# zqs01/ASR_chinese_e2e

Hardware: AMD Instinct MI355X
Metric: training throughput (utterances/s; frames/s = x T), AISHELL-1-shaped 80-mel T=500 (higher is better)
Workload: dtype bf16; 1 GPU; configs[2]: joint CTC/attention (lambda=0.3) encoder-decoder, bf16, per-GPU batch 32, T=500, F=80, V=4232, 6 layers, d_model 512, 8x64 heads, ff 1024, dropout 0.0, fwd+loss+CER+bwd+clip+Noam/Adam per step, eager launches; global_batch=32, seq_len=500, parallelism=dp1

## Files before the change

asr_chinese_e2e_amd/Models/transformer_official.py:

```python
import math

import torch

from .. import engine as E
from .. import kernels as K
from ..Bases import BaseConfig, BaseModel
from ..Utils import Pack

SOS_ID, EOS_ID, PAD_ID = 2, 3, 0
PE_MAXLEN = 5000
CLIP_NORM = 5.0


def _set_nested(root, dotted, value, is_buffer=False):
    parts = dotted.split(".")
    mod = root
    for p in parts[:-1]:
        if not hasattr(mod, p):
            mod.add_module(p, torch.nn.Module())
        mod = getattr(mod, p)
    if is_buffer:
        mod.register_buffer(parts[-1], value)
    else:
        mod.register_parameter(parts[-1], value)


class _SpeechTransformer(BaseModel):
    USE_DECODER = True

    def __init__(self, config, vocab):
        super().__init__()
        self.config = config
        self.vocab = vocab
        c = config
        self.use_decoder = self.USE_DECODER
        lam = float(getattr(c, "ctc_weight", 0.0))
        self.ctc_weight = lam if self.use_decoder else 1.0
        self.use_ctc = (lam > 0.0) or not self.use_decoder
        self.cross_mask = getattr(c, "cross_mask", "ref_compat")
        self.lowp = str(getattr(c, "dtype", "bf16")).lower() in ("bf16", "bfloat16")
        self.attn_window = int(getattr(c, "attn_window", -1))
        self.label_smoothing = float(getattr(c, "label_smoothing", 0.0))
        self.cer_in_iterate = bool(getattr(c, "cer_in_iterate", True))
        self._step_seed = int(getattr(c, "seed", 0))
        d, H, dk, ff = c.d_model, c.num_head, c.hidden_size, c.ff_size
        d_in = c.n_mels * c.lfr_m
        V = vocab.vocab_size
        self.V = V

        blocks = [[("encoder.linear_in.weight", (d, d_in))], [("encoder.linear_in.bias", (d,))],
                  [("encoder.layer_norm_in.weight", (d,))], [("encoder.layer_norm_in.bias", (d,))]]
        for i in range(c.layer_num):
            blocks += E.mha_param_block(f"encoder.layer_stack.{i}.slf_attn.", H, dk, d)
            blocks += E.ffn_param_block(f"encoder.layer_stack.{i}.pos_ffn.", d, ff)
        if self.use_ctc:
            blocks += [[("ctc_lo.weight", (V, d))], [("ctc_lo.bias", (V,))]]
        if self.use_decoder:
            blocks += [[("decoder.tgt_word_emb.weight", (V, d))]]
            blocks += E.cross_kv_param_blocks([f"decoder.layer_stack.{i}.enc_attn." for i in range(c.layer_num)], H, dk, d)
            for i in range(c.layer_num):
                blocks += E.mha_param_block(f"decoder.layer_stack.{i}.slf_attn.", H, dk, d)
                blocks += E.cross_q_param_block(f"decoder.layer_stack.{i}.enc_attn.", H, dk, d)
                blocks += E.ffn_param_block(f"decoder.layer_stack.{i}.pos_ffn.", d, ff)
        self._flat = E.FlatParams(blocks)
        self._engine = None
        self._views_checked = False
        self._grads_checked = False
        self._flat_device = None

        order = self._state_order(c.layer_num)
        for name in order:
            if name.endswith("positional_encoding.pe"):
                _set_nested(self, name, E.positional_encoding(PE_MAXLEN, d), is_buffer=True)
            elif name == "decoder.tgt_word_prj.weight":
                _set_nested(self, name, self.decoder.tgt_word_emb.weight)
            else:
                wname = name[:-5] + ".weight" if name.endswith(".bias") else name
                wshape = self._flat.index[wname][1]
                _set_nested(self, name, torch.nn.Parameter(self._init_tensor(name, self._flat.index[name][1], wshape, d, dk)))

    def _state_order(self, L):
        def mha(pre):
            return [pre + n for n in ("w_qs.weight", "w_qs.bias", "w_ks.weight", "w_ks.bias", "w_vs.weight", "w_vs.bias",
                                      "layer_norm.weight", "layer_norm.bias", "fc.weight", "fc.bias")]

        def ffn(pre):
            return [pre + n for n in ("w_1.weight", "w_1.bias", "w_2.weight", "w_2.bias", "layer_norm.weight", "layer_norm.bias")]

        names = ["encoder.linear_in.weight", "encoder.linear_in.bias", "encoder.layer_norm_in.weight",
                 "encoder.layer_norm_in.bias", "encoder.positional_encoding.pe"]
        for i in range(L):
            names += mha(f"encoder.layer_stack.{i}.slf_attn.") + ffn(f"encoder.layer_stack.{i}.pos_ffn.")
        if self.use_decoder:
            names += ["decoder.tgt_word_emb.weight", "decoder.positional_encoding.pe"]
            for i in range(L):
                names += mha(f"decoder.layer_stack.{i}.slf_attn.") + mha(f"decoder.layer_stack.{i}.enc_attn.") + ffn(f"decoder.layer_stack.{i}.pos_ffn.")
            names += ["decoder.tgt_word_prj.weight"]
        if self.use_ctc:
            names += ["ctc_lo.weight", "ctc_lo.bias"]
        return names

    @staticmethod
    def _init_tensor(name, shape, wshape, d, dk):
        t = torch.empty(*shape)
        leaf = name.rsplit(".", 2)[-2]
        if leaf in ("layer_norm", "layer_norm_in"):
            return t.fill_(1.0) if name.endswith(".weight") else t.zero_()
        fan_out, fan_in = wshape[0], wshape[1]
        if name == "decoder.tgt_word_emb.weight":
            return t.normal_(0.0, 1.0)
        if name.endswith(".weight"):
            if leaf in ("w_qs", "w_ks", "w_vs"):
                return t.normal_(0.0, math.sqrt(2.0 / (d + dk)))
            if leaf in ("fc", "linear_in", "ctc_lo"):
                return t.normal_(0.0, math.sqrt(2.0 / (fan_in + fan_out)))
        bound = 1.0 / math.sqrt(fan_in)
        return t.uniform_(-bound, bound)

    def _named_flat_params(self):
        for name, p in self.named_parameters():
            yield name, p

    def _ensure_engine(self, device):
        device = torch.device(device)
        if device.type == "cuda" and device.index is None:
            device = torch.device("cuda", torch.cuda.current_device())
        if device.type != "cuda":
            raise RuntimeError("the HIP engine runs on an MI355X only: move the model and batch to 'cuda' "
                               "(there is no CPU fallback; the CPU oracle lives in oracle/ for tests)")
        f = self._flat
        ok = self._engine is not None and self._flat_device == device
        if ok and self._views_checked:
            return self._engine
        if ok:
            for name, p in self._named_flat_params():
                off, shape = f.index[name]
                if p.data_ptr() != f.p.data_ptr() + 4 * off:
                    ok = False
                    break
        if ok:
            self._views_checked = True
            return self._engine
        K.bind_device(device)
        old = {name: p.detach().to(device=device, dtype=torch.float32) for name, p in self._named_flat_params()}
        old_mv = (f.m.to(device), f.v.to(device)) if f.m is not None else None
        f.allocate(device, self.lowp)
        if old_mv is not None:
            f.m.copy_(old_mv[0])
            f.v.copy_(old_mv[1])
        for name, p in self._named_flat_params():
            view = f.view(f.p, name)
            view.copy_(old[name].view(view.shape))
            p.data = view
            p.grad = f.view(f.g, name)
        f.refresh_lowp()
        for b in self.buffers():
            b.data = b.data.to(device)
        pe = self.encoder.positional_encoding.pe[0].to(device).contiguous()
        self._engine = E.Engine(f, self.config, self.V, self.use_decoder, self.use_ctc, pe)
        self._flat_device = device
        self._views_checked = True
        self._grads_checked = True
        return self._engine

    def zero_grad(self, set_to_none=True):
        self._grads_checked = False
        return super().zero_grad(set_to_none=set_to_none)

    def _apply(self, fn, *a, **kw):
        self._views_checked = False
        self._grads_checked = False
        return super()._apply(fn, *a, **kw)

    def load_state_dict(self, state_dict, strict=True, **kw):
        state_dict = {k: v for k, v in state_dict.items()}
        self._views_checked = False
        out = super().load_state_dict(state_dict, strict=strict, **kw)
        if self._flat.p is not None:
            self._flat.refresh_lowp()
        return out

    def zero_flat_grads(self):
        f = self._flat
        eng = self._engine
        self._zero_lazy = eng is not None and eng._tr_tiles is not None and eng.overlap_wgrad
        if not self._zero_lazy:
            f.g.zero_()
        if self._grads_checked:
            return
        for name, p in self._named_flat_params():
            if p.grad is None or p.grad.data_ptr() != f.g.data_ptr() + 4 * f.index[name][0]:
                p.grad = f.view(f.g, name)
        self._grads_checked = True

    def _prepare(self, input, training=False):
        wave = input.wave
        eng = self._ensure_engine(wave.device)
        eng.training = bool(training)
        if training:
            self._step_seed = (self._step_seed + 1) & 0x7FFFFFFF
            eng.step_seed = self._step_seed
        x = wave if wave.dtype == eng.dtype else wave.to(eng.dtype)
        x = x.contiguous()
        if input.tgt_for_input is None:
            self._tgt_len32 = None
            return eng, x, self._len32_of(input.wave_len, (), ()).contiguous(), None
        tgt = input.tgt_for_input.contiguous()
        lens64 = [t.contiguous() for t in (input.wave_len, input.tgt_len) if t is not None and t.dtype == torch.int64 and t.device == tgt.device]
        out = K.dec_preprocess(tgt, SOS_ID, EOS_ID, lens64=lens64)
        prep, lens32 = out[:6], (out[6] if lens64 else ())
        wave_len = self._len32_of(input.wave_len, lens64, lens32)
        self._tgt_len32 = self._len32_of(input.tgt_len, lens64, lens32) if input.tgt_len is not None else None
        return eng, x, wave_len, prep

    @staticmethod
    def _len32_of(t, lens64, lens32):
        for a, b in zip(lens64, lens32):
            if a.data_ptr() == t.data_ptr() and a.numel() == t.numel():
                return b
        return t.to(torch.int32)

    def forward(self, input):
        eng, x, wave_len, prep = self._prepare(input)
        B, T, _ = x.shape
        enc, _ = eng.encoder_fwd(x, wave_len, self.attn_window)
        pack = Pack()
        pack.add(encoder_out=enc.view(B, T, -1))
        if self.use_decoder and prep is not None:
            cross_len = self._tgt_len32 if self.cross_mask == "ref_compat" else wave_len
            pred, _ = eng.decoder_fwd(prep, enc, cross_len, B, T)
            pack.add(pred=pred.view(B, -1, self.V), gold=prep[1].long())
        if self.use_ctc:
            logits = eng.ctc_lo.fwd(enc)
            pack.add(ctc_logits=logits.view(B, T, self.V))
        return pack

    def _tok_table(self, device):
        if getattr(self, "_tok_tab", None) is None or self._tok_tab[0].device != torch.device(device):
            self._tok_tab = K.token_table(self.vocab._id2token, device)
        return self._tok_tab

    def _cer_ids(self, ids, gold, hyp_len=None, ref_len=None):
        per = K.cer(ids.int().contiguous(), gold.int().contiguous(), self._tok_table(ids.device), self.vocab._token2id[self.vocab.PAD],
                    hyp_len=hyp_len, ref_len=ref_len)
        return (per.sum() * (100.0 / per.numel())).reshape(1)

    CER_BESIDE_BACKWARD = True

    def _cer_beside_backward(self, eng, pg):
        if not (self.CER_BESIDE_BACKWARD and eng.aux_overlap) or torch.cuda.is_current_stream_capturing():
            return pg
        eng._disarm()
        eng._fork(eng.ctc_stream)
        with torch.cuda.stream(eng.ctc_stream):
            cer = self._cer_ids(pg[0], pg[1])
        if getattr(self, "_cer_event", None) is None:
            self._cer_event = torch.cuda.Event()
        self._cer_event.record(eng.ctc_stream)
        self._cer_keep = pg
        return cer, self._cer_event

    def _ctc_cer_beside_backward(self, eng, path, wave_len, labels32, lab_len):
        def score():
            ids, lens = K.ctc_collapse(path, wave_len, PAD_ID)
            return self._cer_ids(ids, labels32, hyp_len=lens, ref_len=lab_len)
        if not (self.CER_BESIDE_BACKWARD and eng.aux_overlap) or torch.cuda.is_current_stream_capturing():
            return score(), None
        eng._disarm()
        eng._fork(eng.ctc_stream)
        with torch.cuda.stream(eng.ctc_stream):
            cer = score()
        if getattr(self, "_cer_event", None) is None:
            self._cer_event = torch.cuda.Event()
        self._cer_event.record(eng.ctc_stream)
        self._cer_keep = (path, wave_len, labels32, lab_len)
        return cer, self._cer_event

    def _cer_of(self, pg):
        if isinstance(pg[1], torch.cuda.Event):
            torch.cuda.current_stream().wait_event(pg[1])
            return pg[0]
        if pg[1] is None:
            return pg[0]
        return self._cer_ids(pg[0], pg[1])

    def _cer(self, pred, gold):
        return self._cer_ids(pred.argmax(-1), gold)

    def cal_metrics(self, output, input):
        pack = Pack()
        row_nll = nll = n_valid = None
        if self.use_decoder:
            pred, gold = output.pred, output.gold
            B, To, V = pred.shape
            n_valid = (gold != PAD_ID).sum().float().reshape(1)
            row_nll, _ = K.xent_fwd_bwd(pred.reshape(B * To, V).contiguous(), gold.reshape(-1).int(), n_valid, PAD_ID, smoothing=self.label_smoothing, want_grad=False)
        if self.use_ctc:
            prep = K.dec_preprocess(input.tgt_for_input.contiguous(), SOS_ID, EOS_ID)
            nll, _ = K.ctc_fwd_bwd(output.ctc_logits.contiguous(), input.wave_len.to(torch.int32), prep[2], prep[4], self._engine.ws, want_grad=False)
        lam = self.ctc_weight
        loss = K.loss_combine(row_nll, n_valid, nll, 1.0 - lam if self.use_ctc else 1.0, lam)
        assert not torch.isinf(loss[0])
        pack.add(loss=loss[0])
        if self.use_decoder:
            pack.add(cer=self._cer(output.pred, output.gold))
        if self.use_ctc:
            cer = self._ctc_cer(output.ctc_logits.contiguous(), input.wave_len.to(torch.int32), prep[2], prep[4])
            pack.add(**({"ctc_cer": cer} if self.use_decoder else {"cer": cer}))
        return pack

    def beam_search(self, input, beam_size=5, nbest=1, decode_max_len=0, ctc_weight=0.0, joint="rescore", ctc_pre_beam=None):
        from .. import decode
        if joint not in ("rescore", "one_pass"):
            raise ValueError(f"joint must be 'rescore' or 'one_pass' (got {joint!r})")
        if joint == "one_pass":
            return decode.one_pass_beam_search(self, input, beam_size, nbest, decode_max_len, ctc_weight, ctc_pre_beam)
        if ctc_pre_beam is not None:
            raise ValueError("ctc_pre_beam applies to joint='one_pass' only")
        if ctc_weight > 0.0:
            return decode.joint_beam_search(self, input, beam_size, nbest, decode_max_len, ctc_weight)
        return decode.beam_search(self, input, beam_size, nbest, decode_max_len)

    def ctc_prefix_beam_search(self, input, beam_size=5, nbest=1, frame_topk=10, on_device=None):
        from .. import decode
        return decode.ctc_prefix_beam_search(self, input, beam_size, nbest, frame_topk, on_device)

    def ctc_greedy_search(self, input):
        with torch.no_grad():
            out = self.forward(input)
        ids, lens = K.ctc_greedy_decode(out.ctc_logits.contiguous(), input.wave_len.to(torch.int32), PAD_ID)
        ids, lens = ids.cpu(), lens.cpu()
        return [ids[b, : int(lens[b])].tolist() for b in range(ids.shape[0])]

    def frame_seconds(self):
        from ..data_handler.processor import HOP
        return int(getattr(self.config, "lfr_n", 3) or 3) * HOP / float(getattr(self.config, "sample_rate", 16000) or 16000)

    def ctc_align(self, input, labels=None):
        if not self.use_ctc:
            raise RuntimeError("this model has no CTC head (config.ctc_weight = 0)")
        if labels is None:
            if input.tgt_for_input is None:
                raise ValueError("ctc_align(labels=None) aligns the batch's transcripts, and this batch has none: pass labels")
            prep = K.dec_preprocess(input.tgt_for_input.contiguous(), SOS_ID, EOS_ID)
            lab, lens = prep[2].cpu(), prep[4].cpu().tolist()
            labels = [lab[b, : lens[b]].tolist() for b in range(lab.shape[0])]
        return self._align_lists(self._ctc_logits(input), input.wave_len, labels)

    def _ctc_logits(self, input):
        eng = self._ensure_engine(input.wave.device)
        was_training = eng.training
        try:
            with torch.no_grad():
                return self.forward(input).ctc_logits
        finally:
            eng.training = was_training

    def _align_lists(self, logits, wave_len, labels, alignable=None):
        B, T, V = logits.shape
        if len(labels) != B:
            raise ValueError(f"{len(labels)} label sequences for a batch of {B}")
        labels = [[int(x) for x in l] for l in labels]
        ok = [True] * B if alignable is None else list(alignable)
        for b, l in enumerate(labels):
            if ok[b] and (len(l) > 255 or any(x < 0 or x >= V for x in l)):
                raise ValueError(f"utterance {b}: labels must be at most 255 ids in [0, {V})")
        use = [l if ok[b] else [] for b, l in enumerate(labels)]
        Lmax = max([len(l) for l in use] + [0])
        lab = torch.zeros(B, Lmax, dtype=torch.int32)
        for b, l in enumerate(use):
            if l:
                lab[b, : len(l)] = torch.tensor(l, dtype=torch.int32)
        dev = logits.device
        lab_len = torch.tensor([len(l) for l in use], dtype=torch.int32)
        _, spans, tlp, score = K.ctc_align(logits, wave_len.to(torch.int32).contiguous(), lab.to(dev), lab_len.to(dev), blank=PAD_ID,
                                           ws=self._engine.ws)
        spans, tlp, score = spans.cpu().tolist(), tlp.cpu().tolist(), score.cpu().tolist()
        d = self.frame_seconds()
        id2tok = self.vocab._id2token
        out = []
        for b, l in enumerate(labels):
            timed = ok[b] and score[b] != float("-inf")
            toks = []
            for i, x in enumerate(l):
                st, en = (spans[b][i][0], spans[b][i][1]) if timed else (None, None)
                toks.append({"id": x, "token": id2tok[x] if 0 <= x < len(id2tok) else None, "start_frame": st, "end_frame": en,
                             "start_s": st * d if timed else None, "end_s": (en + 1) * d if timed else None,
                             "logp": tlp[b][i] if timed else None})
            out.append({"score": score[b] if ok[b] else None, "tokens": toks})
        return out

    def transcribe(self, input, beam_size=5, ctc_weight=None, timestamps=True, joint="rescore"):
        if joint not in ("rescore", "one_pass"):
            raise ValueError(f"joint must be 'rescore' or 'one_pass' (got {joint!r})")
        if joint == "one_pass" and not (self.use_decoder and self.use_ctc):
            raise RuntimeError("joint='one_pass' needs a model with both the attention decoder and the CTC head")
        if timestamps and not self.use_ctc:
            raise ValueError("timestamps come from the CTC head, and this model has none (config.ctc_weight = 0)")
        if self.use_decoder:
            w = float(getattr(self.config, "ctc_weight", 0.0)) if ctc_weight is None else float(ctc_weight)
            hyps = self.beam_search(input, beam_size, 1, ctc_weight=w if self.use_ctc else 0.0, joint=joint)
        else:
            hyps = self.ctc_prefix_beam_search(input, beam_size, 1)
        ids, scores = [], []
        for h in hyps:
            if not h:
                ids.append([])
                scores.append(float("-inf"))
                continue
            seq = list(h[0]["yseq"])
            if self.use_decoder:
                seq = seq[1:] if seq and seq[0] == SOS_ID else seq
                seq = seq[:-1] if seq and seq[-1] == EOS_ID else seq
            ids.append(seq)
            scores.append(float(h[0]["score"]))
        id2tok = self.vocab._id2token
        out = [{"text": "".join(id2tok[x] for x in seq if x not in (PAD_ID, SOS_ID, EOS_ID)), "ids": seq, "score": sc, "tokens": None}
               for seq, sc in zip(ids, scores)]
        if timestamps:
            V = self.V
            ok = [len(seq) <= 255 and all(0 <= x < V and x != PAD_ID for x in seq) for seq in ids]
            al = self._align_lists(self._ctc_logits(input), input.wave_len, ids, alignable=ok)
            for o, a in zip(out, al):
                o["tokens"] = a["tokens"]
        return out

    def _ctc_cer(self, logits, wave_len, labels32, lab_len):
        ids, lens = K.ctc_greedy_decode(logits, wave_len, PAD_ID)
        return self._cer_ids(ids, labels32, hyp_len=lens, ref_len=lab_len)

    def train_step(self, input, loss_scale=1.0, count_hook=None):
        eng, x, wave_len, prep = self._prepare(input, training=self.training)
        B, T, _ = x.shape
        lam = self.ctc_weight
        ys_in, ys_out, labels32, dec_len, lab_len, n_valid = prep
        pending = count_hook(n_valid, B) if count_hook is not None else None
        zero, self._zero_lazy = (self._flat.g if getattr(self, "_zero_lazy", False) else None), False
        eng.refresh_transposes(zero=zero)
        enc, ecache = eng.encoder_fwd(x, wave_len, self.attn_window)
        batch_div = None
        if pending is not None:
            n_valid, batch_div = pending.wait()
        row_nll = nll = None
        d_enc = None
        pg = None
        ctc_done = None
        ctc_scale = dict(grad_scale=lam * loss_scale, grad_scale_div=batch_div) if batch_div is not None else dict(grad_scale=lam * loss_scale / float(B))
        ctc_async = (self.use_decoder and self.use_ctc and eng.overlap_ctc and not eng.deterministic and not torch.cuda.is_current_stream_capturing())
        if ctc_async:
            eng.decoder_kv_async(prep, enc, B, T)
            nll, d_enc, ctc_done = eng.ctc_branch_async(enc, wave_len, labels32, lab_len, B, T, **ctc_scale)
        if self.use_decoder:
            cross_len = self._tgt_len32 if self.cross_mask == "ref_compat" else wave_len
            pred, dcache = eng.decoder_fwd(prep, enc, cross_len, B, T)
            ids = torch.empty(ys_out.shape, dtype=torch.int32, device=pred.device) if self.cer_in_iterate else None
            w_ce = (1.0 - lam) if self.use_ctc else 1.0
            row_nll, dpred = K.xent_fwd_bwd(pred, ys_out.reshape(-1), n_valid, PAD_ID, smoothing=self.label_smoothing, grad_scale=w_ce * loss_scale, dlogits=pred,
                                            argmax=ids)
            if ids is not None:
                pg = (ids, ys_out)
        if self.use_ctc and not ctc_async:
            path = torch.empty(B, T, dtype=torch.int32, device=enc.device) if (self.cer_in_iterate and not self.use_decoder) else None
            nll, d_enc = eng.ctc_fwd_bwd(enc, wave_len, labels32, lab_len, B, T, best_path=path, **ctc_scale)
            if path is not None:
                pg = self._ctc_cer_beside_backward(eng, path, wave_len, labels32, lab_len)
        if self.use_decoder:
            if d_enc is None:
                d_enc = torch.zeros_like(enc)
            eng.decoder_bwd(dcache, dpred, d_enc, d_enc_ready=ctc_done)
            if pg is not None:
                pg = self._cer_beside_backward(eng, pg)
        eng.encoder_bwd(ecache, d_enc)
        loss = K.loss_combine(row_nll, n_valid, nll, (1.0 - lam) if self.use_ctc else 1.0, lam)
        return loss, pg

    def iterate(self, input, optimizer=None, is_train=True):
        if optimizer is None or not is_train:
            with torch.no_grad():
                output = self.forward(input)
                return self.cal_metrics(output, input), None
        self._ensure_engine(input.wave.device)
        optimizer.zero_grad()
        if getattr(optimizer, "fused_step", None) is None or not getattr(optimizer, "keeps_grad_views", False):
            self._grads_checked = False
        self.zero_flat_grads()
        loss, pg = self.train_step(input)
        fused = getattr(optimizer, "fused_step", None)
        if fused is not None:
            fused(self._flat, CLIP_NORM)
        else:
            torch.nn.utils.clip_grad_norm_(self.parameters(), CLIP_NORM)
            optimizer.step()
            self._flat.refresh_lowp()
        metrics = Pack()
        metrics.add(loss=loss[0])
        if self.use_decoder and self.use_ctc:
            metrics.add(ce=loss[1], ctc=loss[2])
        if pg is not None:
            metrics.add(cer=self._cer_of(pg))
        return metrics, None

    def greedy_search(self, input, decode_max_len=0):
        return self.beam_search(input, 1, 1, decode_max_len)

    @classmethod
    def get_default_config(cls):
        class ModelConfig(BaseConfig):
            d_model = 512
            hidden_size = 64
            ff_size = 1024
            num_head = 8
            dropout = 0.1
            layer_num = 6
            share_weight = False
            ctc_weight = 0.0
            label_smoothing = 0.0
            cross_mask = "ref_compat"
            dtype = "bf16"
            attn_window = -1

        return ModelConfig


class TransformerOffical(_SpeechTransformer):
    USE_DECODER = True


class TransformerCTC(_SpeechTransformer):
    USE_DECODER = False
```

asr_chinese_e2e_amd/_lib.py:

```python
import ctypes
import os
from ctypes import c_char_p, c_float, c_int, c_size_t, c_uint32, c_void_p

import torch

_HERE = os.path.dirname(os.path.abspath(__file__))
LIB_PATH = os.environ.get("ASR_HIP_LIB") or os.path.join(_HERE, "libasr_hip.so")

ASR_F32, ASR_BF16 = 0, 1
ACT_NONE, ACT_RELU, ACT_RELU_MASK = 0, 1, 2
ABI_VERSION = 10
DROP_PRE, DROP_POST = 1, 2

P, I, F, Z, U = c_void_p, c_int, c_float, c_size_t, c_uint32

class TnProblem(ctypes.Structure):
    _fields_ = [("dY", P), ("X", P), ("dW", P), ("dbias", P), ("M", I), ("N", I), ("K", I), ("ldy", I), ("ldx", I), ("ldw", I)]


TN_GROUP_MAX = 8


class LnReduceItem(ctypes.Structure):
    _fields_ = [("ws", P), ("dgamma", P), ("dbeta", P), ("dbias", P), ("rows", I)]


LN_REDUCE_MAX = 16


class DecLayerPlan(ctypes.Structure):
    _fields_ = ([(n, I) for n in ("B", "To", "T", "d", "H", "dk", "ff")] + [("drop_p", F), ("seed", U * 5), ("ld_kv_c_T", I)] +
                [(n, P) for n in ("dec_len", "cross_len",
                                  "w_qkv_s", "w_fc_s", "w_q_c", "w_fc_c", "w_1", "w_2",
                                  "b_qkv_s", "b_fc_s", "b_q_c", "b_fc_c", "b_1", "b_2",
                                  "g_s", "be_s", "g_c", "be_c", "g_f", "be_f",
                                  "w_kv_c_T", "x_in",
                                  "qkv_s", "ctx_s", "a_s", "y_s", "lse_s", "rstd_s",
                                  "q_c", "kv_c", "kv_ready_event",
                                  "ctx_c", "a_c", "y_c", "lse_c", "rstd_c",
                                  "h", "o", "y_f", "rstd_f",
                                  "dz_f", "g_o", "g_h", "dx_f",
                                  "dz_c", "g_ac", "g_qc", "g_kvc", "dx_c",
                                  "dz_s", "g_as", "g_qkv", "dx_s",
                                  "dctx", "gb_2", "gb_fc_c", "gb_fc_s",
                                  "part_f", "part_c", "part_s", "delta")] +
                [("delta_bytes", Z), ("d_enc", P), ("wgrad_stream", P), ("aux_cus", I), ("ld_kv_c", I), ("kv_dgrad_cols", I), ("g_kv_group", P), ("ctx_s_lo", P), ("ctx_c_lo", P)])

SIGNATURES = {
    "asr_abi_version": (I, []),
    "asr_last_error": (I, [c_char_p, Z]),
    "asr_stream_fork": (I, [P, P]),
    "asr_stream_arm": (I, [P, P]),
    "asr_stream_arm_pending": (I, []),
    "asr_stream_create": (I, [I, P]),
    "asr_set_option": (I, [c_char_p, I, P]),
    "asr_get_deterministic": (I, []),
    "asr_set_deterministic": (I, [I]),
    "asr_add_ln_fwd": (I, [P, P, P, P, P, P, P, P, P, I, I, I, F, U, I, I, P]),
    "asr_add_ln_bwd_workspace_bytes": (Z, [I, I]),
    "asr_add_ln_bwd": (I, [P, P, P, P, P, P, P, P, P, P, P, P, Z, I, I, I, F, U, I, I, P]),
    "asr_add_ln_bwd_reduce_batched": (I, [P, I, I, P]),
    "asr_sdpa_fwd": (I, [P, P, P, P, P, P, I, I, I, I, I, I, I, I, I, I, I, F, F, U, P, I, P]),
    "asr_sdpa_bwd_workspace_bytes": (Z, [I, I, I, I, I, I, I, I]),
    "asr_sdpa_bwd": (I, [P, P, P, P, P, P, P, Z, P, P, P, P, I, I, I, I, I, I, I, I, I, I, I, F, F, U, P, I, P]),
    "asr_dropout_mask": (I, [P, I, I, F, U, P]),
    "asr_sdpa_dropout_mask": (I, [P, I, I, I, I, F, U, P]),
    "asr_ctc_workspace_bytes": (Z, [I, I, I]),
    "asr_ctc_fwd_bwd": (I, [P, P, P, P, P, P, I, I, I, I, I, I, F, P, I, P, P, Z, I, P]),
    "asr_ctc_align_workspace_bytes": (Z, [I, I, I]),
    "asr_ctc_align": (I, [P, P, P, P, P, P, P, P, I, I, I, I, I, I, P, Z, I, P]),
    "asr_ctc_greedy_decode": (I, [P, P, P, P, I, I, I, I, I, I, P]),
    "asr_ctc_frame_argmax": (I, [P, P, P, I, I, I, I, I, I, P]),
    "asr_ctc_collapse": (I, [P, P, P, I, I, I, P]),
    "asr_decode_attn": (I, [P, P, P, P, P, I, I, I, I, I, I, I, I, I, I, I, F, I, P]),
    "asr_logsoftmax_topk": (I, [P, P, P, I, I, I, I, I, P]),
    "asr_ctc_frame_topk": (I, [P, P, P, P, I, I, I, I, I, I, P]),
    "asr_ctc_prefix_beam_workspace_bytes": (Z, [I, I, I]),
    "asr_ctc_prefix_beam": (I, [P, P, P, P, P, Z, P, P, P, I, I, I, I, I, I, I, P]),
    "asr_beam_step": (I, [P, P, P, P, P, P, P, P, P, P, P, P, I, I, I, I, P]),
    "asr_cache_gather": (I, [P, P, P, I, I, I, I, I, I, P]),
    "asr_ctc_prefix_logprobs": (I, [P, P, I, I, I, I, I, P]),
    "asr_ctc_prefix_score": (I, [P, P, P, P, P, P, P, P, P, P, P, P, P, P, P, P, I, I, I, I, I, I, F, I, I, P]),
    "asr_ctc_prefix_gather": (I, [P, P, P, P, P, P, P, P, P, I, I, I, I, P]),
    "asr_joint_beam_step": (I, [P, P, P, P, P, P, P, P, P, P, P, P, P, P, P, P, P, P, P, I, I, I, I, F, P]),
    "asr_xent_fwd_bwd": (I, [P, P, P, P, P, I, I, I, F, F, P, I, P]),
    "asr_dec_preprocess": (I, [P, P, P, P, P, P, P, I, I, I, I, P, P, P, P, P]),
    "asr_embed_pe_fwd": (I, [P, P, P, P, F, I, I, I, I, F, U, I, P]),
    "asr_embed_bwd": (I, [P, P, P, P, F, I, I, I, F, U, I, P]),
    "asr_relu_fwd": (I, [P, Z, I, P]),
    "asr_relu_bwd": (I, [P, P, P, P, Z, I, I, I, P]),
    "asr_colsum_workspace_bytes": (Z, [I, I]),
    "asr_colsum": (I, [P, P, P, Z, I, I, I, I, I, P]),
    "asr_cast": (I, [P, P, Z, I, I, P]),
    "asr_sumsq_workspace_bytes": (Z, [Z]),
    "asr_grad_sumsq": (I, [P, Z, P, P, Z, P]),
    "asr_noam_hyper": (I, [P, P, F, F, F, F, F, F, P]),
    "asr_grad_sumsq_noam": (I, [P, Z, P, P, Z, P, P, F, F, F, F, F, F, P]),
    "asr_adam_step": (I, [P, P, P, P, P, Z, P, P, F, F, F, F, I, P]),
    "asr_loss_combine": (I, [P, I, P, P, I, F, F, P, P]),
    "asr_gemm_nt_bf16": (I, [P, P, P, P, P, I, I, I, I, I, I, I, P]),
    "asr_gemm_small_bf16": (I, [P, P, P, P, P, I, I, I, I, I, I, I, I, P]),
    "asr_gemm_f32": (I, [P, P, P, P, P, I, I, I, I, I, I, I, I, I, I, P]),
    "asr_decoder_layer_fwd": (I, [P, P]),
    "asr_decoder_layer_bwd": (I, [P, P, P, P, P]),
    "asr_gemm_tn_workspace_bytes": (Z, [I, I, I]),
    "asr_gemm_tn_bf16": (I, [P, P, P, I, I, I, I, I, I, I, P, Z, P]),
    "asr_gemm_tn_bias_bf16": (I, [P, P, P, P, I, I, I, I, I, I, I, P, Z, P]),
    "asr_gemm_tn_grouped_bf16": (I, [P, I, I, P]),
    "asr_transpose_batched_bf16": (I, [P, P, P, I, P]),
    "asr_cer": (I, [P, P, I, I, P, P, I, I, P, P, I, I, I, I, P, P]),
    "asr_logmel_fwd": (I, [P, P, P, P, P, I, I, I, I, P]),
    "asr_utt_norm_lfr_fwd": (I, [P, P, P, P, I, I, I, I, I, I, I, P]),
    "asr_utt_norm_augment_lfr_fwd": (I, [P, P, P, P, P, I, I, I, I, I, I, I, P]),
}


class AsrHipError(RuntimeError):
    pass


def _check_runtime_env(env=None):
    env = os.environ if env is None else env
    v = env.get("ROC_SYSTEM_SCOPE_SIGNAL")
    if v is not None and v.strip() == "0":
        raise RuntimeError("ROC_SYSTEM_SCOPE_SIGNAL=0 is set: the two-stream training step of asr_chinese_e2e_amd waits on completion signals "
                           "across HIP queues and would hang silently under it - unset the variable (or set it to 1)")


def _load():
    _check_runtime_env()
    if not os.path.isfile(LIB_PATH):
        raise ImportError(
            f"{LIB_PATH} not found: the HIP extension is required (no CPU fallback). "
            "Build it with `make -C asr_chinese_e2e_amd/csrc`.")
    lib = ctypes.CDLL(LIB_PATH)
    for name, (res, args) in SIGNATURES.items():
        try:
            fn = getattr(lib, name)
        except AttributeError as e:
            raise ImportError(f"{LIB_PATH} does not export {name}: rebuild the extension") from e
        fn.restype = res
        fn.argtypes = args
    v = lib.asr_abi_version()
    if v != ABI_VERSION:
        raise ImportError(f"libasr_hip.so ABI version {v}, binding expects {ABI_VERSION}")
    return lib


lib = _load()


def _bind_fast():
    try:
        alt = os.environ.get("ASR_FASTCALL_DIR")
        if alt:
            import glob
            import importlib.machinery
            import importlib.util
            path = glob.glob(os.path.join(alt, "_asr_fastcall*.so"))[0]
            loader = importlib.machinery.ExtensionFileLoader("_asr_fastcall", path)
            _asr_fastcall = importlib.util.module_from_spec(importlib.util.spec_from_loader("_asr_fastcall", loader))
            loader.exec_module(_asr_fastcall)
        else:
            from . import _asr_fastcall
    except (ImportError, IndexError) as e:
        raise ImportError(f"asr_chinese_e2e_amd/_asr_fastcall*.so not found or not loadable ({e}): build it with "
                          "`make -C asr_chinese_e2e_amd/csrc` (it is part of the required native code; there is no slow path)") from e
    kind = {P: "P", I: "I", F: "F", Z: "Z", U: "U", c_char_p: "P"}

    class _Fast:
        pass
    ns = _Fast()
    for name, (res, args) in SIGNATURES.items():
        addr = ctypes.cast(getattr(lib, name), c_void_p).value
        setattr(ns, name, _asr_fastcall.make(addr, name, "".join(kind[a] for a in args), "Z" if res is Z else "I"))
    return ns


fast = _bind_fast()


def last_error():
    buf = ctypes.create_string_buffer(512)
    lib.asr_last_error(buf, 512)
    return buf.value.decode("utf-8", "replace")


def check(rc, what=""):
    if rc != 0:
        names = {-1: "ASR_EINVAL", -2: "ASR_EDTYPE", -3: "ASR_EWORKSPACE", -4: "ASR_EHIP"}
        raise AsrHipError(f"{what}: {names.get(rc, rc)}: {last_error()}")
```

asr_chinese_e2e_amd/csrc/decoder_exec.hip:

```cpp
#include "asr_common.h"

#define DEC_TRY(call)                \
    do {                             \
        const int rc__ = (call);     \
        if (rc__ != ASR_OK) {        \
            asr_stream_arm_pending(); \
            return rc__;             \
        }                            \
    } while (0)

static int dec_check(const asr_dec_layer_plan* p, const char* who) {
    if (!p) ASR_FAIL(ASR_EINVAL, "%s: null plan", who);
    if (p->B <= 0 || p->To <= 0 || p->T <= 0 || p->H <= 0 || p->dk <= 0 || p->d <= 0 || p->ff <= 0)
        ASR_FAIL(ASR_EINVAL, "%s: bad dims B=%d To=%d T=%d d=%d H=%d dk=%d ff=%d", who, p->B, p->To, p->T, p->d, p->H, p->dk, p->ff);
    if (p->d % 8 || (p->H * p->dk) % 8 || p->ff % 8) ASR_FAIL(ASR_EINVAL, "%s: d, H*dk and ff must be multiples of 8", who);
    return ASR_OK;
}

extern "C" int asr_decoder_layer_fwd(const asr_dec_layer_plan* p, void* stream) {
    DEC_TRY(dec_check(p, "asr_decoder_layer_fwd"));
    const int B = p->B, To = p->To, T = p->T, d = p->d, H = p->H, dk = p->dk, hd = H * dk, ff = p->ff, M = B * To;
    const float scale = 1.0f / sqrtf((float)dk);
    const size_t e = 2;
    char* qkv = (char*)p->qkv_s;
    DEC_TRY(asr_gemm_small_bf16(p->x_in, p->w_qkv_s, p->b_qkv_s, nullptr, p->qkv_s, M, 3 * hd, d, d, d, 3 * hd, 0, ASR_ACT_NONE, stream));
    DEC_TRY(asr_sdpa_fwd(qkv, qkv + hd * e, qkv + 2 * hd * e, p->ctx_s, p->lse_s, p->dec_len, B, H, To, To, dk, 3 * hd, 3 * hd, 3 * hd, hd, 1, -1, scale,
                         p->drop_p, p->seed[0], p->ctx_s_lo, ASR_BF16, stream));
    DEC_TRY(asr_gemm_small_bf16(p->ctx_s, p->w_fc_s, p->b_fc_s, nullptr, p->a_s, M, d, hd, hd, hd, d, 0, ASR_ACT_NONE, stream));
    DEC_TRY(asr_add_ln_fwd(p->a_s, p->x_in, p->g_s, p->be_s, nullptr, p->dec_len, p->y_s, p->a_s, p->rstd_s, B, To, d, p->drop_p, p->seed[1], ASR_DROP_PRE,
                           ASR_BF16, stream));
    DEC_TRY(asr_gemm_small_bf16(p->y_s, p->w_q_c, p->b_q_c, nullptr, p->q_c, M, hd, d, d, d, hd, 0, ASR_ACT_NONE, stream));
    if (p->kv_ready_event) {
        const hipError_t he = hipStreamWaitEvent((hipStream_t)stream, (hipEvent_t)p->kv_ready_event, 0);
        if (he != hipSuccess) ASR_FAIL(ASR_EHIP, "asr_decoder_layer_fwd: hipStreamWaitEvent: %s", hipGetErrorString(he));
    }
    char* kv = (char*)p->kv_c;
    const int ldkv = p->ld_kv_c > 0 ? p->ld_kv_c : 2 * hd;
    DEC_TRY(asr_sdpa_fwd(p->q_c, kv, kv + hd * e, p->ctx_c, p->lse_c, p->cross_len, B, H, To, T, dk, hd, ldkv, ldkv, hd, 0, -1, scale, p->drop_p, p->seed[2],
                         p->ctx_c_lo, ASR_BF16, stream));
    DEC_TRY(asr_gemm_small_bf16(p->ctx_c, p->w_fc_c, p->b_fc_c, nullptr, p->a_c, M, d, hd, hd, hd, d, 0, ASR_ACT_NONE, stream));
    DEC_TRY(asr_add_ln_fwd(p->a_c, p->y_s, p->g_c, p->be_c, nullptr, p->dec_len, p->y_c, p->a_c, p->rstd_c, B, To, d, p->drop_p, p->seed[3], ASR_DROP_PRE,
                           ASR_BF16, stream));
    DEC_TRY(asr_gemm_small_bf16(p->y_c, p->w_1, p->b_1, nullptr, p->h, M, ff, d, d, d, ff, 0, ASR_ACT_RELU, stream));
    DEC_TRY(asr_gemm_small_bf16(p->h, p->w_2, p->b_2, nullptr, p->o, M, d, ff, ff, ff, d, 0, ASR_ACT_NONE, stream));
    DEC_TRY(asr_add_ln_fwd(p->o, p->y_c, p->g_f, p->be_f, nullptr, p->dec_len, p->y_f, p->o, p->rstd_f, B, To, d, p->drop_p, p->seed[4], ASR_DROP_PRE, ASR_BF16,
                           stream));
    return ASR_OK;
}

extern "C" int asr_decoder_layer_bwd(const asr_dec_layer_plan* p, const void* dy, const void* dy2, void* stream, void* aux_stream) {
    DEC_TRY(dec_check(p, "asr_decoder_layer_bwd"));
    if (!dy) ASR_FAIL(ASR_EINVAL, "asr_decoder_layer_bwd: null dy");
    const int B = p->B, To = p->To, T = p->T, d = p->d, H = p->H, dk = p->dk, hd = H * dk, ff = p->ff, M = B * To;
    const float scale = 1.0f / sqrtf((float)dk);
    const size_t e = 2;
    const bool drop = p->drop_p > 0.f;
    const size_t part_bytes = asr_add_ln_bwd_workspace_bytes(M, d);
    void* dxg_f = drop ? p->g_o : p->dz_f;
    DEC_TRY(asr_add_ln_bwd(dy, dy2, p->o, p->rstd_f, p->g_f, p->dec_len, p->dz_f, drop ? p->g_o : nullptr, nullptr, nullptr, p->gb_2, p->part_f, part_bytes, B, To, d,
                           p->drop_p, p->seed[4], ASR_DROP_PRE, ASR_BF16, stream));
    DEC_TRY(asr_gemm_small_bf16(dxg_f, p->w_2, nullptr, p->h, p->g_h, M, ff, d, d, ff, ff, 1, ASR_ACT_RELU_MASK, stream));
    DEC_TRY(asr_gemm_small_bf16(p->g_h, p->w_1, nullptr, nullptr, p->dx_f, M, d, ff, ff, d, d, 1, ASR_ACT_NONE, stream));
    void* dxg_c = drop ? p->g_ac : p->dz_c;
    DEC_TRY(asr_add_ln_bwd(p->dx_f, p->dz_f, p->a_c, p->rstd_c, p->g_c, p->dec_len, p->dz_c, drop ? p->g_ac : nullptr, nullptr, nullptr, p->gb_fc_c, p->part_c, part_bytes,
                           B, To, d, p->drop_p, p->seed[3], ASR_DROP_PRE, ASR_BF16, stream));
    DEC_TRY(asr_gemm_small_bf16(dxg_c, p->w_fc_c, nullptr, nullptr, p->dctx, M, hd, d, d, hd, hd, 1, ASR_ACT_NONE, stream));
    char* kv = (char*)p->kv_c;
    char* gkv = (char*)p->g_kvc;
    const bool kv_dgrad = p->d_enc && p->w_kv_c_T;
    const int ldkv = p->ld_kv_c > 0 ? p->ld_kv_c : 2 * hd;
    if (p->kv_dgrad_cols > 0 && (!p->g_kv_group || p->kv_dgrad_cols % 8 || p->kv_dgrad_cols > ldkv)) ASR_FAIL(ASR_EINVAL, "asr_decoder_layer_bwd: kv_dgrad_cols = %d needs g_kv_group, a multiple of 8, <= ld_kv_c = %d", p->kv_dgrad_cols, ldkv);
    if (kv_dgrad && aux_stream) DEC_TRY(asr_stream_arm(stream, aux_stream));
    DEC_TRY(asr_sdpa_bwd(p->q_c, kv, kv + hd * e, p->ctx_c, p->dctx, p->lse_c, p->delta, p->delta_bytes, p->g_qc, gkv, gkv + hd * e, p->cross_len, B, H, To, T, dk, hd,
                         ldkv, ldkv, hd, 0, -1, scale, p->drop_p, p->seed[2], p->ctx_c_lo, ASR_BF16, stream));
    if (kv_dgrad) {
        void* st2 = aux_stream ? aux_stream : stream;
        if (aux_stream && asr_stream_arm_pending()) DEC_TRY(asr_stream_fork(stream, aux_stream));
        const int old_lim = p->aux_cus > 0 ? asr_option_set(ASR_OPT_CU_LIMIT, p->aux_cus) : 0;
        const void* g_a = p->kv_dgrad_cols > 0 ? p->g_kv_group : p->g_kvc;
        const int cols = p->kv_dgrad_cols > 0 ? p->kv_dgrad_cols : 2 * hd;
        const int rc_kv = asr_gemm_nt_bf16(g_a, p->w_kv_c_T, nullptr, p->d_enc, p->d_enc, B * T, d, cols, ldkv, p->ld_kv_c_T, d, ASR_ACT_NONE, st2);
        if (p->aux_cus > 0) asr_option_set(ASR_OPT_CU_LIMIT, old_lim);
        DEC_TRY(rc_kv);
    }
    DEC_TRY(asr_gemm_small_bf16(p->g_qc, p->w_q_c, nullptr, nullptr, p->dx_c, M, d, hd, hd, d, d, 1, ASR_ACT_NONE, stream));
    void* dxg_s = drop ? p->g_as : p->dz_s;
    DEC_TRY(asr_add_ln_bwd(p->dx_c, p->dz_c, p->a_s, p->rstd_s, p->g_s, p->dec_len, p->dz_s, drop ? p->g_as : nullptr, nullptr, nullptr, p->gb_fc_s, p->part_s, part_bytes,
                           B, To, d, p->drop_p, p->seed[1], ASR_DROP_PRE, ASR_BF16, stream));
    DEC_TRY(asr_gemm_small_bf16(dxg_s, p->w_fc_s, nullptr, nullptr, p->dctx, M, hd, d, d, hd, hd, 1, ASR_ACT_NONE, stream));
    char* qkv = (char*)p->qkv_s;
    char* gq = (char*)p->g_qkv;
    DEC_TRY(asr_sdpa_bwd(qkv, qkv + hd * e, qkv + 2 * hd * e, p->ctx_s, p->dctx, p->lse_s, p->delta, p->delta_bytes, gq, gq + hd * e, gq + 2 * hd * e, p->dec_len, B, H, To,
                         To, dk, 3 * hd, 3 * hd, 3 * hd, hd, 1, -1, scale, p->drop_p, p->seed[0], p->ctx_s_lo, ASR_BF16, stream));
    if (p->wgrad_stream) DEC_TRY(asr_stream_arm(stream, p->wgrad_stream));
    DEC_TRY(asr_gemm_small_bf16(p->g_qkv, p->w_qkv_s, nullptr, nullptr, p->dx_s, M, d, 3 * hd, 3 * hd, d, d, 1, ASR_ACT_NONE, stream));
    return ASR_OK;
}
```

asr_chinese_e2e_amd/csrc/misc.hip:

```cpp
#include <stdarg.h>
#include <stdlib.h>

#include "asr_common.h"

static thread_local char g_err[512] = "";

void asr_set_error(const char* fmt, ...) {
    va_list ap;
    va_start(ap, fmt);
    vsnprintf(g_err, sizeof(g_err), fmt, ap);
    va_end(ap);
}

extern "C" int asr_abi_version(void) { return ASR_ABI_VERSION; }

static int g_deterministic = -1;
int asr_deterministic(void) {
    if (g_deterministic < 0) {
        const char* e = getenv("ASR_DETERMINISTIC");
        g_deterministic = (e && atoi(e) != 0) ? 1 : 0;
    }
    return g_deterministic;
}
extern "C" int asr_get_deterministic(void) { return asr_deterministic(); }
// ... 91 lines not shown
    if (e != hipSuccess || !st) ASR_FAIL(ASR_EHIP, "asr_stream_create: %s", hipGetErrorString(e));
    *out_stream = (void*)st;
    return ASR_OK;
}

namespace {

constexpr int EW_BLOCK = 256;
ASR_FULL_WAVES(EW_BLOCK);
static int ew_grid(size_t nvec) {
    size_t g = (nvec + EW_BLOCK - 1) / EW_BLOCK;
    return (int)(g < 2048 ? (g ? g : 1) : 2048);
}

template <typename T> __global__ __launch_bounds__(EW_BLOCK) void relu_fwd_kernel(T* x, size_t n8, size_t n) {
    for (size_t i = blockIdx.x * (size_t)EW_BLOCK + threadIdx.x; i < n8; i += (size_t)gridDim.x * EW_BLOCK) {
        float v[8];
        load8<T>(x + i * 8, v);
#pragma unroll
        for (int j = 0; j < 8; ++j) v[j] = fmaxf(v[j], 0.f);
        store8<T>(x + i * 8, v);
    }
    if (blockIdx.x == 0) {
        size_t i = n8 * 8 + threadIdx.x;
        if (i < n) x[i] = from_f32<T>(fmaxf(to_f32<T>(x[i]), 0.f));
    }
}

template <typename S, typename D> __global__ __launch_bounds__(EW_BLOCK) void cast_kernel(const S* s, D* d, size_t n8, size_t n) {
    for (size_t i = blockIdx.x * (size_t)EW_BLOCK + threadIdx.x; i < n8; i += (size_t)gridDim.x * EW_BLOCK) {
        float v[8];
        load8<S>(s + i * 8, v);
        store8<D>(d + i * 8, v);
    }
    if (blockIdx.x == 0) {
        size_t i = n8 * 8 + threadIdx.x;
        if (i < n) d[i] = from_f32<D>(to_f32<S>(s[i]));
    }
}

constexpr int CS_WAVES = 4;
template <typename T, bool RELU_BWD>
__global__ __launch_bounds__(CS_WAVES* WAVE) void colsum_partial_kernel(T* __restrict__ x, const T* __restrict__ a,
                                                                         float* __restrict__ ws, int rows, int cols, int ld,
                                                                         int row_slots) {
    const int lane = threadIdx.x & 63, w = threadIdx.x >> 6;
    const int c0 = blockIdx.x * 256 + lane * 4;
    f32x4 acc = {0.f, 0.f, 0.f, 0.f};
    const bool full = (c0 + 3 < cols) && (ld % 4 == 0);
    const int rstride = row_slots * CS_WAVES;
    int r = blockIdx.y * CS_WAVES + w;
    if (full) {
        for (; r + 3 * rstride < rows; r += 4 * rstride) {
            f32x4 v[4], av[4];
#pragma unroll
            for (int u = 0; u < 4; ++u) {
                v[u] = load4<T>(x + (size_t)(r + u * rstride) * ld + c0);
                if constexpr (RELU_BWD) av[u] = load4<T>(a + (size_t)(r + u * rstride) * ld + c0);
            }
#pragma unroll
            for (int u = 0; u < 4; ++u) {
                if constexpr (RELU_BWD) {
#pragma unroll
                    for (int j = 0; j < 4; ++j) v[u][j] = av[u][j] > 0.f ? v[u][j] : 0.f;
                    store4<T>(x + (size_t)(r + u * rstride) * ld + c0, v[u]);
                }
                acc += v[u];
            }
        }
    }
    for (; r < rows; r += rstride) {
        T* p = x + (size_t)r * ld + c0;
        if (full) {
            f32x4 v = load4<T>(p);
            if constexpr (RELU_BWD) {
                f32x4 av = load4<T>(a + (size_t)r * ld + c0);
#pragma unroll
                for (int j = 0; j < 4; ++j) v[j] = av[j] > 0.f ? v[j] : 0.f;
                store4<T>(p, v);
            }
            acc += v;
        } else {
#pragma unroll
            for (int j = 0; j < 4; ++j)
                if (c0 + j < cols) {
                    float v = to_f32<T>(p[j]);
                    if constexpr (RELU_BWD) {
                        v = to_f32<T>(a[(size_t)r * ld + c0 + j]) > 0.f ? v : 0.f;
                        p[j] = from_f32<T>(v);
                    }
                    acc[j] += v;
                }
        }
    }
    __shared__ __attribute__((aligned(16))) float sred[CS_WAVES][256];
    *(f32x4*)&sred[w][lane * 4] = acc;
    __syncthreads();
    const int c = blockIdx.x * 256 + threadIdx.x;
    if (c < cols) ws[(size_t)blockIdx.y * cols + c] = sred[0][threadIdx.x] + sred[1][threadIdx.x] + sred[2][threadIdx.x] + sred[3][threadIdx.x];
}

static int cs_row_slots(int rows, int cols) {
    int ctiles = ceil_div(cols, 256);
    int want = 2048 / ctiles;
    int maxs = ceil_div(rows, CS_WAVES);
    if (want > maxs) want = maxs;
    if (want < 1) want = 1;
    if (want > 256) want = 256;
    return want;
}

__global__ void dec_preprocess_kernel(const int64_t* __restrict__ tgt, int32_t* ys_in, int32_t* ys_out,
                                      int32_t* labels32, int32_t* dec_len, int32_t* lab_len, float* n_valid,
                                      int B, int Lmax, int sos, int eos, const int64_t* __restrict__ len_a, int32_t* len32_a,
                                      const int64_t* __restrict__ len_b, int32_t* len32_b) {
    __shared__ int cnt[1024];
    const int b = threadIdx.x;
    int n = 0;
    if (b < B) {
        if (len_a) len32_a[b] = (int32_t)len_a[b];
        if (len_b) len32_b[b] = (int32_t)len_b[b];
        const int To = Lmax + 1;
        int32_t* yi = ys_in + (size_t)b * To;
        int32_t* yo = ys_out + (size_t)b * To;
        int32_t* lb = labels32 + (size_t)b * Lmax;
        yi[0] = sos;
        for (int j = 0; j < Lmax; ++j) {
            int v = (int)tgt[(size_t)b * Lmax + j];
            if (v != 0) {
                lb[n] = v;
                yi[1 + n] = v;
                yo[n] = v;
                ++n;
            }
        }
        yo[n] = eos;
        for (int j = n + 1; j < To; ++j) { yi[j] = eos; yo[j] = 0; }
        for (int j = n; j < Lmax; ++j) lb[j] = 0;
        dec_len[b] = n + 1;
        lab_len[b] = n;
    }
    cnt[threadIdx.x] = (b < B) ? n + 1 : 0;
    __syncthreads();
    if (threadIdx.x == 0) {
        int s = 0;
        for (int i = 0; i < B; ++i) s += cnt[i];
        *n_valid = (float)s;
    }
}

template <typename T, typename W>
__global__ __launch_bounds__(256) void embed_pe_fwd_kernel(const int32_t* __restrict__ ids, const W* __restrict__ emb,
                                                           const float* __restrict__ pe, T* __restrict__ y, float scale,
                                                           int rows, int To, int d, int V, uint32_t seed, uint32_t thr, float dscale) {
    const int row = blockIdx.x;
    int id = ids[row];
    id = id < 0 ? 0 : (id >= V ? V - 1 : id);
    const int t = row % To;
    for (int c = threadIdx.x; c < d; c += blockDim.x) {
        float v = to_f32<W>(emb[(size_t)id * d + c]) * scale + pe[(size_t)t * d + c];
        if (thr) v = drop_keep_at((uint32_t)row * (uint32_t)d + c, seed, thr) ? v * dscale : 0.f;
        y[(size_t)row * d + c] = from_f32<T>(v);
    }
}
template <typename T>
__global__ __launch_bounds__(256) void embed_bwd_kernel(const int32_t* __restrict__ ids, const T* __restrict__ dy, const T* __restrict__ dy2,
                                                        float* __restrict__ demb, float scale, int d, int V, uint32_t seed, uint32_t thr,
                                                        float dscale) {
    const int row = blockIdx.x;
    const int id = ids[row];
    if (id < 0 || id >= V) return;
    for (int c = threadIdx.x; c < d; c += blockDim.x) {
        float g = (to_f32<T>(dy[(size_t)row * d + c]) + (dy2 ? to_f32<T>(dy2[(size_t)row * d + c]) : 0.f)) * scale;
        if (thr) g = drop_keep_at((uint32_t)row * (uint32_t)d + c, seed, thr) ? g * dscale : 0.f;
        if (g != 0.f) atomicAdd(&demb[(size_t)id * d + c], g);
    }
}

template <typename T>
__global__ __launch_bounds__(256) void embed_bwd_serial_kernel(const int32_t* __restrict__ ids, const T* __restrict__ dy, const T* __restrict__ dy2,
                                                               float* demb, float scale, int rows, int d, int V, uint32_t seed, uint32_t thr,
                                                               float dscale) {
    const int c = blockIdx.x * 256 + threadIdx.x;
    if (c >= d) return;
    for (int row = 0; row < rows; ++row) {
        const int id = ids[row];
        if (id < 0 || id >= V) continue;
        float g = (to_f32<T>(dy[(size_t)row * d + c]) + (dy2 ? to_f32<T>(dy2[(size_t)row * d + c]) : 0.f)) * scale;
        if (thr) g = drop_keep_at((uint32_t)row * (uint32_t)d + c, seed, thr) ? g * dscale : 0.f;
        if (g != 0.f) demb[(size_t)id * d + c] += g;
    }
}

__global__ __launch_bounds__(256) void dropout_mask_kernel(uint8_t* mask, size_t rows, int cols, uint32_t seed, uint32_t thr) {
    const size_t n = rows * (size_t)cols;
    const uint32_t cp = (uint32_t)((cols + 1) & ~1);
    for (size_t i = blockIdx.x * 256ull + threadIdx.x; i < n; i += (size_t)gridDim.x * 256) {
        const size_t r = i / cols;
        const uint32_t c = (uint32_t)(i - r * cols);
        mask[i] = drop_keep_at((uint32_t)r * cp + c, seed, thr) ? 1 : 0;
    }
}

constexpr int SS_BLOCK = 256;
ASR_FULL_WAVES(SS_BLOCK);
__global__ __launch_bounds__(SS_BLOCK) void sumsq_partial_kernel(const float* __restrict__ g, size_t n4, size_t n, float* __restrict__ part) {
    __shared__ float red[16];
    float s = 0.f;
    for (size_t i = blockIdx.x * (size_t)SS_BLOCK + threadIdx.x; i < n4; i += (size_t)gridDim.x * SS_BLOCK) {
        f32x4 v = *(const f32x4*)(g + i * 4);
        s += v[0] * v[0] + v[1] * v[1] + v[2] * v[2] + v[3] * v[3];
    }
    if (blockIdx.x == 0) {
        size_t i = n4 * 4 + threadIdx.x;
        if (i < n) s += g[i] * g[i];
    }
    s = block_sum(s, red);
    if (threadIdx.x == 0) part[blockIdx.x] = s;
}
__global__ __launch_bounds__(256) void sum_finalize_kernel(const float* __restrict__ part, int P, float* out) {
    __shared__ float red[16];
    float s = 0.f;
    for (int i = threadIdx.x; i < P; i += 256) s += part[i];
    s = block_sum(s, red);
    if (threadIdx.x == 0) *out = s;
}
__device__ __forceinline__ void noam_update(int32_t* step, float* hyper, float model_size, float warmup, float factor, float lr_const, float b1, float b2) {
    const int s = *step + 1;
    *step = s;
    const double sd = (double)s;
    double lr = lr_const;
    if (warmup > 0.f) {
        double a = pow(sd, -0.5), b = sd * pow((double)warmup, -1.5);
        lr = (double)factor * pow((double)model_size, -0.5) * (a < b ? a : b);
    }
    hyper[0] = (float)lr;
    hyper[1] = (float)(1.0 - pow((double)b1, sd));
    hyper[2] = (float)sqrt(1.0 - pow((double)b2, sd));
    hyper[3] = (float)s;
}
__global__ __launch_bounds__(256) void sum_finalize_noam_kernel(const float* __restrict__ part, int P, float* out, int32_t* step, float* hyper, float model_size,
                                                                float warmup, float factor, float lr_const, float b1, float b2) {
    __shared__ float red[16];
    float s = 0.f;
    for (int i = threadIdx.x; i < P; i += 256) s += part[i];
    s = block_sum(s, red);
    if (threadIdx.x == 0) {
        *out = s;
        noam_update(step, hyper, model_size, warmup, factor, lr_const, b1, b2);
    }
}
static int ss_grid(size_t n) {
    size_t g = (n / 4 + SS_BLOCK - 1) / SS_BLOCK;
    return (int)(g < 1024 ? (g ? g : 1) : 1024);
}

__global__ void noam_hyper_kernel(int32_t* step, float* hyper, float model_size, float warmup, float factor,
                                  float lr_const, float b1, float b2) {
    noam_update(step, hyper, model_size, warmup, factor, lr_const, b1, b2);
}

__global__ __launch_bounds__(EW_BLOCK) void adam_kernel(float* __restrict__ p, float* __restrict__ g, float* __restrict__ m,
                                                        float* __restrict__ v, bf16_t* __restrict__ p_lp, size_t n4, size_t n,
                                                        const float* __restrict__ hyper, const float* __restrict__ sumsq,
                                                        float max_norm, float b1, float b2, float eps, int write_clipped) {
    const float lr = hyper[0], bc1 = hyper[1], bc2s = hyper[2];
    float coef = 1.f;
    if (max_norm > 0.f) {
        const float norm = sqrtf(*sumsq);
        coef = fminf(max_norm / (norm + 1e-6f), 1.f);
    }
    const float step_size = lr / bc1;
    write_clipped = write_clipped && coef != 1.f;
    for (size_t i = blockIdx.x * (size_t)EW_BLOCK + threadIdx.x; i < n4; i += (size_t)gridDim.x * EW_BLOCK) {
        f32x4 gv = *(const f32x4*)(g + i * 4), mv = *(const f32x4*)(m + i * 4), vv = *(const f32x4*)(v + i * 4), pv = *(const f32x4*)(p + i * 4);
#pragma unroll
        for (int j = 0; j < 4; ++j) {
            const float gg = gv[j] * coef;
            gv[j] = gg;
            mv[j] = b1 * mv[j] + (1.f - b1) * gg;
            vv[j] = b2 * vv[j] + (1.f - b2) * gg * gg;
            pv[j] -= step_size * mv[j] / (sqrtf(vv[j]) / bc2s + eps);
        }
        *(f32x4*)(m + i * 4) = mv;
        *(f32x4*)(v + i * 4) = vv;
        *(f32x4*)(p + i * 4) = pv;
        if (write_clipped) *(f32x4*)(g + i * 4) = gv;
        if (p_lp) store4<bf16_t>(p_lp + i * 4, pv);
    }
    if (blockIdx.x == 0) {
        size_t i = n4 * 4 + threadIdx.x;
        if (i < n) {
            const float gg = g[i] * coef;
            const float mm = b1 * m[i] + (1.f - b1) * gg;
            const float vv = b2 * v[i] + (1.f - b2) * gg * gg;
            const float pp = p[i] - step_size * mm / (sqrtf(vv) / bc2s + eps);
            m[i] = mm; v[i] = vv; p[i] = pp;
            if (write_clipped) g[i] = gg;
            if (p_lp) p_lp[i] = (bf16_t)pp;
        }
    }
}

__global__ __launch_bounds__(256) void loss_combine_kernel(const float* row_nll, int M, const float* n_valid, const float* nll, int B,
                                                           float w_ce, float w_ctc, float* loss) {
    __shared__ float red[16];
    float s = 0.f, c = 0.f;
    if (row_nll) for (int i = threadIdx.x; i < M; i += 256) s += row_nll[i];
    if (nll) for (int i = threadIdx.x; i < B; i += 256) c += nll[i];
    s = block_sum(s, red);
    c = block_sum(c, red);
    if (threadIdx.x == 0) {
        const float ce = row_nll ? s / *n_valid : 0.f;
        const float ctc = nll ? c / (float)B : 0.f;
        loss[0] = (row_nll ? w_ce * ce : 0.f) + (nll ? w_ctc * ctc : 0.f);
        loss[1] = ce;
        loss[2] = ctc;
    }
}

}

extern "C" int asr_relu_fwd(void* x, size_t n, int dtype, void* stream) {
    if (!x) ASR_FAIL(ASR_EINVAL, "asr_relu_fwd: null pointer");
    hipStream_t st = (hipStream_t)stream;
    if (dtype == ASR_F32) relu_fwd_kernel<float><<<ew_grid(n / 8), EW_BLOCK, 0, st>>>((float*)x, n / 8, n);
    else if (dtype == ASR_BF16) relu_fwd_kernel<bf16_t><<<ew_grid(n / 8), EW_BLOCK, 0, st>>>((bf16_t*)x, n / 8, n);
    else ASR_FAIL(ASR_EDTYPE, "asr_relu_fwd: dtype %d", dtype);
    ASR_CHECK_LAUNCH("asr_relu_fwd");
    return ASR_OK;
}

__global__ __launch_bounds__(256) void transpose_batched_kernel(const bf16_t* __restrict__ src, bf16_t* __restrict__ dst, const int32_t* __restrict__ tiles) {
    __shared__ bf16_t tile[64][66];
    const int32_t* e = tiles + 6 * (size_t)blockIdx.x;
    const size_t off = (size_t)(uint32_t)e[0], doff = (size_t)(uint32_t)e[4];
    const int N = e[1], K = e[2], r0 = (e[3] >> 16) * 64, c0 = (e[3] & 0xffff) * 64, ldd = e[5];
    const int tx = threadIdx.x & 63, ty = threadIdx.x >> 6;
#pragma unroll
    for (int i = 0; i < 16; ++i) {
        const int r = r0 + ty + 4 * i, c = c0 + tx;
        if (r < N && c < K) tile[ty + 4 * i][tx] = src[off + (size_t)r * K + c];
    }
    __syncthreads();
#pragma unroll
    for (int i = 0; i < 16; ++i) {
        const int c = c0 + ty + 4 * i, r = r0 + tx;
        if (r < N && c < K) dst[doff + (size_t)c * ldd + r] = tile[tx][ty + 4 * i];
    }
}

__global__ __launch_bounds__(256) void transpose_batched_vec_kernel(const bf16_t* __restrict__ src, bf16_t* __restrict__ dst, const int32_t* __restrict__ tiles) {
    __shared__ __attribute__((aligned(16))) bf16_t tile[64][72];
    const int32_t* e = tiles + 6 * (size_t)blockIdx.x;
    const size_t off = (size_t)(uint32_t)e[0], doff = (size_t)(uint32_t)e[4];
    const int N = e[1], K = e[2], r0 = (e[3] >> 16) * 64, c0 = (e[3] & 0xffff) * 64, ldd = e[5];
    const bool vec = ((N | K | ldd) % 8 == 0) && (off % 8 == 0) && (doff % 8 == 0) && (((uintptr_t)src | (uintptr_t)dst) % 16 == 0);
    if (vec) {
#pragma unroll
        for (int c = 0; c < 2; ++c) {
            const int id = threadIdx.x + 256 * c, r = id >> 3, ch = id & 7;
            u32x4 v = {0u, 0u, 0u, 0u};
            if (r0 + r < N && c0 + ch * 8 < K) v = *(const u32x4*)(src + off + (size_t)(r0 + r) * K + c0 + ch * 8);
            *(u32x4*)(&tile[r][ch * 8]) = v;
        }
        __syncthreads();
#pragma unroll
        for (int c = 0; c < 2; ++c) {
            const int id = threadIdx.x + 256 * c, kk = id >> 3, ch = id & 7;
            if (c0 + kk < K && r0 + ch * 8 < N) {
                bf16x8 v;
#pragma unroll
                for (int j = 0; j < 8; ++j) v[j] = tile[ch * 8 + j][kk];
                *(bf16x8*)(dst + doff + (size_t)(c0 + kk) * ldd + r0 + ch * 8) = v;
            }
        }
        return;
    }
    const int tx = threadIdx.x & 63, ty = threadIdx.x >> 6;
#pragma unroll
    for (int i = 0; i < 16; ++i) {
        const int r = r0 + ty + 4 * i, c = c0 + tx;
        if (r < N && c < K) tile[ty + 4 * i][tx] = src[off + (size_t)r * K + c];
    }
    __syncthreads();
#pragma unroll
    for (int i = 0; i < 16; ++i) {
        const int c = c0 + ty + 4 * i, r = r0 + tx;
        if (r < N && c < K) dst[doff + (size_t)c * ldd + r] = tile[tx][ty + 4 * i];
    }
}

extern "C" int asr_transpose_batched_bf16(const void* src, void* dst, const int32_t* tiles, int ntiles, void* stream) {
    if (!src || !dst || !tiles) ASR_FAIL(ASR_EINVAL, "asr_transpose_batched_bf16: null pointer");
    if (ntiles <= 0) ASR_FAIL(ASR_EINVAL, "asr_transpose_batched_bf16: ntiles=%d", ntiles);
    transpose_batched_vec_kernel<<<ntiles, 256, 0, (hipStream_t)stream>>>((const bf16_t*)src, (bf16_t*)dst, tiles);
    ASR_CHECK_LAUNCH("asr_transpose_batched_bf16");
    return ASR_OK;
}

extern "C" int asr_cast(const void* src, void* dst, size_t n, int sd, int dd, void* stream) {
    if (!src || !dst) ASR_FAIL(ASR_EINVAL, "asr_cast: null pointer");
    hipStream_t st = (hipStream_t)stream;
    const int g = ew_grid(n / 8);
    if (sd == ASR_F32 && dd == ASR_BF16) cast_kernel<float, bf16_t><<<g, EW_BLOCK, 0, st>>>((const float*)src, (bf16_t*)dst, n / 8, n);
    else if (sd == ASR_BF16 && dd == ASR_F32) cast_kernel<bf16_t, float><<<g, EW_BLOCK, 0, st>>>((const bf16_t*)src, (float*)dst, n / 8, n);
    else if (sd == ASR_F32 && dd == ASR_F32) cast_kernel<float, float><<<g, EW_BLOCK, 0, st>>>((const float*)src, (float*)dst, n / 8, n);
    else if (sd == ASR_BF16 && dd == ASR_BF16) cast_kernel<bf16_t, bf16_t><<<g, EW_BLOCK, 0, st>>>((const bf16_t*)src, (bf16_t*)dst, n / 8, n);
    else ASR_FAIL(ASR_EDTYPE, "asr_cast: dtypes %d -> %d", sd, dd);
    ASR_CHECK_LAUNCH("asr_cast");
    return ASR_OK;
}

extern "C" size_t asr_colsum_workspace_bytes(int rows, int cols) {
    return (size_t)cs_row_slots(rows, cols) * cols * sizeof(float);
}

template <bool RELU_BWD>
static int colsum_impl(void* x, const void* a, float* out, void* ws, size_t ws_bytes, int rows, int cols, int ld,
                       int accumulate, int dtype, hipStream_t st, const char* name) {
    if (!x || (RELU_BWD && !a)) ASR_FAIL(ASR_EINVAL, "%s: null pointer", name);
    if (rows <= 0 || cols <= 0 || ld < cols) ASR_FAIL(ASR_EINVAL, "%s: bad shape rows=%d cols=%d ld=%d", name, rows, cols, ld);
    const bool want_sum = out != nullptr;
    if (want_sum && (!ws || ws_bytes < asr_colsum_workspace_bytes(rows, cols))) ASR_FAIL(ASR_EWORKSPACE, "%s: workspace too small", name);
    const int slots = cs_row_slots(rows, cols);
    dim3 grid(ceil_div(cols, 256), slots);
    if (!ws || ws_bytes < asr_colsum_workspace_bytes(rows, cols)) ASR_FAIL(ASR_EWORKSPACE, "%s: workspace too small", name);
    if (dtype == ASR_F32) colsum_partial_kernel<float, RELU_BWD><<<grid, CS_WAVES * WAVE, 0, st>>>((float*)x, (const float*)a, (float*)ws, rows, cols, ld, slots);
    else if (dtype == ASR_BF16) colsum_partial_kernel<bf16_t, RELU_BWD><<<grid, CS_WAVES * WAVE, 0, st>>>((bf16_t*)x, (const bf16_t*)a, (float*)ws, rows, cols, ld, slots);
    else ASR_FAIL(ASR_EDTYPE, "%s: dtype %d", name, dtype);
    if (want_sum) colsum_finalize_kernel<<<dim3(ceil_div(cols, 32), accumulate && slots >= 1024 && !asr_deterministic() ? 4 : 1), 1024, 0, st>>>((const float*)ws, slots, (size_t)cols, cols, cols, out, nullptr, nullptr, accumulate);
    ASR_CHECK_LAUNCH(name);
    return ASR_OK;
}

extern "C" int asr_colsum(const void* x, float* out, void* ws, size_t ws_bytes, int rows, int cols, int ld, int accumulate,
                          int dtype, void* stream) {
    if (!out) ASR_FAIL(ASR_EINVAL, "asr_colsum: null out");
    return colsum_impl<false>((void*)x, nullptr, out, ws, ws_bytes, rows, cols, ld, accumulate, dtype, (hipStream_t)stream, "asr_colsum");
}

extern "C" int asr_relu_bwd(void* da, const void* a, float* dbias, void* ws, size_t ws_bytes, int rows, int cols, int dtype,
                            void* stream) {
    return colsum_impl<true>(da, a, dbias, ws, ws_bytes, rows, cols, cols, 1, dtype, (hipStream_t)stream, "asr_relu_bwd");
}

extern "C" int asr_dec_preprocess(const int64_t* tgt, int32_t* ys_in, int32_t* ys_out, int32_t* labels32, int32_t* dec_len,
                                  int32_t* lab_len, float* n_valid, int B, int Lmax, int sos, int eos, const int64_t* len_a, int32_t* len32_a,
                                  const int64_t* len_b, int32_t* len32_b, void* stream) {
    if (!tgt || !ys_in || !ys_out || !labels32 || !dec_len || !lab_len || !n_valid) ASR_FAIL(ASR_EINVAL, "asr_dec_preprocess: null pointer");
    if ((len_a && !len32_a) || (len_b && !len32_b)) ASR_FAIL(ASR_EINVAL, "asr_dec_preprocess: a length vector without its int32 output");
    if (B <= 0 || B > 1024 || Lmax <= 0) ASR_FAIL(ASR_EINVAL, "asr_dec_preprocess: bad shape B=%d Lmax=%d (B <= 1024)", B, Lmax);
    const int threads = ceil_div(B, 64) * 64;
    dec_preprocess_kernel<<<1, threads, 0, (hipStream_t)stream>>>(tgt, ys_in, ys_out, labels32, dec_len, lab_len, n_valid, B, Lmax, sos, eos, len_a, len32_a, len_b, len32_b);
    ASR_CHECK_LAUNCH("asr_dec_preprocess");
    return ASR_OK;
}

extern "C" int asr_embed_pe_fwd(const int32_t* ids, const void* emb, const float* pe, void* y, float scale, int B, int To, int d,
                                int V, float drop_p, uint32_t drop_seed, int dtype, void* stream) {
    if (!ids || !emb || !pe || !y) ASR_FAIL(ASR_EINVAL, "asr_embed_pe_fwd: null pointer");
    if (B <= 0 || To <= 0 || d <= 0 || V <= 0) ASR_FAIL(ASR_EINVAL, "asr_embed_pe_fwd: bad shape");
    if (drop_p < 0.f || drop_p >= 1.f || (drop_p > 0.f && (d & 1))) ASR_FAIL(ASR_EINVAL, "asr_embed_pe_fwd: bad dropout p=%f", drop_p);
    hipStream_t st = (hipStream_t)stream;
    const uint32_t thr = drop_thr16(drop_p);
    const float ds = 1.f / (1.f - drop_p);
    if (dtype == ASR_F32) embed_pe_fwd_kernel<float, float><<<B * To, 256, 0, st>>>(ids, (const float*)emb, pe, (float*)y, scale, B * To, To, d, V, drop_seed, thr, ds);
    else if (dtype == ASR_BF16) embed_pe_fwd_kernel<bf16_t, float><<<B * To, 256, 0, st>>>(ids, (const float*)emb, pe, (bf16_t*)y, scale, B * To, To, d, V, drop_seed, thr, ds);
    else ASR_FAIL(ASR_EDTYPE, "asr_embed_pe_fwd: dtype %d", dtype);
    ASR_CHECK_LAUNCH("asr_embed_pe_fwd");
    return ASR_OK;
}

extern "C" int asr_embed_bwd(const int32_t* ids, const void* dy, const void* dy2, float* demb, float scale, int rows, int d, int V, float drop_p,
                             uint32_t drop_seed, int dtype, void* stream) {
    if (!ids || !dy || !demb) ASR_FAIL(ASR_EINVAL, "asr_embed_bwd: null pointer");
    if (rows <= 0 || d <= 0) ASR_FAIL(ASR_EINVAL, "asr_embed_bwd: bad shape");
    if (drop_p < 0.f || drop_p >= 1.f) ASR_FAIL(ASR_EINVAL, "asr_embed_bwd: bad dropout p=%f", drop_p);
    hipStream_t st = (hipStream_t)stream;
    const uint32_t thr = drop_thr16(drop_p);
    const float ds = 1.f / (1.f - drop_p);
    if (dtype != ASR_F32 && dtype != ASR_BF16) ASR_FAIL(ASR_EDTYPE, "asr_embed_bwd: dtype %d", dtype);
    if (asr_deterministic()) {
        if (dtype == ASR_F32) embed_bwd_serial_kernel<float><<<ceil_div(d, 256), 256, 0, st>>>(ids, (const float*)dy, (const float*)dy2, demb, scale, rows, d, V, drop_seed, thr, ds);
        else embed_bwd_serial_kernel<bf16_t><<<ceil_div(d, 256), 256, 0, st>>>(ids, (const bf16_t*)dy, (const bf16_t*)dy2, demb, scale, rows, d, V, drop_seed, thr, ds);
    } else if (dtype == ASR_F32) embed_bwd_kernel<float><<<rows, 256, 0, st>>>(ids, (const float*)dy, (const float*)dy2, demb, scale, d, V, drop_seed, thr, ds);
    else embed_bwd_kernel<bf16_t><<<rows, 256, 0, st>>>(ids, (const bf16_t*)dy, (const bf16_t*)dy2, demb, scale, d, V, drop_seed, thr, ds);
    ASR_CHECK_LAUNCH("asr_embed_bwd");
    return ASR_OK;
}

extern "C" int asr_dropout_mask(uint8_t* mask, int rows, int cols, float drop_p, uint32_t drop_seed, void* stream) {
    if (!mask || rows <= 0 || cols <= 0 || (cols & 1)) ASR_FAIL(ASR_EINVAL, "asr_dropout_mask: bad arguments (cols must be even)");
    const size_t n = (size_t)rows * cols;
    dropout_mask_kernel<<<(int)((n + 255) / 256 < 2048 ? (n + 255) / 256 : 2048), 256, 0, (hipStream_t)stream>>>(mask, (size_t)rows, cols, drop_seed, drop_thr16(drop_p));
    ASR_CHECK_LAUNCH("asr_dropout_mask");
    return ASR_OK;
}

extern "C" int asr_sdpa_dropout_mask(uint8_t* mask, int B, int H, int Tq, int Tk, float drop_p, uint32_t drop_seed, void* stream) {
    if (!mask || B <= 0 || H <= 0 || Tq <= 0 || Tk <= 0) ASR_FAIL(ASR_EINVAL, "asr_sdpa_dropout_mask: bad arguments");
    const size_t n = (size_t)B * H * Tq * Tk;
    dropout_mask_kernel<<<(int)((n + 255) / 256 < 2048 ? (n + 255) / 256 : 2048), 256, 0, (hipStream_t)stream>>>(mask, (size_t)B * H * Tq, Tk, drop_seed, drop_thr16(drop_p));
    ASR_CHECK_LAUNCH("asr_sdpa_dropout_mask");
    return ASR_OK;
}

extern "C" size_t asr_sumsq_workspace_bytes(size_t n) { return (size_t)ss_grid(n) * sizeof(float); }

extern "C" int asr_grad_sumsq(const float* g, size_t n, float* sumsq, void* ws, size_t ws_bytes, void* stream) {
    if (!g || !sumsq || !ws) ASR_FAIL(ASR_EINVAL, "asr_grad_sumsq: null pointer");
    if (ws_bytes < asr_sumsq_workspace_bytes(n)) ASR_FAIL(ASR_EWORKSPACE, "asr_grad_sumsq: workspace too small");
    if (((uintptr_t)g) % 16) ASR_FAIL(ASR_EINVAL, "asr_grad_sumsq: g must be 16-byte aligned");
    hipStream_t st = (hipStream_t)stream;
    const int grid = ss_grid(n);
    sumsq_partial_kernel<<<grid, SS_BLOCK, 0, st>>>(g, n / 4, n, (float*)ws);
    sum_finalize_kernel<<<1, 256, 0, st>>>((const float*)ws, grid, sumsq);
    ASR_CHECK_LAUNCH("asr_grad_sumsq");
    return ASR_OK;
}

extern "C" int asr_grad_sumsq_noam(const float* g, size_t n, float* sumsq, void* ws, size_t ws_bytes, int32_t* step, float* hyper, float model_size,
                                   float warmup, float factor, float lr_const, float b1, float b2, void* stream) {
    if (!g || !sumsq || !ws || !step || !hyper) ASR_FAIL(ASR_EINVAL, "asr_grad_sumsq_noam: null pointer");
    if (ws_bytes < asr_sumsq_workspace_bytes(n)) ASR_FAIL(ASR_EWORKSPACE, "asr_grad_sumsq_noam: workspace too small");
    if (((uintptr_t)g) % 16) ASR_FAIL(ASR_EINVAL, "asr_grad_sumsq_noam: g must be 16-byte aligned");
    hipStream_t st = (hipStream_t)stream;
    const int grid = ss_grid(n);
    sumsq_partial_kernel<<<grid, SS_BLOCK, 0, st>>>(g, n / 4, n, (float*)ws);
    sum_finalize_noam_kernel<<<1, 256, 0, st>>>((const float*)ws, grid, sumsq, step, hyper, model_size, warmup, factor, lr_const, b1, b2);
    ASR_CHECK_LAUNCH("asr_grad_sumsq_noam");
    return ASR_OK;
}

extern "C" int asr_noam_hyper(int32_t* step, float* hyper, float model_size, float warmup, float factor, float lr_const, float b1,
                              float b2, void* stream) {
    if (!step || !hyper) ASR_FAIL(ASR_EINVAL, "asr_noam_hyper: null pointer");
    noam_hyper_kernel<<<1, 1, 0, (hipStream_t)stream>>>(step, hyper, model_size, warmup, factor, lr_const, b1, b2);
    ASR_CHECK_LAUNCH("asr_noam_hyper");
    return ASR_OK;
}

extern "C" int asr_adam_step(float* p, float* g, float* m, float* v, void* p_lp, size_t n, const float* hyper, const float* sumsq,
                             float max_norm, float b1, float b2, float eps, int write_clipped, void* stream) {
    if (!p || !g || !m || !v || !hyper) ASR_FAIL(ASR_EINVAL, "asr_adam_step: null pointer");
    if (max_norm > 0.f && !sumsq) ASR_FAIL(ASR_EINVAL, "asr_adam_step: clipping needs sumsq");
    if ((((uintptr_t)p) | ((uintptr_t)g) | ((uintptr_t)m) | ((uintptr_t)v)) % 16) ASR_FAIL(ASR_EINVAL, "asr_adam_step: buffers must be 16-byte aligned");
    adam_kernel<<<ew_grid(n / 4), EW_BLOCK, 0, (hipStream_t)stream>>>(p, g, m, v, (bf16_t*)p_lp, n / 4, n, hyper, sumsq, max_norm, b1, b2, eps, write_clipped);
    ASR_CHECK_LAUNCH("asr_adam_step");
    return ASR_OK;
}

extern "C" int asr_loss_combine(const float* row_nll, int M, const float* n_valid, const float* nll, int B, float w_ce, float w_ctc,
                                float* loss, void* stream) {
    if (!loss || (row_nll && !n_valid)) ASR_FAIL(ASR_EINVAL, "asr_loss_combine: null pointer");
    loss_combine_kernel<<<1, 256, 0, (hipStream_t)stream>>>(row_nll, M, n_valid, nll, B, w_ce, w_ctc, loss);
    ASR_CHECK_LAUNCH("asr_loss_combine");
    return ASR_OK;
}
```

asr_chinese_e2e_amd/engine.py:

```python
import math
import os

import torch

import collections
import ctypes

from . import _lib
from . import kernels as K
from ._lib import ACT_NONE, ACT_RELU, ACT_RELU_MASK

ALIGN = 64


def positional_encoding(max_len, d_model):
    pe = torch.zeros(max_len, d_model)
    pos = torch.arange(0, max_len).unsqueeze(1).float()
    w = torch.exp(torch.arange(0, d_model, 2).float() * -(math.log(10000.0) / d_model))
    pe[:, 0::2] = torch.sin(pos * w)
    pe[:, 1::2] = torch.cos(pos * w)
    return pe.unsqueeze(0)


class FlatParams:
# ... 294 lines not shown
            _HELD.append(s)
            s = torch.cuda.Stream(device=device)
        if s.cuda_stream not in verdict:
            return -1
        pos, n, draws = order.index(s.cuda_stream), len(order), len(order) + 1
        if not any(verdict.values()):
            return -1
        while not verdict[order[(pos + 1) % n]]:
            torch.cuda.Stream(device=device)
            pos, draws = pos + 1, draws + 1
        return draws


def shared_stream(device, kind):
    dev = torch.device(device)
    if dev.index is None:
        dev = torch.device("cuda", torch.cuda.current_device())
    key = (dev.index, kind)
    if key not in _STREAMS:
        with torch.cuda.device(dev):
            avoid = [torch.cuda.current_stream()] + [s for (i, _), s in _STREAMS.items() if i == dev.index]
            _STREAMS[key] = pick_stream(dev, avoid, factory=(lambda: _side_stream(dev)) if kind.startswith("wgrad") else None)
    return _STREAMS[key]


_shared_stream = shared_stream


def registered_streams(device):
    dev = torch.device(device)
    idx = dev.index if dev.index is not None else torch.cuda.current_device()
    return [s for (i, _), s in _STREAMS.items() if i == idx]


def _side_stream(device):
    import ctypes
    from . import _lib
    with torch.cuda.device(device):
        h = ctypes.c_void_p()
        _lib.check(_lib.lib.asr_stream_create(-1, ctypes.byref(h)), "asr_stream_create")
    return torch.cuda.ExternalStream(h.value, device=device)


class Engine:
    PAD_HEAD_ROWS = True

    def __init__(self, flat, cfg, vocab_size, use_decoder, use_ctc, pe):
        self.flat, self.cfg = flat, cfg
        self.V = vocab_size
        self.use_decoder, self.use_ctc = use_decoder, use_ctc
        d, H, dk, ff = cfg.d_model, cfg.num_head, cfg.hidden_size, cfg.ff_size
        self.d, self.H, self.dk, self.ff = d, H, dk, ff
        self.d_in = cfg.n_mels * cfg.lfr_m
        self.L = cfg.layer_num
        self.dtype = torch.bfloat16 if flat.lp is not None else torch.float32
        self.pe = pe
        self.ws = K.Workspace(flat.device)
        self.ws_side = K.Workspace(flat.device)
        self.lin_in = Linear(flat, ["encoder.linear_in.weight"], ["encoder.linear_in.bias"], d, self.d_in)
        self.ln_in = LayerNormP(flat, "encoder.layer_norm_in")
        self.enc = [(MHA(flat, f"encoder.layer_stack.{i}.slf_attn.", H, dk, d), FFN(flat, f"encoder.layer_stack.{i}.pos_ffn.", d, ff))
                    for i in range(self.L)]
        if use_decoder:
            self.emb32 = flat.view(flat.p, "decoder.tgt_word_emb.weight")
            self.gemb = flat.view(flat.g, "decoder.tgt_word_emb.weight")
            self.prj = Linear(flat, ["decoder.tgt_word_emb.weight"], None, vocab_size, d)
            self.dec = [(MHA(flat, f"decoder.layer_stack.{i}.slf_attn.", H, dk, d), MHA(flat, f"decoder.layer_stack.{i}.enc_attn.", H, dk, d, cross=True),
                         FFN(flat, f"decoder.layer_stack.{i}.pos_ffn.", d, ff)) for i in range(self.L)]
            kvn = [f"decoder.layer_stack.{i}.enc_attn.{n}" for i in range(self.L) for n in ("w_ks", "w_vs")]
            self.kv_all = Linear(flat, [n + ".weight" for n in kvn], [n + ".bias" for n in kvn], self.L * 2 * H * dk, d)
            self.kv_all.tag = "kv_all"
        if use_ctc:
            self.ctc_lo = Linear(flat, ["ctc_lo.weight"], ["ctc_lo.bias"], vocab_size, d)
        self.ld_v = vocab_size
        if self.dtype == torch.bfloat16 and vocab_size % 8 == 0 and self.PAD_HEAD_ROWS:
            self.ld_v = (vocab_size + 63) // 64 * 64
        self.grad_ready = None
        self._tr_tiles = None
        if flat.lp is not None:
            lins = [l for mha, ffn in self.enc for l in (mha.qkv, mha.fc, ffn.w1, ffn.w2)]
            cross_qkv = [self.kv_all] if getattr(self, "dec", None) else []
            head = [self.ctc_lo] if use_ctc else []
            lins = [l for l in lins + cross_qkv + head if l.N % 8 == 0 and l.K % 8 == 0]
            n_flat = (flat.lp.numel() + 63) // 64 * 64
            pad_head = use_ctc and self.ld_v != self.V and self.ctc_lo in lins
            flat.lpT = torch.zeros(n_flat + (self.ctc_lo.K * self.ld_v if pad_head else 0), dtype=flat.lp.dtype, device=flat.device)
            tiles = []
            for l in lins:
                if pad_head and l is self.ctc_lo:
                    dst_off, ldd = n_flat, self.ld_v
                    l.wlpT = flat.lpT[n_flat:].view(l.K, ldd)[:, :l.N]
                else:
                    dst_off, ldd = l.w_off, l.N
                    l.wlpT = flat.lpT[l.w_off:l.w_off + l.N * l.K].view(l.K, l.N)
                tiles += [[l.w_off, l.N, l.K, (r << 16) | c, dst_off, ldd] for r in range((l.N + 63) // 64) for c in range((l.K + 63) // 64)]
            for i, (_, cross, _) in enumerate(self.dec if getattr(self, "dec", None) else []):
                if self.kv_all.wlpT is not None:
                    cross.kv.wlpT = self.kv_all.wlpT[:, i * cross.kv.N:(i + 1) * cross.kv.N]
            self._tr_tiles = torch.tensor(tiles, dtype=torch.int32, device=flat.device)
            self._tr_event = torch.cuda.Event()
            self._tr_pending = False
        self.side = _shared_stream(flat.device, "wgrad")
        self.ctc_stream = _shared_stream(flat.device, "aux")
        self.ws_ctc = K.Workspace(flat.device)
        self._side_handle = self.side.cuda_stream
        self._events, self._ev_next = [torch.cuda.Event() for _ in range(64)], 0
        self.overlap_wgrad = os.environ.get("ASR_WGRAD_OVERLAP", "1") == "1"
        self.deterministic = K.deterministic()
        if self.deterministic:
            self.overlap_wgrad = False
        self.overlap_ctc = self.aux_overlap = self.overlap_wgrad
        self.group_wgrad = os.environ.get("ASR_WGRAD_GROUP", "decoder")
        self.group_wgrad = None if (self.group_wgrad == "0" or self.deterministic) else self.group_wgrad
        self._pair_tags = {"pair": ("w2", "w1", "fc", "qkv"), "pair_ffn": ("w2", "w1"), "pair_attn": ("fc", "qkv")}.get(self.group_wgrad, ())
        self.dec_cu_limit = int(os.environ.get("ASR_DEC_CU_LIMIT", "192"))
        g = max(1, min(self.L, int(os.environ.get("ASR_KV_GROUPS", "3"))))
        cuts = [round(j * self.L / g) for j in range(g + 1)]
        self.kv_groups = [(cuts[j], cuts[j + 1]) for j in range(g) if cuts[j + 1] > cuts[j]]
        self._kv_ahead = None
        self._pending = []
        self._deferred = []
        self._keep = []
        self.defer_wgrad = tuple(t for t in os.environ.get("ASR_WGRAD_DEFER", "fc").split(",") if t)
        self.armed_fork = os.environ.get("ASR_ARMED_FORK", "1") == "1"
        self._armed = False
        self._arm_covers_pending = False
        self._ln_part, self._ln_pending = {}, []
        self.dec_exec = os.environ.get("ASR_DEC_EXEC", "1") == "1"
        self._dec_cache = collections.OrderedDict()
        self._block_flush = self.group_wgrad == "block"
        self._in_decoder = False
        self.drop_p = float(getattr(cfg, "dropout", 0.0))
        self.training = True
        self.step_seed = 0

    def _drop(self, site):
        if not self.training or self.drop_p <= 0.0:
            return 0.0, 0
        return self.drop_p, (self.step_seed * 0x9E3779B1 + site * 0x85EBCA77 + 0x165667B1) & 0xFFFFFFFF

    def _ready(self, name):
        if self.grad_ready is not None:
            self._release_deferred()
        self.flush_wgrads()
        if self.grad_ready is not None:
            self.flush_ln_reduce()
            streams = [torch.cuda.current_stream()] + ([self.side] if self.overlap_wgrad else [])
            self.grad_ready(self.flat.index[name][0], streams)

    def _ln_bwd(self, ln, dbias, dy, dy2, xhat, rstd, lens, B, T, **kw):
        d = xhat.shape[-1]
        need = K.add_ln_bwd_workspace_bytes(B * T, d)
        part = self._ln_part.get(id(ln))
        if part is None or part.numel() < need:
            part = self._ln_part[id(ln)] = torch.empty(need, dtype=torch.uint8, device=xhat.device)
        out = K.add_ln_bwd(dy, dy2, xhat, rstd, ln.g, lens, ln.gg, ln.gb, dbias, B, T, self.ws, partials=part, **kw)
        self._ln_pending.append((part, ln.gg, ln.gb, dbias, B * T))
        return out

    def flush_ln_reduce(self):
        if self._ln_pending:
            items, self._ln_pending = self._ln_pending, []
            K.add_ln_bwd_reduce_batched(items, self.d)

    def tail_mark_name(self):
        return "encoder.layer_stack.0.pos_ffn.w_1.weight"

    def _event(self):
        if torch.cuda.is_current_stream_capturing():
            return torch.cuda.Event()
        ev = self._events[self._ev_next]
        self._ev_next = (self._ev_next + 1) & 63
        return ev

    def _arm(self):
        if self.armed_fork and self.overlap_wgrad and not torch.cuda.is_current_stream_capturing() and not self._in_decoder:
            K.stream_arm(self._side_handle)
            self._armed = True

    def _disarm(self):
        if self._armed:
            self._armed = False
            K.stream_arm_pending()

    def _fork(self, stream):
        if self._armed:
            self._armed = False
            taken = not K.stream_arm_pending()
            if taken and stream is self.side:
                return
        if torch.cuda.is_current_stream_capturing():
            ev = torch.cuda.Event()
            ev.record()
            stream.wait_event(ev)
        else:
            K.stream_fork(stream.cuda_stream)

    def _release_kept(self, joined=False):
        if self._keep:
            if not joined and not torch.cuda.is_current_stream_capturing():
                cur = torch.cuda.current_stream()
                cur.wait_stream(self.side)
                cur.wait_stream(self.ctc_stream)
            self._keep.clear()

    def refresh_transposes(self, zero=None):
        if self._tr_tiles is None:
            if zero is not None:
                zero.zero_()
            return
        self._disarm()
        self._fork(self.side)
        if zero is not None:
            with torch.cuda.stream(self.side):
                zero.zero_()
        K.STREAM_OVERRIDE = self._side_handle
        try:
            K.transpose_batched(self.flat.lp, self.flat.lpT, self._tr_tiles)
        finally:
            K.STREAM_OVERRIDE = None
        self._tr_event.record(self.side)
        self._tr_pending = True
        self.flat.lpT_version = self.flat.version

    def wait_transposes(self):
        if self._tr_tiles is not None and self._tr_pending:
            torch.cuda.current_stream().wait_event(self._tr_event)

    def join_side(self):
        self._release_deferred()
        self.flush_wgrads()
        if self.overlap_wgrad:
            torch.cuda.current_stream().wait_stream(self.side)

    def flush_wgrads(self):
        if not self._pending:
            return
        probs, self._pending = self._pending, []
        if not self.overlap_wgrad:
            K.gemm_tn_grouped(probs, accumulate=True)
            return
        self._fork(self.side)
        K.STREAM_OVERRIDE = self._side_handle
        lim = self.dec_cu_limit if self._in_decoder else 0
        try:
            if lim:
                K.set_cu_limit(lim)
            K.gemm_tn_grouped(probs, accumulate=True)
        finally:
            K.STREAM_OVERRIDE = None
            if lim:
                K.set_cu_limit(0)
        for dy, x, _, _ in probs:
            self._keep += (dy, x)

    def _release_deferred(self):
        if self._deferred:
            items, self._deferred = self._deferred, []
            hold, self.defer_wgrad = self.defer_wgrad, ""
            try:
                for lin, dy, x, bias_from in items:
                    self._wgrad(lin, dy, x, bias_from)
            finally:
                self.defer_wgrad = hold

    def _wgrad(self, lin, dy, x, bias_from=None):
        pair = self._pair_tags and not self._in_decoder and lin.tag in self._pair_tags
        if self.defer_wgrad and self.overlap_wgrad and not self._in_decoder and lin.tag in self.defer_wgrad and not pair:
            self._deferred.append((lin, dy, x, bias_from))
            self._disarm()
            return
        fused = bias_from is dy and lin.fused_bias_wgrad(dy, x)
        grouped_here = self.group_wgrad and (self._in_decoder or pair or self.group_wgrad in ("layer", "block"))
        if grouped_here and (bias_from is None or fused) and dy.dtype == torch.bfloat16 and lin.N % 8 == 0 and lin.K % 8 == 0 \
                and dy.stride(0) % 8 == 0 and x.stride(0) % 8 == 0 and dy.data_ptr() % 16 == 0 and x.data_ptr() % 16 == 0:
            self._pending.append((dy, x, lin.gw, lin.gb if fused else None))
            if pair and lin.tag in ("w1", "qkv"):
                self.flush_wgrads()
            elif not self._arm_covers_pending:
                self._disarm()
            return
        if not self.overlap_wgrad:
            if bias_from is not None and not fused:
                lin.bgrad(bias_from, self.ws_side)
            lin.wgrad(dy, x, with_bias=fused, ws=self.ws_side)
            return
        self._fork(self.side)
        own = dy.dtype == torch.bfloat16 and lin.N % 8 == 0 and lin.K % 8 == 0 and dy.stride(0) % 8 == 0 and x.stride(0) % 8 == 0
        if own:
            K.STREAM_OVERRIDE = self._side_handle
            try:
                if bias_from is not None and not fused:
                    lin.bgrad(bias_from, self.ws_side)
                lin.wgrad(dy, x, with_bias=fused, ws=self.ws_side)
            finally:
                K.STREAM_OVERRIDE = None
        else:
            with torch.cuda.stream(self.side):
                if bias_from is not None and not fused:
                    lin.bgrad(bias_from, self.ws_side)
                lin.wgrad(dy, x, with_bias=fused)
        self._keep += (dy, x)

    def _attn_block_fwd(self, m, x, kv_src, B, Tq, Tk, k_len, q_lens, causal, window, cross, site, kv_pre=None):
        H, dk, hd = self.H, self.dk, self.H * self.dk
        c = {}
        if not cross:
            qkv = m.qkv.fwd(x)
            q, k, v = qkv[:, :hd], qkv[:, hd:2 * hd], qkv[:, 2 * hd:]
            c["qkv"] = qkv
        else:
            q = m.q.fwd(x)
            if kv_pre is not None:
                kv, ev = kv_pre
                torch.cuda.current_stream().wait_event(ev)
            else:
                kv = m.kv.fwd(kv_src)
            k, v = kv[:, :hd], kv[:, hd:]
            c["q"], c["kv"] = q, kv
        pa, sa = self._drop(site)
        pf, sf = self._drop(site + 1)
        ctx_lo = torch.empty(B * Tq, hd, dtype=q.dtype, device=q.device) if (Tk > 512 and q.dtype == torch.bfloat16 and torch.is_grad_enabled()) else None
        ctx, lse = K.sdpa_fwd(q, k, v, k_len, B, H, Tq, Tk, dk, causal, window, drop_p=pa, drop_seed=sa, o_lo=ctx_lo)
        a = m.fc.fwd(ctx)
        y, xhat, rstd = K.add_ln_fwd(a, x, m.ln.g, m.ln.b, None, q_lens, B, Tq, xhat=a, drop_p=pf, drop_seed=sf, drop_mode=1)
        c.update(x=x, kv_src=kv_src, ctx=ctx, ctx_lo=ctx_lo, lse=lse, xhat=xhat, rstd=rstd, k_len=k_len, q_lens=q_lens, dims=(B, Tq, Tk), causal=causal,
                 window=window, cross=cross, drop=(pa, sa, pf, sf))
        return y, c

    def _attn_block_bwd(self, m, c, dy, dy2, d_kv_src=None):
        H, dk, hd = self.H, self.dk, self.H * self.dk
        B, Tq, Tk = c["dims"]
        pa, sa, pf, sf = c["drop"]
        fc_deferred = bool(self.defer_wgrad) and self.overlap_wgrad and not self._in_decoder and m.fc.tag in self.defer_wgrad and "fc" not in self._pair_tags
        if not fc_deferred:
            self._arm()
        dz, dxg = self._ln_bwd(m.ln, m.fc.gb, dy, dy2, c["xhat"], c["rstd"], c["q_lens"], B, Tq, drop_p=pf, drop_seed=sf, drop_mode=1)
        self._wgrad(m.fc, dxg, c["ctx"])
        if fc_deferred and not c["cross"] and m.fc.own_dgrad(dxg):
            self._arm()
        dctx = m.fc.dgrad(dxg)
        if not c["cross"]:
            qkv = c["qkv"]
            dqkv = torch.empty_like(qkv)
            self._release_deferred()
            self._disarm()
            self._arm()
            K.sdpa_bwd(qkv[:, :hd], qkv[:, hd:2 * hd], qkv[:, 2 * hd:], c["ctx"], dctx, c["lse"], c["k_len"], B, H, Tq, Tk, dk,
                       dqkv[:, :hd], dqkv[:, hd:2 * hd], dqkv[:, 2 * hd:], c["causal"], c["window"], drop_p=pa, drop_seed=sa, o_lo=c["ctx_lo"])
            self._wgrad(m.qkv, dqkv, c["x"], bias_from=dqkv)
            dx = m.qkv.dgrad(dqkv)
        else:
            q, kv = c["q"], c["kv"]
            dq = torch.empty_like(q)
            dkv = torch.empty_like(kv)
            K.sdpa_bwd(q, kv[:, :hd], kv[:, hd:], c["ctx"], dctx, c["lse"], c["k_len"], B, H, Tq, Tk, dk, dq, dkv[:, :hd], dkv[:, hd:],
                       c["causal"], c["window"], drop_p=pa, drop_seed=sa, o_lo=c["ctx_lo"])
            self._wgrad(m.q, dq, c["x"], bias_from=dq)
            self._wgrad(m.kv, dkv, c["kv_src"], bias_from=dkv)
            dx = m.q.dgrad(dq)
            if self.aux_overlap and not torch.cuda.is_current_stream_capturing():
                self._fork(self.ctc_stream)
                with torch.cuda.stream(self.ctc_stream):
                    m.kv.dgrad(dkv, out=d_kv_src, accumulate=True)
                self._keep.append(dkv)
            else:
                m.kv.dgrad(dkv, out=d_kv_src, accumulate=True)
        if self._block_flush:
            self.flush_wgrads()
        return dx, dz

    def _ffn_block_fwd(self, f, x, B, T, lens, site):
        h = f.w1.fwd(x, act=ACT_RELU)
        pf, sf = self._drop(site)
        o = f.w2.fwd(h)
        y, xhat, rstd = K.add_ln_fwd(o, x, f.ln.g, f.ln.b, None, lens, B, T, xhat=o, drop_p=pf, drop_seed=sf, drop_mode=1)
        return y, dict(x=x, h=h, xhat=xhat, rstd=rstd, lens=lens, dims=(B, T), drop=(pf, sf))

    def _ffn_block_bwd(self, f, c, dy, dy2):
        B, T = c["dims"]
        pf, sf = c["drop"]
        self._arm()
        dz, dxg = self._ln_bwd(f.ln, f.w2.gb, dy, dy2, c["xhat"], c["rstd"], c["lens"], B, T, drop_p=pf, drop_seed=sf, drop_mode=1)
        self._wgrad(f.w2, dxg, c["h"])
        fused_relu = (f.w2.own_dgrad(dxg) or f.w2.small(dxg, f.w2.N) or dxg.dtype == torch.float32) and c["h"].is_contiguous() and c["h"].data_ptr() % 16 == 0
        if fused_relu and f.w2.own_dgrad(dxg):
            self._arm()
        dh = f.w2.dgrad(dxg, relu_mask=c["h"] if fused_relu else None)
        fused = f.w1.fused_bias_wgrad(dh, c["x"])
        if not fused_relu:
            self._disarm()
            K.relu_bwd_(dh, c["h"], None if fused else f.w1.gb, self.ws)
        elif not fused:
            f.w1.bgrad(dh, self.ws)
        self._wgrad(f.w1, dh, c["x"], bias_from=dh if fused else None)
        dx = f.w1.dgrad(dh)
        if self._block_flush:
            self.flush_wgrads()
        return dx, dz

    def encoder_fwd(self, wave, wave_len, window=-1):
        B, T, F = wave.shape
        self._deferred.clear()
        self._pending.clear()
        self._ln_pending.clear()
        self._disarm()
        self._release_kept()
        x_in = wave.reshape(B * T, F)
        e0 = self.lin_in.fwd(x_in)
        p0, s0 = self._drop(1)
        h, xhat, rstd = K.add_ln_fwd(e0, None, self.ln_in.g, self.ln_in.b, self.pe, None, B, T, xhat=e0, drop_p=p0, drop_seed=s0, drop_mode=2)
        cache = dict(x_in=x_in, xhat_in=xhat, rstd_in=rstd, B=B, T=T, layers=[], drop=(p0, s0))
        for i, (mha, ffn) in enumerate(self.enc):
            h1, c1 = self._attn_block_fwd(mha, h, h, B, T, T, wave_len, wave_len, False, window, False, site=10 + 4 * i)
            h, c2 = self._ffn_block_fwd(ffn, h1, B, T, wave_len, site=12 + 4 * i)
            cache["layers"].append((c1, c2))
        return h, cache

    def encoder_bwd(self, cache, d_enc):
        B, T = cache["B"], cache["T"]
        dy, dy2 = d_enc, None
        self.wait_transposes()
        for i in reversed(range(self.L)):
            mha, ffn = self.enc[i]
            c1, c2 = cache["layers"][i]
            dx, dz = self._ffn_block_bwd(ffn, c2, dy, dy2)
            if i == 0:
                self._ready(self.tail_mark_name())
            dx, dz = self._attn_block_bwd(mha, c1, dx, dz)
            dy, dy2 = dx, dz
            self._ready(f"encoder.layer_stack.{i}.slf_attn.w_qs.weight")
        p0, s0 = cache["drop"]
        dz, _ = self._ln_bwd(self.ln_in, self.lin_in.gb, dy, dy2, cache["xhat_in"], cache["rstd_in"], None, B, T, drop_p=p0, drop_seed=s0, drop_mode=2)
        self.lin_in.wgrad(dz, cache["x_in"], ws=self.ws)
        self._block_flush = self.group_wgrad == "block"
        self.flush_ln_reduce()
        self.join_side()
        self._release_kept(joined=True)
        self._ready("encoder.linear_in.weight")

    def ctc_branch_async(self, enc, wave_len, labels32, lab_len, B, T, grad_scale, grad_scale_div=None):
        main = torch.cuda.current_stream()
        self._fork(self.ctc_stream)
        with torch.cuda.stream(self.ctc_stream):
            if self.dec_cu_limit:
                K.set_cu_limit(self.dec_cu_limit)
            try:
                nll, d_enc = self.ctc_fwd_bwd(enc, wave_len, labels32, lab_len, B, T, grad_scale, grad_scale_div=grad_scale_div, ws=self.ws_ctc)
            finally:
                if self.dec_cu_limit:
                    K.set_cu_limit(0)
            done = torch.cuda.Event()
            done.record(self.ctc_stream)
        self._keep += (enc, wave_len, labels32, lab_len, nll, d_enc)
        return nll, d_enc, done

    def ctc_fwd_bwd(self, enc, wave_len, labels32, lab_len, B, T, grad_scale, want_grad=True, grad_scale_div=None, ws=None, best_path=None):
        buf = torch.empty(B * T, self.ld_v, dtype=enc.dtype, device=enc.device)
        ws = ws if ws is not None else self.ws
        logits = self.ctc_lo.fwd(enc, out=buf[:, :self.V])
        frames = buf.view(B, T, self.ld_v)[:, :, :self.V]
        if want_grad:
            self._arm()
        nll, dl = K.ctc_fwd_bwd(frames, wave_len, labels32, lab_len, ws, blank=0, grad_scale=grad_scale,
                                dlogits=frames if want_grad else None, want_grad=want_grad, grad_scale_div=grad_scale_div, best_path=best_path)
        if not want_grad:
            return nll, None
        dl = logits
        self._wgrad(self.ctc_lo, dl, enc, bias_from=dl)
        self.wait_transposes()
        d_enc = self.ctc_lo.dgrad(dl)
        if not self.use_decoder:
            self._ready("ctc_lo.weight")
        return nll, d_enc

    DEC_CACHE_SHAPES = 6

    def _dec_exec_ok(self, B, To, T):
        hd = self.H * self.dk
        return (self.dec_exec and self.dtype == torch.bfloat16 and K.TIMER is None and B * To <= Linear.SMALL_M and self.d % 8 == 0 and hd % 8 == 0
                and self.ff % 8 == 0 and max(3 * hd, self.ff, self.d) <= Linear.SMALL_REDUCE)

    def _dec_bufs(self, B, To, T, drop):
        key = (B, To, T, bool(drop))
        hit = self._dec_cache.get(key)
        capturing = torch.cuda.is_current_stream_capturing()
        if hit is not None:
            self._dec_cache.move_to_end(key)
            hit["pinned"] = hit["pinned"] or capturing
            return hit
        evictable = [k for k, v in self._dec_cache.items() if not v["pinned"]]
        while len(evictable) >= self.DEC_CACHE_SHAPES:
            del self._dec_cache[evictable.pop(0)]
        dev, M, d, hd, ff, H = self.flat.device, B * To, self.d, self.H * self.dk, self.ff, self.H
        bf = lambda *shape: torch.empty(*shape, dtype=torch.bfloat16, device=dev)
        f32 = lambda *shape: torch.empty(*shape, dtype=torch.float32, device=dev)
        part_bytes = K.add_ln_bwd_workspace_bytes(M, d)
        need = max(_lib.lib.asr_sdpa_bwd_workspace_bytes(B, H, To, T, self.dk, 0, -1, _lib.ASR_BF16), _lib.lib.asr_sdpa_bwd_workspace_bytes(B, H, To, To, self.dk, 1, -1, _lib.ASR_BF16))
        delta = f32((need + 3) // 4)
        layers = []
        kv_all, g_kv_all = bf(B * T, self.L * 2 * hd), bf(B * T, self.L * 2 * hd)
        for i, (slf, cross, ffn) in enumerate(self.dec):
            t = dict(qkv_s=bf(M, 3 * hd), ctx_s=bf(M, hd), a_s=bf(M, d), y_s=bf(M, d), lse_s=f32(B, H, To), rstd_s=f32(M),
                     q_c=bf(M, hd), kv_c=kv_all[:, i * 2 * hd:(i + 1) * 2 * hd], ctx_c=bf(M, hd), a_c=bf(M, d), y_c=bf(M, d), lse_c=f32(B, H, To), rstd_c=f32(M),
                     h=bf(M, ff), o=bf(M, d), y_f=bf(M, d), rstd_f=f32(M),
                     dz_f=bf(M, d), g_h=bf(M, ff), dx_f=bf(M, d), dz_c=bf(M, d), g_qc=bf(M, hd), g_kvc=g_kv_all[:, i * 2 * hd:(i + 1) * 2 * hd], dx_c=bf(M, d),
                     dz_s=bf(M, d), g_qkv=bf(M, 3 * hd), dx_s=bf(M, d), dctx=bf(M, hd),
                     part_f=torch.empty(part_bytes, dtype=torch.uint8, device=dev), part_c=torch.empty(part_bytes, dtype=torch.uint8, device=dev),
                     part_s=torch.empty(part_bytes, dtype=torch.uint8, device=dev))
            if drop:
                t.update(g_o=bf(M, d), g_ac=bf(M, d), g_as=bf(M, d))
            pl = _lib.DecLayerPlan()
            pl.B, pl.To, pl.T, pl.d, pl.H, pl.dk, pl.ff = B, To, T, d, H, self.dk, ff
            pl.ld_kv_c = self.L * 2 * hd
            for name, ten in t.items():
                setattr(pl, name, ten.data_ptr())
            for name, lin in (("qkv_s", slf.qkv), ("fc_s", slf.fc), ("q_c", cross.q), ("fc_c", cross.fc), ("1", ffn.w1), ("2", ffn.w2)):
                setattr(pl, "w_" + name, lin.wlp.data_ptr())
                setattr(pl, "b_" + name, lin.b32.data_ptr())
            for name, ln in (("s", slf.ln), ("c", cross.ln), ("f", ffn.ln)):
                setattr(pl, "g_" + name, ln.g.data_ptr())
                setattr(pl, "be_" + name, ln.b.data_ptr())
            pl.gb_2, pl.gb_fc_c, pl.gb_fc_s = ffn.w2.gb.data_ptr(), cross.fc.gb.data_ptr(), slf.fc.gb.data_ptr()
            if cross.kv.wlpT is not None:
                pl.w_kv_c_T, pl.ld_kv_c_T = cross.kv.wlpT.data_ptr(), cross.kv.wlpT.stride(0)
            pl.delta, pl.delta_bytes = delta.data_ptr(), delta.numel() * 4
            t["kv_event"] = torch.cuda.Event()
            layers.append((pl, t))
        hit = self._dec_cache[key] = dict(layers=layers, delta=delta, pinned=capturing, kv_all=kv_all, g_kv_all=g_kv_all, kv_event_rest=torch.cuda.Event())
        return hit

    def _kv_exec_async(self, bufs, enc):
        self._fork(self.ctc_stream)
        with torch.cuda.stream(self.ctc_stream):
            if self.dec_cu_limit:
                K.set_cu_limit(self.dec_cu_limit)
            try:
                n0 = self.dec[0][1].kv.N
                pl0, t0 = bufs["layers"][0]
                self.dec[0][1].kv.fwd(enc, out=t0["kv_c"])
                t0["kv_event"].record(self.ctc_stream)
                pl0.kv_ready_event = t0["kv_event"].cuda_event
                if self.L > 1:
                    self.kv_all.rows(n0, self.kv_all.N).fwd(enc, out=bufs["kv_all"][:, n0:])
                    bufs["kv_event_rest"].record(self.ctc_stream)
                    for pl, t in bufs["layers"][1:]:
                        pl.kv_ready_event = bufs["kv_event_rest"].cuda_event
            finally:
                if self.dec_cu_limit:
                    K.set_cu_limit(0)
        self._keep.append(enc)

    def decoder_kv_async(self, prep, enc, B, T):
        self._kv_ahead = None
        To = prep[0].shape[1]
        if not (self.aux_overlap and not torch.cuda.is_current_stream_capturing() and self._dec_exec_ok(B, To, T)):
            return
        bufs = self._dec_bufs(B, To, T, self.training and self.drop_p > 0.0)
        self._kv_exec_async(bufs, enc)
        self._kv_ahead = (bufs, enc)

    def _dec_exec_fwd(self, x, enc, dec_len, cross_len, B, To, T):
        drop = self.training and self.drop_p > 0.0
        bufs = self._dec_bufs(B, To, T, drop)
        main = K._stream()
        overlap = self.aux_overlap and not torch.cuda.is_current_stream_capturing()
        ahead, self._kv_ahead = self._kv_ahead, None
        if overlap and not (ahead is not None and ahead[0] is bufs and ahead[1] is enc):
            self._kv_exec_async(bufs, enc)
        for i, ((pl, t), (_, cross, _)) in enumerate(zip(bufs["layers"], self.dec)):
            if not overlap:
                cross.kv.fwd(enc, out=t["kv_c"])
                pl.kv_ready_event = None
            pl.x_in = x.data_ptr()
            pl.dec_len, pl.cross_len = dec_len.data_ptr(), cross_len.data_ptr()
            pl.drop_p = self.drop_p if drop else 0.0
            for j, site in enumerate((100 + 8 * i, 101 + 8 * i, 102 + 8 * i, 103 + 8 * i, 104 + 8 * i)):
                pl.seed[j] = self._drop(site)[1]
            _lib.check(_lib.fast.asr_decoder_layer_fwd(ctypes.addressof(pl), main), "asr_decoder_layer_fwd")
            t["x_in"] = x
            x = t["y_f"]
        return x, bufs

    def _dec_exec_bwd(self, bufs, dy, enc, d_enc, d_enc_ready):
        drop = self.training and self.drop_p > 0.0
        main = K._stream()
        aux = self.ctc_stream.cuda_stream if (self.aux_overlap and not torch.cuda.is_current_stream_capturing()) else None
        dy2 = None
        M = dy.shape[0]
        nkv = self.dec[0][1].kv.N
        groups = {lo: (lo, hi) for lo, hi in self.kv_groups}
        for i in reversed(range(self.L)):
            pl, t = bufs["layers"][i]
            slf, cross, ffn = self.dec[i]
            if cross.kv.wlpT is not None:
                cross.kv._fresh_transpose()
            if d_enc_ready is not None:
                torch.cuda.current_stream().wait_event(d_enc_ready)
                d_enc_ready = None
            grp = groups.get(i) if cross.kv.wlpT is not None else None
            pl.d_enc, pl.kv_dgrad_cols, pl.g_kv_group = None, 0, None
            if grp is not None:
                c0, c1 = grp[0] * nkv, grp[1] * nkv
                pl.d_enc, pl.kv_dgrad_cols = d_enc.data_ptr(), c1 - c0
                pl.g_kv_group = bufs["g_kv_all"][:, c0:].data_ptr()
                pl.w_kv_c_T, pl.ld_kv_c_T = self.kv_all.wlpT[:, c0:].data_ptr(), self.kv_all.wlpT.stride(0)
            hand_over = self.armed_fork and self.overlap_wgrad and not torch.cuda.is_current_stream_capturing()
            pl.wgrad_stream = self._side_handle if hand_over else None
            pl.aux_cus = self.dec_cu_limit if aux is not None else 0
            _lib.check(_lib.fast.asr_decoder_layer_bwd(ctypes.addressof(pl), dy.data_ptr(), None if dy2 is None else dy2.data_ptr(), main, aux),
                       "asr_decoder_layer_bwd")
            self._armed = self._arm_covers_pending = hand_over
            if cross.kv.wlpT is None:
                cross.kv.dgrad(t["g_kvc"], out=d_enc, accumulate=True)
            self._wgrad(ffn.w2, t["g_o"] if drop else t["dz_f"], t["h"])
            self._wgrad(ffn.w1, t["g_h"], t["y_c"], bias_from=t["g_h"])
            self._wgrad(cross.fc, t["g_ac"] if drop else t["dz_c"], t["ctx_c"])
            self._wgrad(cross.q, t["g_qc"], t["y_s"], bias_from=t["g_qc"])
            if cross.kv.wlpT is None:
                self._wgrad(cross.kv, t["g_kvc"], enc, bias_from=t["g_kvc"])
            elif grp is not None:
                c0, c1 = grp[0] * nkv, grp[1] * nkv
                g = bufs["g_kv_all"][:, c0:c1]
                self._wgrad(self.kv_all.rows(c0, c1), g, enc, bias_from=g)
            self._wgrad(slf.fc, t["g_as"] if drop else t["dz_s"], t["ctx_s"])
            self._wgrad(slf.qkv, t["g_qkv"], t["x_in"], bias_from=t["g_qkv"])
            self._ln_pending += [(t["part_f"], ffn.ln.gg, ffn.ln.gb, ffn.w2.gb, M), (t["part_c"], cross.ln.gg, cross.ln.gb, cross.fc.gb, M),
                                 (t["part_s"], slf.ln.gg, slf.ln.gb, slf.fc.gb, M)]
            dy, dy2 = t["dx_s"], t["dz_s"]
            self._ready(f"decoder.layer_stack.{i}.slf_attn.w_qs.weight")
            self._arm_covers_pending = False
        return dy, dy2

    def decoder_fwd(self, prep, enc, cross_len, B, T):
        ys_in, ys_out, labels32, dec_len, lab_len, n_valid = prep
        To = ys_in.shape[1]
        pe_, se_ = self._drop(2)
        x = K.embed_pe_fwd(ys_in.reshape(-1), self.emb32, self.pe, self.d ** -0.5, B, To, self.dtype, drop_p=pe_, drop_seed=se_)
        cache = dict(B=B, T=T, To=To, ys_in=ys_in, layers=[], drop=(pe_, se_))
        if self._dec_exec_ok(B, To, T):
            x, bufs = self._dec_exec_fwd(x, enc, dec_len, cross_len, B, To, T)
            cache.update(exec_bufs=bufs, enc=enc, keep=(dec_len, cross_len))
            pred = self.prj.fwd(x)
            cache["x_last"] = x
            return pred, cache
        kv_pre = [None] * self.L
        if self.aux_overlap and not torch.cuda.is_current_stream_capturing():
            self._fork(self.ctc_stream)
            with torch.cuda.stream(self.ctc_stream):
                for i, (slf, cross, ffn) in enumerate(self.dec):
                    kv = cross.kv.fwd(enc)
                    e = torch.cuda.Event()
                    e.record(self.ctc_stream)
                    kv_pre[i] = (kv, e)
            self._keep.append(enc)
            self._keep += [kv for kv, _ in kv_pre]
        for i, (slf, cross, ffn) in enumerate(self.dec):
            x1, c1 = self._attn_block_fwd(slf, x, x, B, To, To, dec_len, dec_len, True, -1, False, site=100 + 8 * i)
            x2, c2 = self._attn_block_fwd(cross, x1, enc, B, To, T, cross_len, dec_len, False, -1, True, site=102 + 8 * i, kv_pre=kv_pre[i])
            x, c3 = self._ffn_block_fwd(ffn, x2, B, To, dec_len, site=104 + 8 * i)
            cache["layers"].append((c1, c2, c3))
        pred = self.prj.fwd(x)
        cache["x_last"] = x
        return pred, cache

    def decoder_bwd(self, cache, dpred, d_enc, d_enc_ready=None):
        self._in_decoder = True
        self.wait_transposes()
        self._wgrad(self.prj, dpred, cache["x_last"])
        dy, dy2 = self.prj.dgrad(dpred), None
        if "exec_bufs" in cache:
            dy, dy2 = self._dec_exec_bwd(cache["exec_bufs"], dy, cache["enc"], d_enc, d_enc_ready)
        for i in (reversed(range(self.L)) if "exec_bufs" not in cache else ()):
            slf, cross, ffn = self.dec[i]
            c1, c2, c3 = cache["layers"][i]
            dx, dz = self._ffn_block_bwd(ffn, c3, dy, dy2)
            if d_enc_ready is not None:
                torch.cuda.current_stream().wait_event(d_enc_ready)
                d_enc_ready = None
            dx, dz = self._attn_block_bwd(cross, c2, dx, dz, d_kv_src=d_enc)
            dx, dz = self._attn_block_bwd(slf, c1, dx, dz)
            dy, dy2 = dx, dz
            self._ready(f"decoder.layer_stack.{i}.slf_attn.w_qs.weight")
        ids_flat, dyc, dy2c = cache["ys_in"].reshape(-1), dy.contiguous(), (dy2.contiguous() if dy2 is not None else None)
        self.flush_wgrads()
        if self.overlap_wgrad:
            self._disarm()
            self._fork(self.side)
            K.STREAM_OVERRIDE = self._side_handle
            try:
                K.embed_bwd(ids_flat, dyc, self.gemb, self.d ** -0.5, drop_p=cache["drop"][0], drop_seed=cache["drop"][1], dy2=dy2c)
            finally:
                K.STREAM_OVERRIDE = None
            self._keep += (ids_flat, dyc) + ((dy2c,) if dy2c is not None else ())
        else:
            K.embed_bwd(ids_flat, dyc, self.gemb, self.d ** -0.5, drop_p=cache["drop"][0], drop_seed=cache["drop"][1], dy2=dy2c)
        if self.aux_overlap and not torch.cuda.is_current_stream_capturing():
            torch.cuda.current_stream().wait_stream(self.ctc_stream)
        self._in_decoder = False
        self._ready("decoder.tgt_word_emb.weight")
        if self.use_ctc:
            self._ready("ctc_lo.weight")
```

asr_chinese_e2e_amd/kernels.py:

```python
import threading
import ctypes

import torch

from . import _lib
from ._lib import ASR_BF16, ASR_F32, ACT_NONE, ACT_RELU, LN_REDUCE_MAX, TN_GROUP_MAX, LnReduceItem, TnProblem, check
from ._lib import fast as lib

_DT = {torch.float32: ASR_F32, torch.bfloat16: ASR_BF16}


def _dt(t):
    try:
        return _DT[t.dtype]
    except KeyError:
        raise TypeError(f"unsupported dtype {t.dtype} (float32 or bfloat16)")


def _p(t):
    if t is None:
        return None
    if not t.is_cuda:
        raise ValueError("the HIP path needs CUDA (ROCm) tensors; there is no CPU fallback")
    return t.data_ptr()
# ... 204 lines not shown
        delta = torch.empty((need + 3) // 4, dtype=torch.float32, device=q.device)
    scale = float(dk) ** -0.5 if scale is None else float(scale)
    e = q.element_size()
    timed("sdpa_bwd", 10.0 * B * H * Tq * Tk * dk, lambda: check(
        lib.asr_sdpa_bwd(_p(q), _p(k), _p(v), _p(o), _p(do), _p(lse), _p(delta), delta.numel() * 4, _p(dq), _p(dk_), _p(dv), _p(k_len),
                         B, H, Tq, Tk, dk, ldq, ldk, ldv, ldo, int(causal), int(window), scale, float(drop_p),
                         int(drop_seed) & 0xFFFFFFFF, _p(o_lo), _dt(q), _stream()), "asr_sdpa_bwd"),
          B * H * (4.0 * Tq + 4.0 * Tk) * dk * e)
    return dq, dk_, dv


def _frame_rows(logits):
    B, T, V = logits.shape
    ld = logits.stride(1) if B * T > 1 else V
    assert logits.stride(2) == 1 and ld >= V and (B == 1 or logits.stride(0) == T * ld), f"frames must be rows of one (B*T, ld) buffer: {logits.stride()}"
    return ld


def ctc_fwd_bwd(logits, in_len, labels, lab_len, ws, blank=0, grad_scale=1.0, zero_infinity=False, dlogits=None,
                want_grad=True, nll=None, grad_scale_div=None, best_path=None):
    B, T, V = logits.shape
    ld = _frame_rows(logits)
    _chk_i32(in_len, labels, lab_len)
    Lmax = labels.shape[1]
    assert labels.shape[0] == B and in_len.numel() == B and lab_len.numel() == B
    nll = torch.empty(B, dtype=torch.float32, device=logits.device) if nll is None else nll
    if want_grad and dlogits is None:
        dlogits = torch.empty_strided(logits.shape, logits.stride(), dtype=logits.dtype, device=logits.device)
    if dlogits is not None:
        assert dlogits.shape == logits.shape and dlogits.stride() == logits.stride() and dlogits.dtype == logits.dtype
    w = ws.get(lib.asr_ctc_workspace_bytes(B, T, Lmax))
    _chk_f32(grad_scale_div)
    _chk_i32(best_path)
    assert best_path is None or best_path.numel() == B * T
    timed("ctc", 0.0, lambda: check(
        lib.asr_ctc_fwd_bwd(_p(logits), _p(dlogits), _p(in_len), _p(labels), _p(lab_len), _p(nll), B, T, V, ld, Lmax,
                            int(blank), float(grad_scale), _p(grad_scale_div), int(zero_infinity), _p(best_path), _p(w), w.numel(), _dt(logits), _stream()),
        "asr_ctc_fwd_bwd"), (3.0 if dlogits is not None else 1.0) * logits.numel() * logits.element_size())

    return nll, dlogits


def ctc_align(logits, in_len, labels, lab_len, blank=0, ws=None):
    B, T, V = logits.shape
    ld = _frame_rows(logits)
    _chk_i32(in_len, labels, lab_len)
    assert labels.dim() == 2 and labels.shape[0] == B and in_len.numel() == B and lab_len.numel() == B
    Lmax = labels.shape[1]
    dev = logits.device
    lab = labels if Lmax > 0 else torch.zeros(B, 1, dtype=torch.int32, device=dev)
    La = lab.shape[1]
    path = torch.empty(B, T, dtype=torch.int32, device=dev)
    spans = torch.empty(B, La, 2, dtype=torch.int32, device=dev)
    token_logp = torch.empty(B, La, dtype=torch.float32, device=dev)
    score = torch.empty(B, dtype=torch.float32, device=dev)
    nbytes = lib.asr_ctc_align_workspace_bytes(B, T, La)
    w = ws.get(nbytes) if ws is not None else torch.empty(max(nbytes, 16), dtype=torch.uint8, device=dev)
    timed("ctc_align", 0.0, lambda: check(
        lib.asr_ctc_align(_p(logits), _p(in_len), _p(lab), _p(lab_len), _p(path), _p(spans), _p(token_logp), _p(score), B, T, V, ld, La,
                          int(blank), _p(w), w.numel(), _dt(logits), _stream()),
        "asr_ctc_align"), logits.numel() * logits.element_size())
    return path, spans[:, :Lmax], token_logp[:, :Lmax], score


def ctc_greedy_decode(logits, in_len, blank=0):
    B, T, V = logits.shape
    ld = _frame_rows(logits)
    _chk_i32(in_len)
    ids = torch.empty(B, T, dtype=torch.int32, device=logits.device)
    lens = torch.empty(B, dtype=torch.int32, device=logits.device)
    check(lib.asr_ctc_greedy_decode(_p(logits), _p(in_len), _p(ids), _p(lens), B, T, V, ld, int(blank), _dt(logits), _stream()),
          "asr_ctc_greedy_decode")
    return ids, lens


def ctc_collapse(path, in_len, blank=0):
    B, T = path.shape
    _chk_i32(path, in_len)
    lens = torch.empty(B, dtype=torch.int32, device=path.device)
    check(lib.asr_ctc_collapse(_p(path), _p(in_len), _p(lens), B, T, int(blank), _stream()), "asr_ctc_collapse")
    return path, lens


def decode_attn(q, k, v, H, dk, Tk_cap, kv_div=1, k_len=None, k_len_uniform=0, len_div=1, scale=None, o=None):
    R = q.shape[0]
    ldq, ldk, ldv = _strided_rows(q, H, dk), _strided_rows(k, H, dk), _strided_rows(v, H, dk)
    assert q.dtype == k.dtype == v.dtype
    _chk_i32(k_len)
    o = torch.empty(R, H * dk, dtype=q.dtype, device=q.device) if o is None else o
    scale = float(dk) ** -0.5 if scale is None else float(scale)
    check(lib.asr_decode_attn(_p(q), _p(k), _p(v), _p(o), _p(k_len), int(k_len_uniform), int(len_div), R, H, dk, int(Tk_cap), int(kv_div),
                              ldq, ldk, ldv, _strided_rows(o, H, dk), scale, _dt(q), _stream()), "asr_decode_attn")
    return o


def logsoftmax_topk(logits, beam):
    R, V = logits.shape
    assert logits.stride(1) == 1
    vals = torch.empty(R, beam, dtype=torch.float32, device=logits.device)
    ids = torch.empty(R, beam, dtype=torch.int32, device=logits.device)
    check(lib.asr_logsoftmax_topk(_p(logits), _p(vals), _p(ids), R, V, logits.stride(0), int(beam), _dt(logits), _stream()), "asr_logsoftmax_topk")
    return vals, ids


def ctc_frame_topk(logits, k, blank=0):
    R, V = logits.shape
    assert logits.stride(1) == 1
    vals = torch.empty(R, k, dtype=torch.float32, device=logits.device)
    ids = torch.empty(R, k, dtype=torch.int32, device=logits.device)
    blank_lp = torch.empty(R, dtype=torch.float32, device=logits.device)
    check(lib.asr_ctc_frame_topk(_p(logits), _p(vals), _p(ids), _p(blank_lp), R, V, logits.stride(0), int(k), int(blank), _dt(logits), _stream()),
          "asr_ctc_frame_topk")
    return vals, ids, blank_lp


def ctc_prefix_beam(vals, ids, blank_lp, in_len, B, T, beam, nbest, blank=0, max_len=None):
    k = vals.shape[1]
    assert vals.shape == (B * T, k) and ids.shape == (B * T, k) and blank_lp.numel() == B * T
    _chk_f32(vals, blank_lp)
    _chk_i32(ids, in_len)
    Lcap = int(T if max_len is None else max_len)
    ws = torch.empty(lib.asr_ctc_prefix_beam_workspace_bytes(B, T, beam), dtype=torch.uint8, device=vals.device)
    out_tok = torch.zeros(B, nbest, Lcap, dtype=torch.int32, device=vals.device)
    out_len = torch.empty(B, nbest, dtype=torch.int32, device=vals.device)
    out_score = torch.empty(B, nbest, dtype=torch.float32, device=vals.device)
    check(lib.asr_ctc_prefix_beam(_p(vals), _p(ids), _p(blank_lp), _p(in_len), _p(ws), ws.numel(), _p(out_tok), _p(out_len), _p(out_score),
                                  B, T, k, int(beam), int(nbest), Lcap, int(blank), _stream()), "asr_ctc_prefix_beam")
    return out_tok, out_len, out_score


def beam_step(top_vals, top_ids, score, alive, last_tok, parent, rec_tok, rec_par, rec_end, rec_score, maxlen, alive_total, B, beam, step, eos):
    _chk_f32(top_vals, score, rec_score)
    _chk_i32(top_ids, alive, last_tok, parent, rec_tok, rec_par, rec_end, maxlen, alive_total)
    check(lib.asr_beam_step(_p(top_vals), _p(top_ids), _p(score), _p(alive), _p(last_tok), _p(parent), _p(rec_tok), _p(rec_par), _p(rec_end),
                            _p(rec_score), _p(maxlen), _p(alive_total), B, beam, int(step), int(eos), _stream()), "asr_beam_step")


def cache_gather(src, dst, parent, L, R, beam, Lcap, n_pos, row_bytes):
    _chk_i32(parent)
    check(lib.asr_cache_gather(_p(src), _p(dst), _p(parent), L, R, beam, Lcap, int(n_pos), int(row_bytes), _stream()), "asr_cache_gather")


def ctc_prefix_logprobs(logits):
    B, T, V = logits.shape
    ld = _frame_rows(logits)
    lpT = torch.empty(B, V, T, dtype=torch.float32, device=logits.device)
    check(lib.asr_ctc_prefix_logprobs(_p(logits), _p(lpT), B, T, V, ld, _dt(logits), _stream()), "asr_ctc_prefix_logprobs")
    return lpT


def ctc_prefix_score(lpT, in_len, st_rb, st_rt, hyp_psi, last_tok, alive, att_vals, att_ids, cand_rb, cand_rt, beam, step, ctc_weight,
                     eos, blank=0, out=None):
    B, V, T = lpT.shape
    R, C = att_ids.shape
    assert R == B * beam and att_vals.shape == (R, C) and lpT.is_contiguous()
    assert cand_rb.shape == cand_rt.shape == (T, R * C) and cand_rb.dtype == cand_rt.dtype == torch.float64
    assert step == 0 or (st_rb.shape == st_rt.shape == (T, R) and st_rb.dtype == st_rt.dtype == torch.float64)
    _chk_f32(lpT, att_vals, hyp_psi)
    _chk_i32(in_len, last_tok, alive, att_ids)
    if out is None:
        dev = lpT.device
        out = (torch.empty(R, beam, dtype=torch.float32, device=dev), torch.empty(R, beam, dtype=torch.int32, device=dev),
               torch.empty(R, beam, dtype=torch.float32, device=dev), torch.empty(R, beam, dtype=torch.float32, device=dev),
               torch.empty(R, beam, dtype=torch.float32, device=dev))
    vals, ids, att, psi, full = out
    check(lib.asr_ctc_prefix_score(_p(lpT), _p(in_len), _p(st_rb), _p(st_rt), _p(hyp_psi), _p(last_tok), _p(alive), _p(att_vals), _p(att_ids),
                                   _p(cand_rb), _p(cand_rt), _p(vals), _p(ids), _p(att), _p(psi), _p(full), B, T, V, int(beam), C, int(step),
                                   float(ctc_weight), int(eos), int(blank), _stream()), "asr_ctc_prefix_score")
    return out


def ctc_prefix_gather(cand_rb, cand_rt, st_rb, st_rt, parent, last_tok, alive, att_ids, in_len, B, beam):
    T, R = st_rb.shape
    C = att_ids.shape[1]
    assert R == B * beam and cand_rb.shape == cand_rt.shape == (T, R * C) and st_rt.shape == (T, R)
    _chk_i32(parent, last_tok, alive, att_ids, in_len)
    check(lib.asr_ctc_prefix_gather(_p(cand_rb), _p(cand_rt), _p(st_rb), _p(st_rt), _p(parent), _p(last_tok), _p(alive), _p(att_ids), _p(in_len),
                                    B, T, int(beam), C, _stream()), "asr_ctc_prefix_gather")


def joint_beam_step(top, score, att_score, ctc_score, alive, last_tok, parent, rec_tok, rec_par, rec_end, rec_score, rec_att, rec_ctc, maxlen,
                    alive_total, B, beam, step, eos, ctc_weight):
    vals, ids, att, psi, full = top
    _chk_f32(vals, att, psi, full, score, att_score, ctc_score, rec_score, rec_att, rec_ctc)
    _chk_i32(ids, alive, last_tok, parent, rec_tok, rec_par, rec_end, maxlen, alive_total)
    check(lib.asr_joint_beam_step(_p(vals), _p(ids), _p(att), _p(psi), _p(full), _p(score), _p(att_score), _p(ctc_score), _p(alive), _p(last_tok),
                                  _p(parent), _p(rec_tok), _p(rec_par), _p(rec_end), _p(rec_score), _p(rec_att), _p(rec_ctc), _p(maxlen),
                                  _p(alive_total), B, beam, int(step), int(eos), float(ctc_weight), _stream()), "asr_joint_beam_step")


def xent_fwd_bwd(logits, gold, n_valid, ignore_index=0, smoothing=0.0, grad_scale=1.0, dlogits=None, want_grad=True,
                 row_nll=None, argmax=None):
    M, V = logits.shape
    assert logits.is_contiguous() and gold.numel() == M
    _chk_i32(gold, argmax)
    assert argmax is None or argmax.numel() == M
    _chk_f32(n_valid)
    row_nll = torch.empty(M, dtype=torch.float32, device=logits.device) if row_nll is None else row_nll
    if want_grad and dlogits is None:
        dlogits = torch.empty_like(logits)
    timed("xent", 0.0, lambda: check(
        lib.asr_xent_fwd_bwd(_p(logits), _p(gold), _p(n_valid), _p(row_nll), _p(dlogits), M, V, int(ignore_index),
                             float(smoothing), float(grad_scale), _p(argmax), _dt(logits), _stream()), "asr_xent_fwd_bwd"),
          (3.0 if dlogits is not None else 1.0) * logits.numel() * logits.element_size())
    return row_nll, dlogits


def loss_combine(row_nll, n_valid, nll, w_ce, w_ctc, out=None):
    dev = (row_nll if row_nll is not None else nll).device
    out = torch.empty(3, dtype=torch.float32, device=dev) if out is None else out
    M = row_nll.numel() if row_nll is not None else 0
    B = nll.numel() if nll is not None else 0
    check(lib.asr_loss_combine(_p(row_nll), M, _p(n_valid), _p(nll), B, float(w_ce), float(w_ctc), _p(out), _stream()),
          "asr_loss_combine")
    return out


def dec_preprocess(tgt, sos=2, eos=3, lens64=()):
    assert tgt.dtype == torch.int64 and tgt.is_contiguous() and tgt.dim() == 2
    B, Lmax = tgt.shape
    dev = tgt.device
    lens64 = tuple(lens64)
    assert len(lens64) <= 2 and all(t.dtype == torch.int64 and t.is_contiguous() and t.numel() == B and t.device == dev for t in lens64)
    lens32 = tuple(torch.empty(B, dtype=torch.int32, device=dev) for _ in lens64)
    la, lb = (list(zip(lens64, lens32)) + [(None, None), (None, None)])[:2]
    ys_in = torch.empty(B, Lmax + 1, dtype=torch.int32, device=dev)
    ys_out = torch.empty(B, Lmax + 1, dtype=torch.int32, device=dev)
    labels32 = torch.empty(B, Lmax, dtype=torch.int32, device=dev)
    dec_len = torch.empty(B, dtype=torch.int32, device=dev)
    lab_len = torch.empty(B, dtype=torch.int32, device=dev)
    n_valid = torch.empty(1, dtype=torch.float32, device=dev)
    check(lib.asr_dec_preprocess(_p(tgt), _p(ys_in), _p(ys_out), _p(labels32), _p(dec_len), _p(lab_len), _p(n_valid),
                                 B, Lmax, sos, eos, _p(la[0]), _p(la[1]), _p(lb[0]), _p(lb[1]), _stream()), "asr_dec_preprocess")
    if lens64:
        return ys_in, ys_out, labels32, dec_len, lab_len, n_valid, lens32
    return ys_in, ys_out, labels32, dec_len, lab_len, n_valid


def embed_pe_fwd(ids, emb, pe, scale, B, To, dtype, y=None, drop_p=0.0, drop_seed=0):
    V, d = emb.shape
    _chk_i32(ids)
    _chk_f32(emb, pe)
    assert ids.numel() == B * To and pe.shape[-1] == d and pe.shape[-2] >= To
    y = torch.empty(B * To, d, dtype=dtype, device=emb.device) if y is None else y
    check(lib.asr_embed_pe_fwd(_p(ids), _p(emb), _p(pe), _p(y), float(scale), B, To, d, V, float(drop_p),
                               int(drop_seed) & 0xFFFFFFFF, _dt(y), _stream()), "asr_embed_pe_fwd")
    return y


def embed_bwd(ids, dy, demb, scale, drop_p=0.0, drop_seed=0, dy2=None):
    V, d = demb.shape
    _chk_i32(ids)
    _chk_f32(demb)
    assert dy.is_contiguous() and dy.shape[-1] == d and dy.numel() == ids.numel() * d
    assert dy2 is None or (dy2.is_contiguous() and dy2.shape == dy.shape and dy2.dtype == dy.dtype)
    check(lib.asr_embed_bwd(_p(ids), _p(dy), _p(dy2), _p(demb), float(scale), ids.numel(), d, V, float(drop_p),
                            int(drop_seed) & 0xFFFFFFFF, _dt(dy), _stream()), "asr_embed_bwd")


def dropout_mask(rows, cols, drop_p, drop_seed, device="cuda"):
    m = torch.empty(rows, cols, dtype=torch.uint8, device=device)
    check(lib.asr_dropout_mask(_p(m), rows, cols, float(drop_p), int(drop_seed) & 0xFFFFFFFF, _stream()), "asr_dropout_mask")
    return m


def sdpa_dropout_mask(B, H, Tq, Tk, drop_p, drop_seed, device="cuda"):
    m = torch.empty(B, H, Tq, Tk, dtype=torch.uint8, device=device)
    check(lib.asr_sdpa_dropout_mask(_p(m), B, H, Tq, Tk, float(drop_p), int(drop_seed) & 0xFFFFFFFF, _stream()), "asr_sdpa_dropout_mask")
    return m


def relu_(x):
    assert x.is_contiguous()
    check(lib.asr_relu_fwd(_p(x), x.numel(), _dt(x), _stream()), "asr_relu_fwd")
    return x


def relu_bwd_(da, a, dbias, ws):
    assert da.is_contiguous() and a.is_contiguous() and da.shape == a.shape and da.dtype == a.dtype and da.dim() == 2
    _chk_f32(dbias)
    rows, cols = da.shape
    w = ws.get(lib.asr_colsum_workspace_bytes(rows, cols))
    check(lib.asr_relu_bwd(_p(da), _p(a), _p(dbias), _p(w), w.numel(), rows, cols, _dt(da), _stream()), "asr_relu_bwd")
    return da


def colsum(x, out, ws, accumulate=True):
    assert x.dim() == 2 and x.stride(1) == 1
    _chk_f32(out)
    rows, cols = x.shape
    assert out.numel() == cols
    w = ws.get(lib.asr_colsum_workspace_bytes(rows, cols))
    check(lib.asr_colsum(_p(x), _p(out), _p(w), w.numel(), rows, cols, x.stride(0), int(accumulate), _dt(x), _stream()),
          "asr_colsum")
    return out


def cast(src, dst):
    assert src.is_contiguous() and dst.is_contiguous() and src.numel() == dst.numel()
    check(lib.asr_cast(_p(src), _p(dst), src.numel(), _dt(src), _dt(dst), _stream()), "asr_cast")
    return dst


def grad_sumsq(g, out, ws):
    _chk_f32(g, out)
    w = ws.get(lib.asr_sumsq_workspace_bytes(g.numel()))
    timed("grad_sumsq", 0.0, lambda: check(lib.asr_grad_sumsq(_p(g), g.numel(), _p(out), _p(w), w.numel(), _stream()), "asr_grad_sumsq"), 4.0 * g.numel())
    return out


def grad_sumsq_noam(g, out, ws, step, hyper, model_size, warmup, factor, lr_const, b1, b2):
    _chk_f32(g, out, hyper)
    _chk_i32(step)
    assert hyper.numel() >= 4
    w = ws.get(lib.asr_sumsq_workspace_bytes(g.numel()))
    timed("grad_sumsq", 0.0, lambda: check(lib.asr_grad_sumsq_noam(_p(g), g.numel(), _p(out), _p(w), w.numel(), _p(step), _p(hyper), float(model_size),
                                                                   float(warmup), float(factor), float(lr_const), float(b1), float(b2), _stream()),
                                           "asr_grad_sumsq_noam"), 4.0 * g.numel())
    return out


def noam_hyper(step, hyper, model_size, warmup, factor, lr_const, b1, b2):
    _chk_i32(step)
    _chk_f32(hyper)
    assert hyper.numel() >= 4
    check(lib.asr_noam_hyper(_p(step), _p(hyper), float(model_size), float(warmup), float(factor), float(lr_const),
                             float(b1), float(b2), _stream()), "asr_noam_hyper")


def adam_step(p, g, m, v, p_lp, hyper, sumsq, max_norm, b1, b2, eps, write_clipped=True):
    _chk_f32(p, g, m, v, hyper, sumsq)
    n = p.numel()
    assert g.numel() == n and m.numel() == n and v.numel() == n
    if p_lp is not None:
        assert p_lp.dtype == torch.bfloat16 and p_lp.numel() == n and p_lp.is_contiguous()
    timed("adam", 0.0, lambda: check(
        lib.asr_adam_step(_p(p), _p(g), _p(m), _p(v), _p(p_lp), n, _p(hyper), _p(sumsq), float(max_norm), float(b1),
                          float(b2), float(eps), int(write_clipped), _stream()), "asr_adam_step"),
          (28.0 + (4.0 if write_clipped else 0.0) + (2.0 if p_lp is not None else 0.0)) * n)


def gemm_nt_supported(M, N, K, lda, ldb, ldc):
    return K % 8 == 0 and lda % 8 == 0 and ldb % 8 == 0 and ldc % 4 == 0


def transpose_batched(src, dst, tiles):
    assert src.dtype == dst.dtype == torch.bfloat16 and tiles.dtype == torch.int32 and tiles.is_contiguous() and tiles.shape[1] == 6
    check(lib.asr_transpose_batched_bf16(_p(src), _p(dst), _p(tiles), tiles.shape[0], _stream()), "asr_transpose_batched_bf16")


def gemm_nt(a, w, bias, out, act=ACT_NONE, res=None, family="gemm_nt"):
    assert a.dtype == w.dtype == out.dtype == torch.bfloat16
    M, K = a.shape
    N = w.shape[0]
    assert w.shape[1] == K and out.shape == (M, N) and a.stride(1) == 1 and w.stride(1) == 1 and out.stride(1) == 1
    _chk_f32(bias)
    if res is not None:
        assert res.dtype == torch.bfloat16 and res.shape == out.shape and res.stride() == out.stride()
    timed(family, 2.0 * M * N * K, lambda: check(
        lib.asr_gemm_nt_bf16(_p(a), _p(w), _p(bias), _p(res), _p(out), M, N, K, a.stride(0), w.stride(0), out.stride(0), int(act),
                             _stream()), "asr_gemm_nt_bf16"))
    return out


_CU_LIMIT_NAME = ctypes.create_string_buffer(b"cu_limit")


def set_cu_limit(n):
    check(lib.asr_set_option(ctypes.addressof(_CU_LIMIT_NAME), int(n), None), "asr_set_option")


def set_option(name, value):
    prev = ctypes.c_int(0)
    check(_lib.lib.asr_set_option(name.encode(), int(value), ctypes.byref(prev)), "asr_set_option")
    return prev.value


def deterministic():
    return bool(lib.asr_get_deterministic())


def set_deterministic(on):
    return bool(lib.asr_set_deterministic(int(bool(on))))


def gemm_f32(a, b, out, bias=None, trans_a=False, trans_b=False, act=ACT_NONE, mask=None, accumulate=False):
    assert a.dtype == b.dtype == out.dtype == torch.float32 and a.stride(1) == 1 and b.stride(1) == 1 and out.stride(1) == 1
    M, N = out.shape
    K = a.shape[0] if trans_a else a.shape[1]
    assert a.shape == ((K, M) if trans_a else (M, K)) and b.shape == ((N, K) if trans_b else (K, N)), (a.shape, b.shape, out.shape)
    _chk_f32(bias)
    if mask is not None:
        assert mask.dtype == torch.float32 and mask.shape == out.shape and mask.stride() == out.stride()
    timed("gemm_f32", 2.0 * M * N * K, lambda: check(
        lib.asr_gemm_f32(_p(a), _p(b), _p(bias), _p(mask), _p(out), M, N, K, a.stride(0), b.stride(0), out.stride(0), int(trans_a), int(trans_b), int(act),
                         int(accumulate), _stream()), "asr_gemm_f32"))
    return out


def gemm_small(a, bm, bias, out, trans_b=False, act=ACT_NONE, mask=None):
    M, K = a.shape
    N = out.shape[1]
    assert a.dtype == bm.dtype == out.dtype == torch.bfloat16 and out.shape[0] == M
    assert bm.shape == ((K, N) if trans_b else (N, K)) and a.stride(1) == 1 and bm.stride(1) == 1 and out.stride(1) == 1
    _chk_f32(bias)
    if mask is not None:
        assert mask.dtype == torch.bfloat16 and mask.shape == out.shape and mask.stride() == out.stride()
    timed("gemm_small", 2.0 * M * N * K, lambda: check(
        lib.asr_gemm_small_bf16(_p(a), _p(bm), _p(bias), _p(mask), _p(out), M, N, K, a.stride(0), bm.stride(0), out.stride(0), int(trans_b), int(act),
                                _stream()), "asr_gemm_small_bf16"))
    return out


def gemm_tn(dy, x, dw, accumulate=True, dbias=None, ws=None):
    assert dy.dtype == x.dtype == torch.bfloat16 and dw.dtype == torch.float32
    M, N = dy.shape
    K = x.shape[1]
    assert x.shape[0] == M and dw.shape == (N, K) and dy.stride(1) == 1 and x.stride(1) == 1 and dw.stride(1) == 1
    _chk_f32(dbias)
    assert dbias is None or dbias.numel() == N
    need = lib.asr_gemm_tn_workspace_bytes(M, N, K)
    w = None
    if need:
        w = ws.get(need) if ws is not None else torch.empty(need, dtype=torch.uint8, device=dy.device)
    timed("gemm_tn", 2.0 * M * N * K, lambda: check(
        lib.asr_gemm_tn_bias_bf16(_p(dy), _p(x), _p(dw), _p(dbias), M, N, K, dy.stride(0), x.stride(0), dw.stride(0), int(accumulate), _p(w),
                                  w.numel() if w is not None else 0, _stream()), "asr_gemm_tn_bias_bf16"))
    return dw


_TN_SIZE = ctypes.sizeof(TnProblem)
_TN_BUF = (ctypes.c_char * (_TN_SIZE * TN_GROUP_MAX))()
_TN_ADDR = ctypes.addressof(_TN_BUF)
_TN_PACK = __import__("struct").Struct("<QQQQiiiiii").pack_into
assert _TN_SIZE == 56


def gemm_tn_grouped(problems, accumulate=True):
    for i in range(0, len(problems), TN_GROUP_MAX):
        chunk = problems[i:i + TN_GROUP_MAX]
        flops = 0.0
        for j, (dy, x, dw, dbias) in enumerate(chunk):
            assert dy.dtype == x.dtype == torch.bfloat16 and dw.dtype == torch.float32
            M, N = dy.shape
            Kd = x.shape[1]
            assert x.shape[0] == M and dw.shape == (N, Kd) and dy.stride(1) == 1 and x.stride(1) == 1 and dw.stride(1) == 1
            _chk_f32(dbias)
            assert dbias is None or dbias.numel() == N
            _TN_PACK(_TN_BUF, j * _TN_SIZE, _p(dy), _p(x), _p(dw), _p(dbias) or 0, M, N, Kd, dy.stride(0), x.stride(0), dw.stride(0))
            flops += 2.0 * M * N * Kd
        timed("gemm_tn", flops, lambda: check(lib.asr_gemm_tn_grouped_bf16(_TN_ADDR, len(chunk), int(accumulate), _stream()),
                                              "asr_gemm_tn_grouped_bf16"))


def token_table(id2token, device):
    cps, off = [], [0]
    for tok in id2token:
        cps.extend(ord(c) for c in tok)
        off.append(len(cps))
    mx = max((off[i + 1] - off[i] for i in range(len(id2token))), default=0)
    return (torch.tensor(cps if cps else [0], dtype=torch.int32, device=device), torch.tensor(off, dtype=torch.int32, device=device), mx)


def cer(hyp, ref, table, pad_id, hyp_len=None, ref_len=None):
    tok_cp, tok_off, mx = table
    _chk_i32(hyp, ref, hyp_len, ref_len)
    assert hyp.dim() == 2 and ref.dim() == 2 and hyp.shape[0] == ref.shape[0] and hyp.stride(1) == 1 and ref.stride(1) == 1
    B = hyp.shape[0]
    out = torch.empty(B, dtype=torch.float32, device=hyp.device)
    check(lib.asr_cer(_p(hyp), _p(hyp_len), hyp.shape[1], hyp.stride(0), _p(ref), _p(ref_len), ref.shape[1], ref.stride(0), _p(tok_cp), _p(tok_off),
                      tok_off.numel() - 1, mx, int(pad_id), B, _p(out), _stream()), "asr_cer")
    return out


def logmel(wav, wav_len, window, melfb, Tmax, feat=None):
    _chk_f32(wav, window, melfb)
    _chk_i32(wav_len)
    B, Smax = wav.shape
    n_mels = melfb.shape[1]
    assert melfb.shape[0] == 201 and window.numel() == 400 and wav_len.numel() == B
    feat = torch.empty(B, Tmax, n_mels, dtype=torch.float32, device=wav.device) if feat is None else feat
    check(lib.asr_logmel_fwd(_p(wav), _p(wav_len), _p(window), _p(melfb), _p(feat), B, Smax, Tmax, n_mels, _stream()),
          "asr_logmel_fwd")
    return feat


def utt_norm_lfr(feat, wav_len, m, n, Tlfr_max, dtype=torch.float32, masks=None):
    _chk_f32(feat)
    _chk_i32(wav_len, masks)
    B, Tmax, n_mels = feat.shape
    assert masks is None or tuple(masks.shape) == (B, 4)
    out = torch.empty(B, Tlfr_max, m * n_mels, dtype=dtype, device=feat.device)
    out_len = torch.empty(B, dtype=torch.int32, device=feat.device)
    check(lib.asr_utt_norm_augment_lfr_fwd(_p(feat), _p(wav_len), _p(masks), _p(out), _p(out_len), B, Tmax, n_mels, m, n, Tlfr_max,
                                           _dt(out), _stream()), "asr_utt_norm_augment_lfr_fwd")
    return out, out_len
```

include/asr_hip.h:

```cpp
#ifndef ASR_HIP_H
#define ASR_HIP_H

#include <stddef.h>
#include <stdint.h>

#ifdef __cplusplus
extern "C" {
#endif

#define ASR_ABI_VERSION 10

typedef enum { ASR_F32 = 0, ASR_BF16 = 1 } asr_dtype_t;

#define ASR_OK 0
#define ASR_EINVAL (-1)
#define ASR_EDTYPE (-2)
#define ASR_EWORKSPACE (-3)
#define ASR_EHIP (-4)

#define ASR_ACT_NONE 0
#define ASR_ACT_RELU 1
#define ASR_ACT_RELU_MASK 2

int asr_abi_version(void);
int asr_last_error(char* buf, size_t n);
int asr_stream_fork(void* from_stream, void* to_stream);
int asr_stream_arm(void* from_stream, void* to_stream);
int asr_stream_arm_pending(void);
int asr_stream_create(int priority, void** out_stream);
int asr_set_option(const char* name, int value, int* previous);
int asr_get_deterministic(void);
int asr_set_deterministic(int on);

#define ASR_DROP_PRE 1
#define ASR_DROP_POST 2
int asr_add_ln_fwd(const void* x, const void* res, const float* gamma, const float* beta,
                   const float* pe, const int32_t* lens, void* y, void* xhat, float* rstd,
                   int B, int T, int d, float drop_p, uint32_t drop_seed, int drop_mode, int dtype,
                   void* stream);

size_t asr_add_ln_bwd_workspace_bytes(int rows, int d);
int asr_add_ln_bwd(const void* dy, const void* dy2, const void* xhat, const float* rstd,
                   const float* gamma, const int32_t* lens, void* dz, void* dx, float* dgamma,
                   float* dbeta, float* dbias, void* ws, size_t ws_bytes, int B, int T, int d,
                   float drop_p, uint32_t drop_seed, int drop_mode, int dtype, void* stream);
#define ASR_LN_REDUCE_MAX 16
typedef struct asr_ln_reduce_item {
    const void* ws;
    float* dgamma;
    float* dbeta;
    float* dbias;
    int rows;
} asr_ln_reduce_item;
int asr_add_ln_bwd_reduce_batched(const asr_ln_reduce_item* items, int n, int d, void* stream);

int asr_sdpa_fwd(const void* q, const void* k, const void* v, void* o, float* lse,
                 const int32_t* k_len, int B, int H, int Tq, int Tk, int dk, int ldq, int ldk,
                 int ldv, int ldo, int causal, int window, float scale, float drop_p,
                 uint32_t drop_seed, void* o_lo, int dtype, void* stream);

size_t asr_sdpa_bwd_workspace_bytes(int B, int H, int Tq, int Tk, int dk, int causal, int window, int dtype);
int asr_sdpa_bwd(const void* q, const void* k, const void* v, const void* o, const void* d_o,
                 const float* lse, float* delta, size_t delta_bytes, void* dq, void* dk_, void* dv,
                 const int32_t* k_len, int B, int H, int Tq, int Tk, int dk, int ldq, int ldk,
                 int ldv, int ldo, int causal, int window, float scale, float drop_p,
                 uint32_t drop_seed, const void* o_lo, int dtype, void* stream);

int asr_dropout_mask(uint8_t* mask, int rows, int cols, float drop_p, uint32_t drop_seed, void* stream);
int asr_sdpa_dropout_mask(uint8_t* mask, int B, int H, int Tq, int Tk, float drop_p, uint32_t drop_seed, void* stream);

size_t asr_ctc_workspace_bytes(int B, int T, int Lmax);
int asr_ctc_fwd_bwd(const void* logits, void* dlogits, const int32_t* in_len,
                    const int32_t* labels, const int32_t* lab_len, float* nll, int B, int T, int V, int ld,
                    int Lmax, int blank, float grad_scale, const float* grad_scale_div, int zero_infinity,
                    int32_t* best_path, void* ws, size_t ws_bytes, int dtype, void* stream);

size_t asr_ctc_align_workspace_bytes(int B, int T, int Lmax);
int asr_ctc_align(const void* logits, const int32_t* in_len, const int32_t* labels, const int32_t* lab_len, int32_t* path,
                  int32_t* spans, float* token_logp, float* score, int B, int T, int V, int ld, int Lmax, int blank, void* ws,
                  size_t ws_bytes, int dtype, void* stream);

int asr_ctc_greedy_decode(const void* logits, const int32_t* in_len, int32_t* out_ids,
                          int32_t* out_len, int B, int T, int V, int ld, int blank, int dtype, void* stream);
int asr_ctc_frame_argmax(const void* logits, const int32_t* in_len, int32_t* path, int B, int T, int V, int ld, int blank,
                         int dtype, void* stream);
int asr_ctc_collapse(int32_t* ids, const int32_t* in_len, int32_t* out_len, int B, int T, int blank, void* stream);

int asr_ctc_frame_topk(const void* logits, float* vals, int32_t* ids, float* blank_lp, int R, int V, int ld, int k,
                       int blank, int dtype, void* stream);
size_t asr_ctc_prefix_beam_workspace_bytes(int B, int T, int beam);
int asr_ctc_prefix_beam(const float* vals, const int32_t* ids, const float* blank_lp, const int32_t* in_len, void* ws, size_t ws_bytes,
                        int32_t* out_tok, int32_t* out_len, float* out_score, int B, int T, int k, int beam, int nbest, int Lcap,
                        int blank, void* stream);
int asr_decode_attn(const void* q, const void* k, const void* v, void* o, const int32_t* k_len,
                    int k_len_uniform, int len_div, int R, int H, int dk, int Tk_cap, int kv_div,
                    int ldq, int ldk, int ldv, int ldo, float scale, int dtype, void* stream);
int asr_logsoftmax_topk(const void* logits, float* vals, int32_t* ids, int R, int V, int ld,
                        int beam, int dtype, void* stream);
int asr_beam_step(const float* top_vals, const int32_t* top_ids, float* score, int32_t* alive,
                  int32_t* last_tok, int32_t* parent, int32_t* rec_tok, int32_t* rec_par,
                  int32_t* rec_end, float* rec_score, const int32_t* maxlen, int32_t* alive_total,
                  int B, int beam, int step, int eos, void* stream);
int asr_cache_gather(const void* src, void* dst, const int32_t* parent, int L, int R, int beam,
                     int Lcap, int n_pos, int row_bytes, void* stream);

int asr_ctc_prefix_logprobs(const void* logits, float* lpT, int B, int T, int V, int ld, int dtype, void* stream);
int asr_ctc_prefix_score(const float* lpT, const int32_t* in_len, const double* st_rb, const double* st_rt, const float* hyp_psi,
                         const int32_t* last_tok, const int32_t* alive, const float* att_vals, const int32_t* att_ids, double* cand_rb,
                         double* cand_rt, float* out_vals, int32_t* out_ids, float* out_att, float* out_psi, float* out_full, int B, int T,
                         int V, int beam, int C, int step, float ctc_weight, int eos, int blank, void* stream);
int asr_ctc_prefix_gather(const double* cand_rb, const double* cand_rt, double* st_rb, double* st_rt, const int32_t* parent,
                          const int32_t* last_tok, const int32_t* alive, const int32_t* att_ids, const int32_t* in_len, int B, int T,
                          int beam, int C, void* stream);
int asr_joint_beam_step(const float* top_vals, const int32_t* top_ids, const float* top_att, const float* top_psi, const float* top_full,
                        float* score, float* att_score, float* ctc_score, int32_t* alive, int32_t* last_tok, int32_t* parent, int32_t* rec_tok,
                        int32_t* rec_par, int32_t* rec_end, float* rec_score, float* rec_att, float* rec_ctc, const int32_t* maxlen,
                        int32_t* alive_total, int B, int beam, int step, int eos, float ctc_weight, void* stream);

int asr_cer(const int32_t* hyp, const int32_t* hyp_len, int Lh, int ldh, const int32_t* ref,
            const int32_t* ref_len, int Lr, int ldr, const int32_t* tok_cp, const int32_t* tok_off,
            int V, int max_tok_len, int pad_id, int B, float* per_utt, void* stream);

int asr_xent_fwd_bwd(const void* logits, const int32_t* gold, const float* n_valid,
                     float* row_nll, void* dlogits, int M, int V, int ignore_index,
                     float smoothing, float grad_scale, int32_t* argmax_out, int dtype, void* stream);

int asr_dec_preprocess(const int64_t* tgt, int32_t* ys_in, int32_t* ys_out, int32_t* labels32,
                       int32_t* dec_len, int32_t* lab_len, float* n_valid, int B, int Lmax, int sos, int eos,
                       const int64_t* len_a, int32_t* len32_a, const int64_t* len_b, int32_t* len32_b, void* stream);

int asr_embed_pe_fwd(const int32_t* ids, const void* emb, const float* pe, void* y, float scale,
                     int B, int To, int d, int V, float drop_p, uint32_t drop_seed, int dtype,
                     void* stream);
int asr_embed_bwd(const int32_t* ids, const void* dy, const void* dy2, float* demb, float scale, int rows, int d,
                  int V, float drop_p, uint32_t drop_seed, int dtype, void* stream);

int asr_relu_fwd(void* x, size_t n, int dtype, void* stream);
int asr_relu_bwd(void* da, const void* a, float* dbias, void* ws, size_t ws_bytes, int rows,
                 int cols, int dtype, void* stream);
size_t asr_colsum_workspace_bytes(int rows, int cols);
int asr_colsum(const void* x, float* out, void* ws, size_t ws_bytes, int rows, int cols, int ld,
               int accumulate, int dtype, void* stream);
int asr_cast(const void* src, void* dst, size_t n, int src_dtype, int dst_dtype, void* stream);
int asr_transpose_batched_bf16(const void* src, void* dst, const int32_t* tiles, int ntiles, void* stream);

size_t asr_sumsq_workspace_bytes(size_t n);
int asr_grad_sumsq(const float* g, size_t n, float* sumsq, void* ws, size_t ws_bytes, void* stream);
int asr_noam_hyper(int32_t* step, float* hyper, float model_size, float warmup, float factor,
                   float lr_const, float b1, float b2, void* stream);
int asr_grad_sumsq_noam(const float* g, size_t n, float* sumsq, void* ws, size_t ws_bytes, int32_t* step, float* hyper, float model_size,
                        float warmup, float factor, float lr_const, float b1, float b2, void* stream);
int asr_adam_step(float* p, float* g, float* m, float* v, void* p_lp, size_t n,
                  const float* hyper, const float* sumsq, float max_norm, float b1, float b2,
                  float eps, int write_clipped, void* stream);
int asr_loss_combine(const float* row_nll, int M, const float* n_valid, const float* nll, int B,
                     float w_ce, float w_ctc, float* loss, void* stream);

int asr_gemm_nt_bf16(const void* A, const void* W, const float* bias, const void* res, void* C,
                     int M, int N, int K, int lda, int ldb, int ldc, int act, void* stream);
int asr_gemm_small_bf16(const void* A, const void* Bm, const float* bias, const void* mask, void* C, int M, int N, int K,
                        int lda, int ldb, int ldc, int trans_b, int act, void* stream);
int asr_gemm_f32(const float* A, const float* B, const float* bias, const float* mask, float* C, int M, int N, int K,
                 int lda, int ldb, int ldc, int trans_a, int trans_b, int act, int accumulate, void* stream);
size_t asr_gemm_tn_workspace_bytes(int M, int N, int K);
int asr_gemm_tn_bf16(const void* dY, const void* X, float* dW, int M, int N, int K, int ldy,
                     int ldx, int ldw, int accumulate, void* ws, size_t ws_bytes, void* stream);
int asr_gemm_tn_bias_bf16(const void* dY, const void* X, float* dW, float* dbias, int M, int N, int K,
                          int ldy, int ldx, int ldw, int accumulate, void* ws, size_t ws_bytes,
                          void* stream);
typedef struct asr_tn_problem {
    const void* dY;
    const void* X;
    float* dW;
    float* dbias;
    int M, N, K, ldy, ldx, ldw;
} asr_tn_problem;
int asr_gemm_tn_grouped_bf16(const asr_tn_problem* probs, int nprob, int accumulate, void* stream);

typedef struct asr_dec_layer_plan {
    int B, To, T, d, H, dk, ff;
    float drop_p;
    uint32_t seed[5];
    int ld_kv_c_T;
    const int32_t* dec_len;
    const int32_t* cross_len;
    const void *w_qkv_s, *w_fc_s, *w_q_c, *w_fc_c, *w_1, *w_2;
    const float *b_qkv_s, *b_fc_s, *b_q_c, *b_fc_c, *b_1, *b_2;
    const float *g_s, *be_s, *g_c, *be_c, *g_f, *be_f;
    const void* w_kv_c_T;
    const void* x_in;
    void *qkv_s, *ctx_s, *a_s, *y_s;
    float *lse_s, *rstd_s;
    void* q_c;
    const void* kv_c;
    void* kv_ready_event;
    void *ctx_c, *a_c, *y_c;
    float *lse_c, *rstd_c;
    void *h, *o, *y_f;
    float* rstd_f;
    void *dz_f, *g_o, *g_h, *dx_f;
    void *dz_c, *g_ac, *g_qc, *g_kvc, *dx_c;
    void *dz_s, *g_as, *g_qkv, *dx_s;
    void* dctx;
    float *gb_2, *gb_fc_c, *gb_fc_s;
    void *part_f, *part_c, *part_s;
    float* delta;
    size_t delta_bytes;
    void* d_enc;
    void* wgrad_stream;
    int aux_cus;
    int ld_kv_c;
    int kv_dgrad_cols;
    const void* g_kv_group;
    void *ctx_s_lo, *ctx_c_lo;
} asr_dec_layer_plan;
int asr_decoder_layer_fwd(const asr_dec_layer_plan* plan, void* stream);
int asr_decoder_layer_bwd(const asr_dec_layer_plan* plan, const void* dy, const void* dy2, void* stream, void* aux_stream);

int asr_logmel_fwd(const float* wav, const int32_t* wav_len, const float* window,
                   const float* melfb, float* feat, int B, int Smax, int Tmax, int n_mels,
                   void* stream);
int asr_utt_norm_lfr_fwd(const float* feat, const int32_t* wav_len, void* out, int32_t* out_len,
                         int B, int Tmax, int n_mels, int m, int n, int Tlfr_max, int dtype,
                         void* stream);
int asr_utt_norm_augment_lfr_fwd(const float* feat, const int32_t* wav_len, const int32_t* masks,
                                 void* out, int32_t* out_len, int B, int Tmax, int n_mels, int m,
                                 int n, int Tlfr_max, int dtype, void* stream);

#ifdef __cplusplus
}
#endif
#endif
```

Measured before the change: 6467 utterances/s.

## Compact encoder rows for cross-attention KV when the mask limits keys to target length

In ref_compat cross-mask mode, cross-attention keys are masked by target length, so only the first rows of each utterance's encoder output can ever be attended. The change gathers those rows (target width rounded up to 16) into a compact buffer. The cross-attention K/V projection, attention and KV dgrad/wgrad then run on that buffer, and a new scatter-add kernel folds the gradient back into the full encoder gradient. This removes most of the cross-KV GEMM and attention work over all T=500 frames, at the cost of extra gather/scatter kernels, new plan fields, and a guard on tgt_len versus padded width.

After: 6917 utterances/s (median of 6 runs). 1.07x the previous value.

```diff
diff --git a/asr_chinese_e2e_amd/Models/transformer_official.py b/asr_chinese_e2e_amd/Models/transformer_official.py
--- a/asr_chinese_e2e_amd/Models/transformer_official.py
+++ b/asr_chinese_e2e_amd/Models/transformer_official.py
@@ -206,12 +206,20 @@
             self._tgt_len32 = None
             return eng, x, self._len32_of(input.wave_len, (), ()).contiguous(), None
         tgt = input.tgt_for_input.contiguous()
+        tl = input.tgt_len
+        if self.cross_mask == "ref_compat" and tl is not None and tl.device.type == "cpu" and tl.numel() and int(tl.max()) > tgt.shape[1]:
+            raise ValueError(f"tgt_len {int(tl.max())} exceeds the padded target width {tgt.shape[1]} of tgt_for_input")
         lens64 = [t.contiguous() for t in (input.wave_len, input.tgt_len) if t is not None and t.dtype == torch.int64 and t.device == tgt.device]
         out = K.dec_preprocess(tgt, SOS_ID, EOS_ID, lens64=lens64)
         prep, lens32 = out[:6], (out[6] if lens64 else ())
         wave_len = self._len32_of(input.wave_len, lens64, lens32)
         self._tgt_len32 = self._len32_of(input.tgt_len, lens64, lens32) if input.tgt_len is not None else None
         return eng, x, wave_len, prep
+
+    def _cross(self, eng, input, wave_len, T):
+        if self.cross_mask == "ref_compat":
+            return self._tgt_len32, eng.cross_rows(input.tgt_for_input.shape[1], T, self._tgt_len32 is not None)
+        return wave_len, T
 
     @staticmethod
     def _len32_of(t, lens64, lens32):
@@ -227,8 +235,8 @@
         pack = Pack()
         pack.add(encoder_out=enc.view(B, T, -1))
         if self.use_decoder and prep is not None:
-            cross_len = self._tgt_len32 if self.cross_mask == "ref_compat" else wave_len
-            pred, _ = eng.decoder_fwd(prep, enc, cross_len, B, T)
+            cross_len, Tk = self._cross(eng, input, wave_len, T)
+            pred, _ = eng.decoder_fwd(prep, enc, cross_len, B, T, Tk)
             pack.add(pred=pred.view(B, -1, self.V), gold=prep[1].long())
         if self.use_ctc:
             logits = eng.ctc_lo.fwd(enc)
@@ -447,12 +455,13 @@
         ctc_done = None
         ctc_scale = dict(grad_scale=lam * loss_scale, grad_scale_div=batch_div) if batch_div is not None else dict(grad_scale=lam * loss_scale / float(B))
         ctc_async = (self.use_decoder and self.use_ctc and eng.overlap_ctc and not eng.deterministic and not torch.cuda.is_current_stream_capturing())
+        if self.use_decoder:
+            cross_len, Tk = self._cross(eng, input, wave_len, T)
         if ctc_async:
-            eng.decoder_kv_async(prep, enc, B, T)
+            eng.decoder_kv_async(prep, enc, B, T, Tk)
             nll, d_enc, ctc_done = eng.ctc_branch_async(enc, wave_len, labels32, lab_len, B, T, **ctc_scale)
         if self.use_decoder:
-            cross_len = self._tgt_len32 if self.cross_mask == "ref_compat" else wave_len
-            pred, dcache = eng.decoder_fwd(prep, enc, cross_len, B, T)
+            pred, dcache = eng.decoder_fwd(prep, enc, cross_len, B, T, Tk)
             ids = torch.empty(ys_out.shape, dtype=torch.int32, device=pred.device) if self.cer_in_iterate else None
             w_ce = (1.0 - lam) if self.use_ctc else 1.0
             row_nll, dpred = K.xent_fwd_bwd(pred, ys_out.reshape(-1), n_valid, PAD_ID, smoothing=self.label_smoothing, grad_scale=w_ce * loss_scale, dlogits=pred,
diff --git a/asr_chinese_e2e_amd/_lib.py b/asr_chinese_e2e_amd/_lib.py
--- a/asr_chinese_e2e_amd/_lib.py
+++ b/asr_chinese_e2e_amd/_lib.py
@@ -44,7 +44,8 @@
                                   "dz_s", "g_as", "g_qkv", "dx_s",
                                   "dctx", "gb_2", "gb_fc_c", "gb_fc_s",
                                   "part_f", "part_c", "part_s", "delta")] +
-                [("delta_bytes", Z), ("d_enc", P), ("wgrad_stream", P), ("aux_cus", I), ("ld_kv_c", I), ("kv_dgrad_cols", I), ("g_kv_group", P), ("ctx_s_lo", P), ("ctx_c_lo", P)])
+                [("delta_bytes", Z), ("d_enc", P), ("wgrad_stream", P), ("aux_cus", I), ("ld_kv_c", I), ("kv_dgrad_cols", I), ("g_kv_group", P), ("ctx_s_lo", P), ("ctx_c_lo", P),
+                 ("w_kv_c", P), ("g_enc_x", P), ("T_enc", I)])
 
 SIGNATURES = {
     "asr_abi_version": (I, []),
@@ -92,6 +93,8 @@
     "asr_colsum_workspace_bytes": (Z, [I, I]),
     "asr_colsum": (I, [P, P, P, Z, I, I, I, I, I, P]),
     "asr_cast": (I, [P, P, Z, I, I, P]),
+    "asr_rows_gather": (I, [P, P, I, I, I, I, I, P]),
+    "asr_rows_scatter_add": (I, [P, P, I, I, I, I, I, P]),
     "asr_sumsq_workspace_bytes": (Z, [Z]),
     "asr_grad_sumsq": (I, [P, Z, P, P, Z, P]),
     "asr_noam_hyper": (I, [P, P, F, F, F, F, F, F, P]),
diff --git a/asr_chinese_e2e_amd/csrc/decoder_exec.hip b/asr_chinese_e2e_amd/csrc/decoder_exec.hip
--- a/asr_chinese_e2e_amd/csrc/decoder_exec.hip
+++ b/asr_chinese_e2e_amd/csrc/decoder_exec.hip
@@ -67,9 +67,11 @@
     DEC_TRY(asr_gemm_small_bf16(dxg_c, p->w_fc_c, nullptr, nullptr, p->dctx, M, hd, d, d, hd, hd, 1, ASR_ACT_NONE, stream));
     char* kv = (char*)p->kv_c;
     char* gkv = (char*)p->g_kvc;
-    const bool kv_dgrad = p->d_enc && p->w_kv_c_T;
+    const bool compact = p->g_enc_x != nullptr;
+    const bool kv_dgrad = p->d_enc && (compact ? p->w_kv_c != nullptr : p->w_kv_c_T != nullptr);
     const int ldkv = p->ld_kv_c > 0 ? p->ld_kv_c : 2 * hd;
     if (p->kv_dgrad_cols > 0 && (!p->g_kv_group || p->kv_dgrad_cols % 8 || p->kv_dgrad_cols > ldkv)) ASR_FAIL(ASR_EINVAL, "asr_decoder_layer_bwd: kv_dgrad_cols = %d needs g_kv_group, a multiple of 8, <= ld_kv_c = %d", p->kv_dgrad_cols, ldkv);
+    if (compact && p->T_enc < T) ASR_FAIL(ASR_EINVAL, "asr_decoder_layer_bwd: T_enc = %d < T = %d key rows", p->T_enc, T);
     if (kv_dgrad && aux_stream) DEC_TRY(asr_stream_arm(stream, aux_stream));
     DEC_TRY(asr_sdpa_bwd(p->q_c, kv, kv + hd * e, p->ctx_c, p->dctx, p->lse_c, p->delta, p->delta_bytes, p->g_qc, gkv, gkv + hd * e, p->cross_len, B, H, To, T, dk, hd,
                          ldkv, ldkv, hd, 0, -1, scale, p->drop_p, p->seed[2], p->ctx_c_lo, ASR_BF16, stream));
@@ -79,7 +81,13 @@
         const int old_lim = p->aux_cus > 0 ? asr_option_set(ASR_OPT_CU_LIMIT, p->aux_cus) : 0;
         const void* g_a = p->kv_dgrad_cols > 0 ? p->g_kv_group : p->g_kvc;
         const int cols = p->kv_dgrad_cols > 0 ? p->kv_dgrad_cols : 2 * hd;
-        const int rc_kv = asr_gemm_nt_bf16(g_a, p->w_kv_c_T, nullptr, p->d_enc, p->d_enc, B * T, d, cols, ldkv, p->ld_kv_c_T, d, ASR_ACT_NONE, st2);
+        int rc_kv;
+        if (compact) {
+            rc_kv = asr_gemm_small_bf16(g_a, p->w_kv_c, nullptr, nullptr, p->g_enc_x, B * T, d, cols, ldkv, d, d, 1, ASR_ACT_NONE, st2);
+            if (rc_kv == ASR_OK) rc_kv = asr_rows_scatter_add(p->g_enc_x, p->d_enc, B, p->T_enc, T, d, ASR_BF16, st2);
+        } else {
+            rc_kv = asr_gemm_nt_bf16(g_a, p->w_kv_c_T, nullptr, p->d_enc, p->d_enc, B * T, d, cols, ldkv, p->ld_kv_c_T, d, ASR_ACT_NONE, st2);
+        }
         if (p->aux_cus > 0) asr_option_set(ASR_OPT_CU_LIMIT, old_lim);
         DEC_TRY(rc_kv);
     }
diff --git a/asr_chinese_e2e_amd/csrc/misc.hip b/asr_chinese_e2e_amd/csrc/misc.hip
--- a/asr_chinese_e2e_amd/csrc/misc.hip
+++ b/asr_chinese_e2e_amd/csrc/misc.hip
@@ -417,6 +417,50 @@
     }
 }
 
+template <typename T, bool ADD, int V>
+__global__ __launch_bounds__(EW_BLOCK) void rows_compact_kernel(const T* __restrict__ src, T* __restrict__ dst, int T_full, int Tk, int dv, int n) {
+    for (int i = blockIdx.x * EW_BLOCK + threadIdx.x; i < n; i += gridDim.x * EW_BLOCK) {
+        const unsigned r = (unsigned)i / (unsigned)dv, b = r / (unsigned)Tk;
+        const size_t full = (((size_t)b * T_full + (r - b * Tk)) * dv + (i - r * dv)) * V, comp = (size_t)i * V;
+        if constexpr (V == 4) {
+            if constexpr (ADD) {
+                const f32x4 a = load4<T>(dst + full), g = load4<T>(src + comp);
+                store4<T>(dst + full, a + g);
+            } else {
+                store4<T>(dst + comp, load4<T>(src + full));
+            }
+        } else {
+            if constexpr (ADD) dst[full] = from_f32<T>(to_f32<T>(dst[full]) + to_f32<T>(src[comp]));
+            else dst[comp] = src[full];
+        }
+    }
+}
+
+template <bool ADD>
+static int rows_compact(const void* src, void* dst, int B, int T, int Tk, int d, int dtype, void* stream, const char* who) {
+    if (!src || !dst) ASR_FAIL(ASR_EINVAL, "%s: null pointer", who);
+    if (B < 0 || d <= 0 || Tk < 0 || T < Tk) ASR_FAIL(ASR_EINVAL, "%s: bad shape B=%d T=%d Tk=%d d=%d", who, B, T, Tk, d);
+    if (dtype != ASR_F32 && dtype != ASR_BF16) ASR_FAIL(ASR_EDTYPE, "%s: dtype %d", who, dtype);
+    if ((size_t)B * Tk == 0) return ASR_OK;
+    hipStream_t st = (hipStream_t)stream;
+    const size_t es = dtype == ASR_F32 ? 4 : 2;
+    const bool vec = d % 4 == 0 && (((uintptr_t)src | (uintptr_t)dst) % (4 * es) == 0);
+    const int dv = vec ? d / 4 : d;
+    const size_t n = (size_t)B * Tk * dv;
+    if (n > (size_t)INT32_MAX - (2048 * EW_BLOCK)) ASR_FAIL(ASR_EINVAL, "%s: too many rows (B=%d T=%d Tk=%d d=%d)", who, B, T, Tk, d);
+#define ROWS(T_, V_) rows_compact_kernel<T_, ADD, V_><<<ew_grid(n), EW_BLOCK, 0, st>>>((const T_*)src, (T_*)dst, T, Tk, dv, (int)n)
+    if (dtype == ASR_F32) {
+        if (vec) ROWS(float, 4);
+        else ROWS(float, 1);
+    } else {
+        if (vec) ROWS(bf16_t, 4);
+        else ROWS(bf16_t, 1);
+    }
+#undef ROWS
+    ASR_CHECK_LAUNCH(who);
+    return ASR_OK;
+}
+
 __global__ __launch_bounds__(256) void loss_combine_kernel(const float* row_nll, int M, const float* n_valid, const float* nll, int B,
                                                            float w_ce, float w_ctc, float* loss) {
     __shared__ float red[16];
@@ -525,6 +569,14 @@
     else ASR_FAIL(ASR_EDTYPE, "asr_cast: dtypes %d -> %d", sd, dd);
     ASR_CHECK_LAUNCH("asr_cast");
     return ASR_OK;
+}
+
+extern "C" int asr_rows_gather(const void* src, void* dst, int B, int T, int Tk, int d, int dtype, void* stream) {
+    return rows_compact<false>(src, dst, B, T, Tk, d, dtype, stream, "asr_rows_gather");
+}
+
+extern "C" int asr_rows_scatter_add(const void* src, void* dst, int B, int T, int Tk, int d, int dtype, void* stream) {
+    return rows_compact<true>(src, dst, B, T, Tk, d, dtype, stream, "asr_rows_scatter_add");
 }
 
 extern "C" size_t asr_colsum_workspace_bytes(int rows, int cols) {
diff --git a/asr_chinese_e2e_amd/engine.py b/asr_chinese_e2e_amd/engine.py
--- a/asr_chinese_e2e_amd/engine.py
+++ b/asr_chinese_e2e_amd/engine.py
@@ -620,7 +620,7 @@
                 lin.wgrad(dy, x, with_bias=fused)
         self._keep += (dy, x)
 
-    def _attn_block_fwd(self, m, x, kv_src, B, Tq, Tk, k_len, q_lens, causal, window, cross, site, kv_pre=None):
+    def _attn_block_fwd(self, m, x, kv_src, B, Tq, Tk, k_len, q_lens, causal, window, cross, site, kv_pre=None, kv_rows=None):
         H, dk, hd = self.H, self.dk, self.H * self.dk
         c = {}
         if not cross:
@@ -643,7 +643,7 @@
         a = m.fc.fwd(ctx)
         y, xhat, rstd = K.add_ln_fwd(a, x, m.ln.g, m.ln.b, None, q_lens, B, Tq, xhat=a, drop_p=pf, drop_seed=sf, drop_mode=1)
         c.update(x=x, kv_src=kv_src, ctx=ctx, ctx_lo=ctx_lo, lse=lse, xhat=xhat, rstd=rstd, k_len=k_len, q_lens=q_lens, dims=(B, Tq, Tk), causal=causal,
-                 window=window, cross=cross, drop=(pa, sa, pf, sf))
+                 window=window, cross=cross, drop=(pa, sa, pf, sf), kv_rows=kv_rows)
         return y, c
 
     def _attn_block_bwd(self, m, c, dy, dy2, d_kv_src=None):
@@ -677,13 +677,19 @@
             self._wgrad(m.q, dq, c["x"], bias_from=dq)
             self._wgrad(m.kv, dkv, c["kv_src"], bias_from=dkv)
             dx = m.q.dgrad(dq)
+
+            def kv_src_grad():
+                if c["kv_rows"] is None:
+                    m.kv.dgrad(dkv, out=d_kv_src, accumulate=True)
+                else:
+                    K.rows_scatter_add(m.kv.dgrad(dkv), d_kv_src, B, c["kv_rows"], Tk)
             if self.aux_overlap and not torch.cuda.is_current_stream_capturing():
                 self._fork(self.ctc_stream)
                 with torch.cuda.stream(self.ctc_stream):
-                    m.kv.dgrad(dkv, out=d_kv_src, accumulate=True)
+                    kv_src_grad()
                 self._keep.append(dkv)
             else:
-                m.kv.dgrad(dkv, out=d_kv_src, accumulate=True)
+                kv_src_grad()
         if self._block_flush:
             self.flush_wgrads()
         return dx, dz
@@ -794,13 +800,17 @@
 
     DEC_CACHE_SHAPES = 6
 
+    @staticmethod
+    def cross_rows(W, T, text_mask):
+        return min(T, (max(W, 1) + 15) // 16 * 16) if text_mask else T
+
     def _dec_exec_ok(self, B, To, T):
         hd = self.H * self.dk
         return (self.dec_exec and self.dtype == torch.bfloat16 and K.TIMER is None and B * To <= Linear.SMALL_M and self.d % 8 == 0 and hd % 8 == 0
                 and self.ff % 8 == 0 and max(3 * hd, self.ff, self.d) <= Linear.SMALL_REDUCE)
 
-    def _dec_bufs(self, B, To, T, drop):
-        key = (B, To, T, bool(drop))
+    def _dec_bufs(self, B, To, T, Tk, drop):
+        key = (B, To, T, Tk, bool(drop))
         hit = self._dec_cache.get(key)
         capturing = torch.cuda.is_current_stream_capturing()
         if hit is not None:
@@ -814,10 +824,12 @@
         bf = lambda *shape: torch.empty(*shape, dtype=torch.bfloat16, device=dev)
         f32 = lambda *shape: torch.empty(*shape, dtype=torch.float32, device=dev)
         part_bytes = K.add_ln_bwd_workspace_bytes(M, d)
-        need = max(_lib.lib.asr_sdpa_bwd_workspace_bytes(B, H, To, T, self.dk, 0, -1, _lib.ASR_BF16), _lib.lib.asr_sdpa_bwd_workspace_bytes(B, H, To, To, self.dk, 1, -1, _lib.ASR_BF16))
+        need = max(_lib.lib.asr_sdpa_bwd_workspace_bytes(B, H, To, Tk, self.dk, 0, -1, _lib.ASR_BF16), _lib.lib.asr_sdpa_bwd_workspace_bytes(B, H, To, To, self.dk, 1, -1, _lib.ASR_BF16))
         delta = f32((need + 3) // 4)
         layers = []
-        kv_all, g_kv_all = bf(B * T, self.L * 2 * hd), bf(B * T, self.L * 2 * hd)
+        kv_all, g_kv_all = bf(B * Tk, self.L * 2 * hd), bf(B * Tk, self.L * 2 * hd)
+        compact = Tk < T
+        enc_x, g_enc_x = (bf(B * Tk, d), bf(B * Tk, d)) if compact else (None, None)
         for i, (slf, cross, ffn) in enumerate(self.dec):
             t = dict(qkv_s=bf(M, 3 * hd), ctx_s=bf(M, hd), a_s=bf(M, d), y_s=bf(M, d), lse_s=f32(B, H, To), rstd_s=f32(M),
                      q_c=bf(M, hd), kv_c=kv_all[:, i * 2 * hd:(i + 1) * 2 * hd], ctx_c=bf(M, hd), a_c=bf(M, d), y_c=bf(M, d), lse_c=f32(B, H, To), rstd_c=f32(M),
@@ -829,8 +841,10 @@
             if drop:
                 t.update(g_o=bf(M, d), g_ac=bf(M, d), g_as=bf(M, d))
             pl = _lib.DecLayerPlan()
-            pl.B, pl.To, pl.T, pl.d, pl.H, pl.dk, pl.ff = B, To, T, d, H, self.dk, ff
+            pl.B, pl.To, pl.T, pl.d, pl.H, pl.dk, pl.ff = B, To, Tk, d, H, self.dk, ff
             pl.ld_kv_c = self.L * 2 * hd
+            pl.T_enc = T
+            pl.g_enc_x = g_enc_x.data_ptr() if compact else None
             for name, ten in t.items():
                 setattr(pl, name, ten.data_ptr())
             for name, lin in (("qkv_s", slf.qkv), ("fc_s", slf.fc), ("q_c", cross.q), ("fc_c", cross.fc), ("1", ffn.w1), ("2", ffn.w2)):
@@ -840,13 +854,19 @@
                 setattr(pl, "g_" + name, ln.g.data_ptr())
                 setattr(pl, "be_" + name, ln.b.data_ptr())
             pl.gb_2, pl.gb_fc_c, pl.gb_fc_s = ffn.w2.gb.data_ptr(), cross.fc.gb.data_ptr(), slf.fc.gb.data_ptr()
-            if cross.kv.wlpT is not None:
+            if cross.kv.wlpT is not None and not compact:
                 pl.w_kv_c_T, pl.ld_kv_c_T = cross.kv.wlpT.data_ptr(), cross.kv.wlpT.stride(0)
             pl.delta, pl.delta_bytes = delta.data_ptr(), delta.numel() * 4
             t["kv_event"] = torch.cuda.Event()
             layers.append((pl, t))
-        hit = self._dec_cache[key] = dict(layers=layers, delta=delta, pinned=capturing, kv_all=kv_all, g_kv_all=g_kv_all, kv_event_rest=torch.cuda.Event())
+        hit = self._dec_cache[key] = dict(layers=layers, delta=delta, pinned=capturing, kv_all=kv_all, g_kv_all=g_kv_all, kv_event_rest=torch.cuda.Event(),
+                                          rows=(B, T, Tk), enc_x=enc_x, g_enc_x=g_enc_x)
         return hit
+
+    def _kv_src(self, bufs, enc):
+        if bufs["enc_x"] is None:
+            return enc
+        return K.rows_gather(enc, *bufs["rows"], out=bufs["enc_x"])
 
     def _kv_exec_async(self, bufs, enc):
         self._fork(self.ctc_stream)
@@ -854,13 +874,14 @@
             if self.dec_cu_limit:
                 K.set_cu_limit(self.dec_cu_limit)
             try:
+                src = self._kv_src(bufs, enc)
                 n0 = self.dec[0][1].kv.N
                 pl0, t0 = bufs["layers"][0]
-                self.dec[0][1].kv.fwd(enc, out=t0["kv_c"])
+                self.dec[0][1].kv.fwd(src, out=t0["kv_c"])
                 t0["kv_event"].record(self.ctc_stream)
                 pl0.kv_ready_event = t0["kv_event"].cuda_event
                 if self.L > 1:
-                    self.kv_all.rows(n0, self.kv_all.N).fwd(enc, out=bufs["kv_all"][:, n0:])
+                    self.kv_all.rows(n0, self.kv_all.N).fwd(src, out=bufs["kv_all"][:, n0:])
                     bufs["kv_event_rest"].record(self.ctc_stream)
                     for pl, t in bufs["layers"][1:]:
                         pl.kv_ready_event = bufs["kv_event_rest"].cuda_event
@@ -869,26 +890,27 @@
                     K.set_cu_limit(0)
         self._keep.append(enc)
 
-    def decoder_kv_async(self, prep, enc, B, T):
+    def decoder_kv_async(self, prep, enc, B, T, Tk=None):
         self._kv_ahead = None
         To = prep[0].shape[1]
         if not (self.aux_overlap and not torch.cuda.is_current_stream_capturing() and self._dec_exec_ok(B, To, T)):
             return
-        bufs = self._dec_bufs(B, To, T, self.training and self.drop_p > 0.0)
+        bufs = self._dec_bufs(B, To, T, T if Tk is None else Tk, self.training and self.drop_p > 0.0)
         self._kv_exec_async(bufs, enc)
         self._kv_ahead = (bufs, enc)
 
-    def _dec_exec_fwd(self, x, enc, dec_len, cross_len, B, To, T):
+    def _dec_exec_fwd(self, x, enc, dec_len, cross_len, B, To, T, Tk):
         drop = self.training and self.drop_p > 0.0
-        bufs = self._dec_bufs(B, To, T, drop)
+        bufs = self._dec_bufs(B, To, T, Tk, drop)
         main = K._stream()
         overlap = self.aux_overlap and not torch.cuda.is_current_stream_capturing()
         ahead, self._kv_ahead = self._kv_ahead, None
         if overlap and not (ahead is not None and ahead[0] is bufs and ahead[1] is enc):
             self._kv_exec_async(bufs, enc)
+        src = self._kv_src(bufs, enc) if not overlap else None
         for i, ((pl, t), (_, cross, _)) in enumerate(zip(bufs["layers"], self.dec)):
             if not overlap:
-                cross.kv.fwd(enc, out=t["kv_c"])
+                cross.kv.fwd(src, out=t["kv_c"])
                 pl.kv_ready_event = None
             pl.x_in = x.data_ptr()
             pl.dec_len, pl.cross_len = dec_len.data_ptr(), cross_len.data_ptr()
@@ -908,39 +930,45 @@
         M = dy.shape[0]
         nkv = self.dec[0][1].kv.N
         groups = {lo: (lo, hi) for lo, hi in self.kv_groups}
+        compact = bufs["enc_x"] is not None
+        src = bufs["enc_x"] if compact else enc
         for i in reversed(range(self.L)):
             pl, t = bufs["layers"][i]
             slf, cross, ffn = self.dec[i]
-            if cross.kv.wlpT is not None:
+            own_kv = compact or cross.kv.wlpT is not None
+            if own_kv and not compact:
                 cross.kv._fresh_transpose()
             if d_enc_ready is not None:
                 torch.cuda.current_stream().wait_event(d_enc_ready)
                 d_enc_ready = None
-            grp = groups.get(i) if cross.kv.wlpT is not None else None
+            grp = groups.get(i) if own_kv else None
             pl.d_enc, pl.kv_dgrad_cols, pl.g_kv_group = None, 0, None
             if grp is not None:
                 c0, c1 = grp[0] * nkv, grp[1] * nkv
                 pl.d_enc, pl.kv_dgrad_cols = d_enc.data_ptr(), c1 - c0
                 pl.g_kv_group = bufs["g_kv_all"][:, c0:].data_ptr()
-                pl.w_kv_c_T, pl.ld_kv_c_T = self.kv_all.wlpT[:, c0:].data_ptr(), self.kv_all.wlpT.stride(0)
+                if compact:
+                    pl.w_kv_c = self.kv_all.wlp[c0:].data_ptr()
+                else:
+                    pl.w_kv_c_T, pl.ld_kv_c_T = self.kv_all.wlpT[:, c0:].data_ptr(), self.kv_all.wlpT.stride(0)
             hand_over = self.armed_fork and self.overlap_wgrad and not torch.cuda.is_current_stream_capturing()
             pl.wgrad_stream = self._side_handle if hand_over else None
             pl.aux_cus = self.dec_cu_limit if aux is not None else 0
             _lib.check(_lib.fast.asr_decoder_layer_bwd(ctypes.addressof(pl), dy.data_ptr(), None if dy2 is None else dy2.data_ptr(), main, aux),
                        "asr_decoder_layer_bwd")
             self._armed = self._arm_covers_pending = hand_over
-            if cross.kv.wlpT is None:
+            if not own_kv:
                 cross.kv.dgrad(t["g_kvc"], out=d_enc, accumulate=True)
             self._wgrad(ffn.w2, t["g_o"] if drop else t["dz_f"], t["h"])
             self._wgrad(ffn.w1, t["g_h"], t["y_c"], bias_from=t["g_h"])
             self._wgrad(cross.fc, t["g_ac"] if drop else t["dz_c"], t["ctx_c"])
             self._wgrad(cross.q, t["g_qc"], t["y_s"], bias_from=t["g_qc"])
-            if cross.kv.wlpT is None:
+            if not own_kv:
                 self._wgrad(cross.kv, t["g_kvc"], enc, bias_from=t["g_kvc"])
             elif grp is not None:
                 c0, c1 = grp[0] * nkv, grp[1] * nkv
                 g = bufs["g_kv_all"][:, c0:c1]
-                self._wgrad(self.kv_all.rows(c0, c1), g, enc, bias_from=g)
+                self._wgrad(self.kv_all.rows(c0, c1), g, src, bias_from=g)
             self._wgrad(slf.fc, t["g_as"] if drop else t["dz_s"], t["ctx_s"])
             self._wgrad(slf.qkv, t["g_qkv"], t["x_in"], bias_from=t["g_qkv"])
             self._ln_pending += [(t["part_f"], ffn.ln.gg, ffn.ln.gb, ffn.w2.gb, M), (t["part_c"], cross.ln.gg, cross.ln.gb, cross.fc.gb, M),
@@ -950,32 +978,35 @@
             self._arm_covers_pending = False
         return dy, dy2
 
-    def decoder_fwd(self, prep, enc, cross_len, B, T):
+    def decoder_fwd(self, prep, enc, cross_len, B, T, Tk=None):
         ys_in, ys_out, labels32, dec_len, lab_len, n_valid = prep
         To = ys_in.shape[1]
+        Tk = T if Tk is None else Tk
         pe_, se_ = self._drop(2)
         x = K.embed_pe_fwd(ys_in.reshape(-1), self.emb32, self.pe, self.d ** -0.5, B, To, self.dtype, drop_p=pe_, drop_seed=se_)
         cache = dict(B=B, T=T, To=To, ys_in=ys_in, layers=[], drop=(pe_, se_))
         if self._dec_exec_ok(B, To, T):
-            x, bufs = self._dec_exec_fwd(x, enc, dec_len, cross_len, B, To, T)
+            x, bufs = self._dec_exec_fwd(x, enc, dec_len, cross_len, B, To, T, Tk)
             cache.update(exec_bufs=bufs, enc=enc, keep=(dec_len, cross_len))
             pred = self.prj.fwd(x)
             cache["x_last"] = x
             return pred, cache
         kv_pre = [None] * self.L
+        kv_rows = T if Tk < T else None
+        src = K.rows_gather(enc, B, T, Tk) if kv_rows else enc
         if self.aux_overlap and not torch.cuda.is_current_stream_capturing():
             self._fork(self.ctc_stream)
             with torch.cuda.stream(self.ctc_stream):
                 for i, (slf, cross, ffn) in enumerate(self.dec):
-                    kv = cross.kv.fwd(enc)
+                    kv = cross.kv.fwd(src)
                     e = torch.cuda.Event()
                     e.record(self.ctc_stream)
                     kv_pre[i] = (kv, e)
-            self._keep.append(enc)
+            self._keep += (enc, src)
             self._keep += [kv for kv, _ in kv_pre]
         for i, (slf, cross, ffn) in enumerate(self.dec):
             x1, c1 = self._attn_block_fwd(slf, x, x, B, To, To, dec_len, dec_len, True, -1, False, site=100 + 8 * i)
-            x2, c2 = self._attn_block_fwd(cross, x1, enc, B, To, T, cross_len, dec_len, False, -1, True, site=102 + 8 * i, kv_pre=kv_pre[i])
+            x2, c2 = self._attn_block_fwd(cross, x1, src, B, To, Tk, cross_len, dec_len, False, -1, True, site=102 + 8 * i, kv_pre=kv_pre[i], kv_rows=kv_rows)
             x, c3 = self._ffn_block_fwd(ffn, x2, B, To, dec_len, site=104 + 8 * i)
             cache["layers"].append((c1, c2, c3))
         pred = self.prj.fwd(x)
diff --git a/asr_chinese_e2e_amd/kernels.py b/asr_chinese_e2e_amd/kernels.py
--- a/asr_chinese_e2e_amd/kernels.py
+++ b/asr_chinese_e2e_amd/kernels.py
@@ -530,6 +530,21 @@
     return dst
 
 
+def rows_gather(src, B, T, Tk, out=None):
+    assert src.is_contiguous() and src.dim() == 2 and src.shape[0] == B * T and 0 <= Tk <= T
+    out = torch.empty(B * Tk, src.shape[1], dtype=src.dtype, device=src.device) if out is None else out
+    assert out.is_contiguous() and out.shape == (B * Tk, src.shape[1]) and out.dtype == src.dtype
+    check(lib.asr_rows_gather(_p(src), _p(out), B, T, Tk, src.shape[1], _dt(src), _stream()), "asr_rows_gather")
+    return out
+
+
+def rows_scatter_add(src, dst, B, T, Tk):
+    assert src.is_contiguous() and dst.is_contiguous() and src.dtype == dst.dtype and 0 <= Tk <= T
+    assert src.shape == (B * Tk, dst.shape[1]) and dst.shape[0] == B * T
+    check(lib.asr_rows_scatter_add(_p(src), _p(dst), B, T, Tk, dst.shape[1], _dt(dst), _stream()), "asr_rows_scatter_add")
+    return dst
+
+
 def grad_sumsq(g, out, ws):
     _chk_f32(g, out)
     w = ws.get(lib.asr_sumsq_workspace_bytes(g.numel()))
diff --git a/include/asr_hip.h b/include/asr_hip.h
--- a/include/asr_hip.h
+++ b/include/asr_hip.h
@@ -141,6 +141,8 @@
 size_t asr_colsum_workspace_bytes(int rows, int cols);
 int asr_colsum(const void* x, float* out, void* ws, size_t ws_bytes, int rows, int cols, int ld,
                int accumulate, int dtype, void* stream);
+int asr_rows_gather(const void* src, void* dst, int B, int T, int Tk, int d, int dtype, void* stream);
+int asr_rows_scatter_add(const void* src, void* dst, int B, int T, int Tk, int d, int dtype, void* stream);
 int asr_cast(const void* src, void* dst, size_t n, int src_dtype, int dst_dtype, void* stream);
 int asr_transpose_batched_bf16(const void* src, void* dst, const int32_t* tiles, int ntiles, void* stream);
 
@@ -213,6 +215,9 @@
     int kv_dgrad_cols;
     const void* g_kv_group;
     void *ctx_s_lo, *ctx_c_lo;
+    const void* w_kv_c;
+    void* g_enc_x;
+    int T_enc;
 } asr_dec_layer_plan;
 int asr_decoder_layer_fwd(const asr_dec_layer_plan* plan, void* stream);
 int asr_decoder_layer_bwd(const asr_dec_layer_plan* plan, const void* dy, const void* dy2, void* stream, void* aux_stream);
```
